# beltegeuse/rustlight

Measured on AMD Instinct MI355X. Metric: Msamples/s (paths/s) at 1080p x 128spp cbox, higher is better.
Workload: dtype f32

## Files before the change

rustlight_amd/csrc/device_types.h:

```cpp
#pragma once
#include <stdint.h>

namespace rl {

struct alignas(16) BvhNode {
    float lmin[3]; float lmax0;
    float lmax12[2]; float rmin01[2];
    float rmin2; float rmax[3];
    int32_t left, right; int32_t pad0, pad1;
};
static_assert(sizeof(BvhNode) == 64, "BvhNode must be 64 bytes");
static const int32_t RL_CHILD_NONE = (int32_t)0x80000000;

struct alignas(16) BvhNode2 {
    float lox[4], loy[4], loz[4];
    float hix[4], hiy[4], hiz[4];
    int32_t slot[4];
    int32_t child[2];
    int32_t pad[2];
};
static_assert(sizeof(BvhNode2) == 128, "BvhNode2 must be 128 bytes");

struct alignas(16) Bvh4Node {
    float org[3];
    uint32_t exps;
    uint32_t qlo[3];
    uint32_t qhi[3];
    int32_t child[4];
    uint32_t pad[2];
};
static_assert(sizeof(Bvh4Node) == 64, "Bvh4Node must be 64 bytes");

struct alignas(16) TriRecord {
    float v0[3]; float n0;
    float e1[3]; float n1;
    float e2[3]; float n2;
    float det;
    int32_t mesh;
    int32_t tri;
    int32_t gtri;
};
static_assert(sizeof(TriRecord) == 64, "TriRecord must be 64 bytes");

struct ColorTex {
    int32_t type;
    float c0[3];
    float c1[3];
    float offset[2];
    float scale[2];
    float line_width;
    int32_t bitmap;
    int32_t pad[3];
};
static_assert(sizeof(ColorTex) == 64, "ColorTex must be 64 bytes");

struct BitmapDesc { uint32_t w, h; uint64_t offset; };

struct Material {
    int32_t type;
    int32_t distribution;
    float exponent, weight_specular;
    float alpha_u, alpha_v;
    float glass_eta, glass_inv_eta;
    int32_t smooth;
    int32_t twosided;
    int32_t pad[2];
    ColorTex diffuse, specular, transmittance, eta, k;
};

struct MeshRecord {
    int32_t material;
    int32_t flags;
    float emission[3];
    float inv_area;
    float emitter_pdf;
    uint32_t vertex_base;
    uint32_t tri_base;
    uint32_t n_tris;
    uint32_t cdf_base;
    uint32_t ats_base;
    int32_t emission_type;
    float emission_scale;
    int32_t emission_bitmap;
};
enum { MESH_HAS_NORMALS = 1, MESH_HAS_UV = 2, MESH_IS_LIGHT = 4 };

enum { EMITTER_MESH = 0, EMITTER_ENV = 1, EMITTER_POINT = 2, EMITTER_DIRECTIONAL = 3 };
struct EmitterRecord {
    int32_t kind;
    int32_t mesh;
    float v[3];
    float c[3];
    float center[3];
    float radius;
    float pad[4];
};
static_assert(sizeof(EmitterRecord) == 64, "EmitterRecord must be 64 bytes");

struct LightNode {
    float bmin[3], bmax[3];
    float axis[3];
    float phi, cos_theta_o, cos_theta_e;
    int32_t left, right, parent;
    int32_t light;
};
static_assert(sizeof(LightNode) == 64, "LightNode must be 64 bytes");

struct CameraRecord {
    float sample_to_camera[16];
    float to_world[16];
    float position[3];
    uint32_t width, height;
};

struct MediumRecord {
    int32_t enabled;
    float sigma_a[3], sigma_s[3], sigma_t[3];
    int32_t phase;
    float g;
};

struct DeviceScene {
    const BvhNode* nodes;
    const TriRecord* tris;
    float root_min[3], root_max[3];
    int32_t root;
    uint32_t n_nodes, n_prims;
    uint32_t stack_depth;
    const BvhNode* nodes_t;
    int32_t root_t;
    const BvhNode2* nodes2;
    const Bvh4Node* nodes4;
    int32_t root4;
    uint32_t stack_depth4;
    const uint32_t* tri_indices;
    const float* positions;
    const float* normals;
    const float* uvs;
    const MeshRecord* meshes;
    const Material* materials;
    const BitmapDesc* bitmaps;
    const float* bitmap_texels;
    const EmitterRecord* emitters;
    const float* emitters_cdf;
    uint32_t n_emitters;
    int32_t env_emitter;
    float env_color[3];
    float env_pdf;
    uint32_t env_w, env_h;
    const float* env_texels;
    const float* env_cond_cdf;
    const float* env_cond_func;
    const float* env_marg_cdf;
    float env_marg_func_int;
    float env_sel_pdf;
    int32_t ats_root;
    const LightNode* ats_nodes;
    const int32_t* ats_light_mesh;
    const int32_t* ats_light_prim;
    const uint32_t* ats_leaf_of;
    const float* mesh_cdf;
    uint32_t n_meshes;
    CameraRecord camera;
    MediumRecord medium;
};

}
```

rustlight_amd/csrc/kernels/fused_body.inc.h:

```cpp
    const RenderConst& rc = rc_arg;
    const DeviceScene& sc = sc_arg;
    extern __shared__ __attribute__((aligned(16))) float4 smem[];
    SceneRecs recs;
    float4* after_scene = smem;
    if (LDS_SCENE) {
        stage_scene_lds(sc, smem, smem + lds_nodes_float4s(sc.n_nodes));
        recs.nodes = smem; recs.tris = smem + lds_nodes_float4s(sc.n_nodes);
        after_scene = smem + lds_scene_float4s(sc.n_nodes, sc.n_prims);
    } else {
        recs.nodes = streamed_nodes<TravStackT<false>>(sc);
        recs.tris = reinterpret_cast<const float4*>(sc.tris);
    }
    const unsigned tid = blockIdx.x * blockDim.x + threadIdx.x;
    unsigned long long* cold_q = reinterpret_cast<unsigned long long*>(after_scene);
    float* cold_f = reinterpret_cast<float*>(cold_q + 256 * FusedState::kColdQ);
    unsigned* cold_u = reinterpret_cast<unsigned*>(cold_f + 256 * FusedState::kColdF);
    const TravStackT<LDS_SCENE> stack(make_stack<LDS_SCENE>(stc, cold_u + 256 * FusedState::kColdU, tid));
    FusedState ps;
    ps.cold_q = cold_q + threadIdx.x; ps.cold_f = cold_f + threadIdx.x; ps.cold_u = cold_u + threadIdx.x;
#pragma unroll
    for (int i = 0; i < F_COUNT; i++) ps.fv[i] = 0.0f;
#pragma unroll
    for (int i = 0; i < U_COUNT; i++) ps.uv[i] = 0u;
#pragma unroll
    for (int i = 0; i < Q_COUNT; i++) ps.qv[i] = 0ull;
    storec(ps, F_AR, czero());
    PU(U_CURSOR) = 0u; PU(U_SAMPLE) = 0u;
    const unsigned item0 = (tid & ((1u << rc.item_shift) - 1u)) == 0u ? (tid >> rc.item_shift) : 0xffffffffu;
    PU(U_ITEM) = item0;
    PU(U_PRIM) = 0xffffffffu;
    PU(U_FLAGS) = item0 < rc.n_items ? (ST_REGEN | ST_FRESH) : ST_FINISHED;
    unsigned n_samples = 0, n_draws = 0, n_vertices = 0, n_shadow = 0, n_ext = 0;
#ifdef RL_STAGE_TIMERS
    unsigned long long tm[4] = {0, 0, 0, 0}, ln[5] = {0, 0, 0, 0, 0};
    unsigned long long sh_hist[5] = {0, 0, 0, 0, 0}, sh_pair[4] = {0, 0, 0, 0}, sh_cyc_exec = 0; unsigned sh_prev = 0, sh_parity = 0;
#define RL_T0 { t0 = __builtin_readcyclecounter(); }
#define RL_T1(K, COND) { unsigned long long t1 = __builtin_readcyclecounter(); tm[K] += t1 - t0; ln[K] += __popcll(__ballot(COND)); t0 = t1; }
    unsigned long long t0;
    const unsigned long long wg_t0 = wall_clock64();
#else
#define RL_T0
#define RL_T1(K, COND)
#endif
    constexpr bool qmode = QUEUE;
    constexpr unsigned kQDone = 0xffffffffu;
    if constexpr (qmode) {
        PU(U_ITEM) = 0u;
        PU(U_FLAGS) = ST_FINISHED;
    }
    for (;;) {
    if constexpr (qmode) {
        const char __attribute__((address_space(4)))* kq = (const char __attribute__((address_space(4)))*)__builtin_amdgcn_kernarg_segment_ptr();
        asm volatile("" : "+s"(kq));
        const RenderConst& rc_arg = *(const RenderConst*)kq;
        const unsigned ipb = 256u * rc_arg.split, total = rc_arg.q_n * ipb;
        unsigned fl = PU(U_FLAGS);
        for (int tries = 0; tries < 4; tries++) {
            if ((fl & ST_FINISHED) && PU(U_ITEM) != kQDone) {
                const unsigned c = atomicAdd(rc_arg.q_ctr, 1u);
                if (c >= total) PU(U_ITEM) = kQDone;
                else {
                    const unsigned j = rc_arg.q_list[c / ipb], idx = c - (c / ipb) * ipb;
                    unsigned bx_, by_, bw_, bh_;
                    block_geometry(rc_arg, rc_arg.owned_blocks[j], &bx_, &by_, &bw_, &bh_);
                    const unsigned npx = min(rc_arg.cursor_end, bw_ * bh_) - min(rc_arg.cursor_begin, bw_ * bh_);
                    if (idx < npx * rc_arg.split) {
                        PU(U_ITEM) = rc_arg.block_item_base[j] * rc_arg.split + idx;
                        PU(U_PRIM) = 0xffffffffu; PU(U_CURSOR) = 0u; PU(U_SAMPLE) = 0u;
                        storec(ps, F_AR, czero());
                        fl = ST_REGEN | ST_FRESH;
                    }
                }
            }
            if (__ballot((fl & ST_FINISHED) && PU(U_ITEM) != kQDone) == 0ull) break;
        }
        PU(U_FLAGS) = fl;
        if (__ballot(!(fl & ST_FINISHED)) == 0ull) {
            if (__ballot((fl & ST_FINISHED) && PU(U_ITEM) != kQDone) == 0ull) break;
            continue;
        }
    }
    if (!(PU(U_FLAGS) & ST_FINISHED)) do {
        const char __attribute__((address_space(4)))* ka = (const char __attribute__((address_space(4)))*)__builtin_amdgcn_kernarg_segment_ptr();
        asm volatile("" : "+s"(ka));
        constexpr size_t sc_off = (sizeof(RenderConst) + alignof(DeviceScene) - 1) / alignof(DeviceScene) * alignof(DeviceScene);
        static_assert(sc_off == offsetof(PathKernargs, sc) && offsetof(PathKernargs, rc) == 0, "kernarg layout of k_path_fused(RenderConst, DeviceScene, StackConf)");
        const DeviceScene& sc = *(const DeviceScene*)(ka + sc_off);
        const RenderConst& rc = MEDIUM ? *(const RenderConst*)ka : rc_arg;
        RL_T0
#ifdef RL_STAGE_TIMERS
        ln[4] += 64;
        const bool c0 = PU(U_FLAGS) & ST_REGEN;
#endif
#ifdef RL_FUSED_BODY_TAIL
        constexpr bool kTail = RL_FUSED_BODY_TAIL;
#else
        constexpr bool kTail = false;
#endif
        if (PU(U_FLAGS) & ST_REGEN) raygen_slot<true, decltype(ps), SMP, kTail>(rc, sc, ps, n_samples, n_draws);
        RL_T1(0, c0)
#ifdef RL_STAGE_TIMERS
        const bool c1 = PU(U_FLAGS) & ST_RAY;
#endif
        if (PU(U_FLAGS) & ST_RAY) {
            extend_slot(sc, recs, stack, ps);
            RL_T1(1, c1)
            shade_slot<MAT, MEDIUM, LIGHTS, false, SMP>(rc, sc, ps, PU(U_FLAGS), n_vertices, n_draws, n_shadow, n_ext);
        }
        RL_T1(2, c1)
#ifdef RL_STAGE_TIMERS
        const bool c3 = PU(U_FLAGS) & ST_SHADOW;
#endif
        if (PU(U_FLAGS) & ST_SHADOW) shadow_slot(sc, recs, stack, ps);
#ifdef RL_STAGE_TIMERS
        { const unsigned nsh = (unsigned)__popcll(__ballot(c3)); sh_hist[nsh == 0u ? 0 : 1 + (nsh - 1u) / 16u]++;
          if (nsh) sh_cyc_exec += __builtin_readcyclecounter() - t0;
          if (sh_parity) { const unsigned a = sh_prev, b = nsh; sh_pair[(a == 0u && b == 0u) ? 0 : ((a == 0u || b == 0u) ? 1 : (a + b <= 64u ? 2 : 3))]++; }
          sh_prev = nsh; sh_parity ^= 1u; }
#endif
        RL_T1(3, c3)
    } while (!qmode && !(PU(U_FLAGS) & ST_FINISHED));
    if (!qmode) break;
    }
#ifdef RL_STAGE_TIMERS
    if ((threadIdx.x & 63u) == 0u) { for (int k = 0; k < 4; k++) { atomicAdd(&g_stage_timers[k], tm[k]); atomicAdd(&g_stage_timers[4 + k], ln[k]); } atomicAdd(&g_stage_timers[8], ln[4]);
        for (int k = 0; k < 5; k++) atomicAdd(&g_stage_timers[16 + k], sh_hist[k]); for (int k = 0; k < 4; k++) atomicAdd(&g_stage_timers[21 + k], sh_pair[k]); atomicAdd(&g_stage_timers[25], sh_cyc_exec); }
#endif
    {
        const int which[5] = {STAT_SAMPLES, STAT_VERTICES, STAT_DRAWS, STAT_SHADOW_RAYS, STAT_EXT_RAYS};
        const unsigned vals[5] = {n_samples, n_vertices, n_draws, n_shadow, n_ext};
        block_stats<5>(rc.partials, which, vals);
    }
#ifdef RL_STAGE_TIMERS
    if (threadIdx.x == 0u && blockIdx.x < kFusedWgSlots) { g_fused_wgs[2 * blockIdx.x] = wg_t0; g_fused_wgs[2 * blockIdx.x + 1] = wall_clock64(); }
#endif
```

rustlight_amd/csrc/kernels/knobs.h:

```cpp
#pragma once
#include <cstdlib>
#include <cstring>
#include <string>

namespace rl {

enum KnobId {
    K_REF_SINGLE_PASS,
    K_STATE_BUDGET_MB,
    K_NO_OVERLAP,
    K_CHAIN_SERIAL,
    K_CHAIN_NO_PRE,
    K_CHAIN_NO_TREELETS,
    K_SPEC_FORCE,
    K_SPEC_DRAWS_PER_SAMPLE,
    K_ITEM_SHIFT,
    K_FUSED_DYNAMIC,
    K_FUSED_TAIL_BLOCKS,
    K_FUSED_TAIL_SPLIT,
    K_FUSED_TAIL_NO_BUFFER_TEST,
    K_EVAL_SPLIT,
    K_EVAL_MIN, K_EVAL_DIV,
    K_NO_EVENTS,
    K_QUEUE_DEBUG,
    K_SPEC_GROUP, K_SPEC_SUB, K_SPEC_CAP, K_SPEC_PROBE, K_SPEC_LEAD, K_SPEC_LEAD_MAX, K_SPEC_LEAD_VAR, K_SPEC_EXTRA, K_SPEC_DENSE, K_SPEC_DENSE_FRAC,
    K_SPEC_PROBE_EVERY, K_SPEC_KS, K_SPEC_KE, K_SPEC_SERIAL_RATIO, K_SPEC_NO_TRIVIAL, K_SPEC_LDS_LIMIT_TEST, K_SPEC_STATS, K_SPEC_WAVE_TIMES,
    K_SPEC_LDS_LEVELS,
    K_VPL_BATCH_PATHS,
    K_PHOTON_TREE_GROUP_PHOTONS,
    K_PLANE_GENERATE_LANES,
    K_PLANE_TREE_DEVICE,
    K_PLANE_TREE_GROUP_PLANES,
    K_PPLANE_TREE_DEVICE,
    K_FORCE_STREAMING,
    K_GENERIC_LIGHTS,
    K_COUNT
};

struct Knobs {
    struct Entry { bool set = false; std::string value; };
    Entry e[K_COUNT];

    static const char* name_of(int k) {
        static const char* const names[K_COUNT] = {
            "ref_single_pass", "state_budget_mb", "no_overlap", "chain_serial", "chain_no_pre", "chain_no_treelets", "spec_force", "spec_draws_per_sample", "item_shift",
            "fused_dynamic", "fused_tail_blocks", "fused_tail_split", "fused_tail_no_buffer_test", "eval_split", "eval_min", "eval_div", "no_events", "queue_debug",
            "spec_group", "spec_sub", "spec_cap", "spec_probe", "spec_lead", "spec_lead_max", "spec_lead_var", "spec_extra", "spec_dense", "spec_dense_frac",
            "spec_probe_every", "spec_ks", "spec_ke", "spec_serial_ratio", "spec_no_trivial", "spec_lds_limit_test", "spec_stats", "spec_wave_times", "spec_lds_levels", "vpl_batch_paths", "photon_tree_group_photons",
            "plane_generate_lanes", "plane_tree_device", "plane_tree_group_planes", "pplane_tree_device",
            "force_streaming", "generic_lights"};
        return names[k];
    }
    static int find(const char* name) {
        if (!name) return -1;
        for (int k = 0; k < K_COUNT; k++) if (std::strcmp(name, name_of(k)) == 0) return k;
        return -1;
    }
    void from_environment() {
        for (int k = 0; k < K_COUNT; k++) {
            std::string env = "RL_";
            for (const char* p = name_of(k); *p; p++) env += (char)((*p >= 'a' && *p <= 'z') ? *p - 'a' + 'A' : *p);
            const char* v = std::getenv(env.c_str());
            e[k].set = v != nullptr;
            e[k].value = v ? v : "";
        }
    }
    bool has(int k) const { return e[k].set; }
    const char* str(int k) const { return e[k].set ? e[k].value.c_str() : nullptr; }
    long long i(int k, long long dflt) const { return e[k].set ? std::atoll(e[k].value.c_str()) : dflt; }
    double f(int k, double dflt) const { return e[k].set ? std::atof(e[k].value.c_str()) : dflt; }
};

}
```

rustlight_amd/csrc/kernels/path_render.hip.h:

```cpp
#pragma once

namespace {

using namespace rl;

std::atomic<int> g_path_renders_in_flight{0};

struct Plan { unsigned split, n_items, P, item_shift; };
struct Chunk { unsigned c0, c1, n_pix; std::vector<unsigned> base; };
struct Tail { unsigned begin, pixels, shift; };

class PathRender : RenderFrame {
public:
    PathRender(rl_context* c, const rl_path_params* p, const uint64_t* seeds, size_t nb, float* out, int out_dev, void* stream_arg, rl_render_stats* s)
        : RenderFrame(c, seeds, nb, out, out_dev, stream_arg, s, p->shard_index, p->shard_count), params(p) {}

    int run() {
        struct InFlight { InFlight() { g_path_renders_in_flight++; } ~InFlight() { g_path_renders_in_flight--; } } in_flight;
        int r;
        if ((r = choose_form()) != RL_OK) return r;
        plan_chunks();
        if ((r = plan_lanes()) != RL_OK) return r;
        if ((r = upload()) != RL_OK) return r;
        if (two_pass) r = run_two_pass();
        else if (fused) r = run_fused();
        else r = run_wavefront();
        if (r != RL_OK) return r;
        return finish();
    }

private:
    const rl_path_params* const params;
    bool per_sample = false, fused = false, fast_math = false, two_pass = false, medium = false;
    bool strat = false;
    bool overlap_wanted = false;
    bool one_lane_per_pixel = false;
    bool overlapped = false;
    size_t state_budget = 0;
    std::vector<Chunk> chunks;
    unsigned max_chunk_pix = 0;
    Plan plan{1u, 0u, 0u, 0u}, plan_chain{1u, 0u, 0u, 0u};
    Tail tail{0u, 0u, 0u};
    long long tail_blocks = 0;
    unsigned tail_shift = 0;
    bool tail_forced = false;
    unsigned split = 1, n_items = 0, item_shift = 0, P = 0, n_item_pixels = 0;
    Pool pool{};
    RenderConst rc{};
    StackConf stc{};
    size_t lds_trav = 0, lds_fused = 0;
    double ms[4] = {0, 0, 0, 0}, ms_fused = 0.0, ms_chain = 0.0, ms_eval_span = 0.0;
    uint64_t iterations = 0, launches = 2, n_extend = 0;
    unsigned long long spec_stat[3] = {0, 0, 0};
    unsigned spec_group = 0;
    bool spec = false;
    SpecConf spc{};
    unsigned spec_threads = 0;
    StackConf stc_c{}, stc_s{};
    size_t lds_chain = 0, lds_spec = 0;
    int spec_levels = -1;

    static constexpr unsigned kMaxEvalLaunches = 256u;
    static constexpr size_t kEventsPerIter = 8;

    int choose_form() {
        strat = params->stream_mode == RL_STREAM_STRATIFIED;
        per_sample = params->stream_mode == RL_STREAM_PER_SAMPLE || strat;
        if (params->pipeline > 2) { rl_set_error("pipeline must be 0 (auto), 1 (wavefront) or 2 (fused)"); return RL_ERR_INVALID_ARGUMENT; }
        fused = params->pipeline == 2 || (params->pipeline == 0 && params->pool_slots == 0);
        fast_math = params->numerics == RL_NUMERICS_FAST;
        if (fast_math && !fused) { rl_set_error("numerics = fast exists for the persistent kernel only (pipeline 0 or 2, pool_slots 0)"); return RL_ERR_UNSUPPORTED; }
        if (fast_math && strat) { rl_set_error("numerics = fast is not built with the stratified sampler (stream_mode = RL_STREAM_STRATIFIED)"); return RL_ERR_UNSUPPORTED; }
        medium = ctx->ds.medium.enabled != 0;
        two_pass = !per_sample && fused && !owned.empty() && !knobs.has(K_REF_SINGLE_PASS);
        state_budget = max_state_bytes();
        if (two_pass && (size_t)owned.size() * params->spp * 32 > state_budget) two_pass = false;
        return RL_OK;
    }

    bool dynamic_items() const { return knobs.has(K_FUSED_DYNAMIC) ? knobs.i(K_FUSED_DYNAMIC, 0) != 0 : (medium || !ctx->lds_scene); }

    Plan plan_items(bool per_pixel, unsigned n_pix, unsigned n_chains, unsigned tail_lanes = 0u) const {
        Plan pl{1u, 0u, 0u, 0u};
        if (per_pixel && n_pix > 0) {
            const unsigned fused_groups = (n_pix + 255u) / 256u;
            const unsigned fused_auto = fused_groups >= 6000u ? 1u : std::max(1u, 16384u / std::max(1u, fused_groups));
            unsigned want = params->sample_split ? params->sample_split
                                : (fused ? (ctx->lds_scene ? fused_auto : std::max(fused_auto, 64u))
                                         : (ctx->lds_scene ? 1u : std::max(1u, (8u << 20) / std::max(1u, n_pix))));
            if (overlap_wanted && !params->sample_split) want = std::max(want, (unsigned)std::max<long long>(1, knobs.i(K_EVAL_SPLIT, 4)));
            if (tail_forced) want = 1u;
            pl.split = std::max(1u, std::min(want, params->spp));
            if ((size_t)n_pix * params->spp * 3 * sizeof(float) > kSampleBufBudget || one_lane_per_pixel) pl.split = 1;
            while (pl.split > 1 && (size_t)n_pix * pl.split > (size_t)0x7fffff00u) pl.split--;
        }
        pl.n_items = per_pixel ? n_pix * pl.split + tail_lanes : n_chains;
        unsigned Pp = params->pool_slots ? std::min(params->pool_slots, std::max(pl.n_items, 1u)) : std::min<unsigned>(pl.n_items, 16u << 20);
        Pp = std::max(256u, (unsigned)(((unsigned long long)Pp + 255ull) / 256ull * 256ull));
        if (fused) {
            const unsigned resident = (unsigned)cus * (unsigned)(ctx->lds_scene ? RL_FUSED_WAVES : RL_FUSED_WAVES_STREAMING) * 256u;
            Pp = std::max(256u, (std::min(pl.n_items, dynamic_items() ? resident : pl.n_items) + 255u) / 256u * 256u);
            const unsigned resident4 = (unsigned)cus * 4u * 256u / ((medium && !per_pixel) ? 2u : 1u);
            while (pl.item_shift < 6u && ((size_t)pl.n_items << (pl.item_shift + 1u)) <= resident4) pl.item_shift++;
            if (!per_pixel && knobs.has(K_ITEM_SHIFT)) pl.item_shift = std::min(6u, (unsigned)std::max<long long>(0, knobs.i(K_ITEM_SHIFT, 0)));
            if (pl.item_shift) Pp = std::max(256u, (unsigned)((((size_t)pl.n_items << pl.item_shift) + 255u) / 256u * 256u));
        }
        pl.P = Pp;
        return pl;
    }

    void plan_chunks() {
        if (two_pass && !knobs.has(K_STATE_BUDGET_MB)) {
            size_t free_b = 0, total_b = 0;
            if (hipMemGetInfo(&free_b, &total_b) == hipSuccess) state_budget = std::min(state_budget, ctx->d_sample_states.capacity() * sizeof(unsigned long long) + free_b / 10 * 6);
            else (void)hipGetLastError();
        }
        for (bool planned_states = false; two_pass && !planned_states;) {
            const size_t budget = state_budget;
            const size_t per_cursor = (size_t)owned.size() * params->spp * 32;
            if (per_cursor > budget) { two_pass = false; chunks.clear(); break; }
            chunks.clear();
            const unsigned cursors_per_chunk = (unsigned)std::max<size_t>(1, std::min<size_t>(256, budget / std::max<size_t>(1, per_cursor)));
            for (unsigned c0 = 0; c0 < 256u; c0 += cursors_per_chunk) {
                Chunk ch; ch.c0 = c0; ch.c1 = std::min(256u, c0 + cursors_per_chunk); ch.n_pix = 0;
                for (size_t j = 0; j < owned.size(); j++) {
                    const BlockRect r = block_rect(owned[j], nby, W, H);
                    const unsigned npx = r.w * r.h;
                    ch.base.push_back(ch.n_pix);
                    ch.n_pix += std::min(ch.c1, npx) - std::min(ch.c0, npx);
                }
                if (ch.n_pix) chunks.push_back(std::move(ch));
            }
            size_t need = 0;
            for (const Chunk& ch : chunks) need = std::max(need, (size_t)ch.n_pix * params->spp * 4);
            if (ctx->d_sample_states.ensure(need) == RL_OK) planned_states = true;
            else state_budget /= 2;
        }
        max_chunk_pix = 0;
        for (const Chunk& ch : chunks) max_chunk_pix = std::max(max_chunk_pix, ch.n_pix);
    }

    int plan_lanes() {
        overlap_wanted = two_pass && ctx->stream2 && !fast_math && !knobs.has(K_NO_OVERLAP) && knobs.i(K_SPEC_GROUP, 0) != 256;
        int rcode;
        tail_request();
        for (int attempt = 0; attempt < 2; attempt++) {
            plan = two_pass ? plan_items(true, max_chunk_pix, 0) : plan_items(per_sample, n_pixels, (unsigned)owned.size());
            if (two_pass) for (const Chunk& ch : chunks) { const Plan pc = plan_items(true, ch.n_pix, 0); plan.P = std::max(plan.P, pc.P); plan.split = std::max(plan.split, pc.split); }
            plan_chain = two_pass ? plan_items(false, 0, (unsigned)owned.size()) : Plan{1u, 0u, 0u, 0u};
            split = plan.split; n_items = plan.n_items; item_shift = plan.item_shift;
            P = std::max(plan.P, plan_chain.P);
            n_item_pixels = two_pass ? max_chunk_pix : n_pixels;
            if (split <= 1) break;
            if (ctx->d_sample_buf.ensure((size_t)n_item_pixels * params->spp * 3) == RL_OK) break;
            if (params->sample_split || attempt == 1) return RL_ERR_HIP;
            one_lane_per_pixel = true; overlap_wanted = false;
        }
        if ((rcode = plan_tail()) != RL_OK) return rcode;
        if ((rcode = alloc_tables()) != RL_OK) return rcode;
        if (per_sample || two_pass) {
            if (per_sample && (rcode = ctx->d_item_seed.ensure(n_item_pixels)) != RL_OK) return rcode;
            if ((rcode = ctx->d_item_pixel.ensure(n_item_pixels)) != RL_OK) return rcode;
        }
        if (two_pass) {
            if ((rcode = ctx->d_sample_states.ensure((size_t)max_chunk_pix * params->spp * 4)) != RL_OK) return rcode;
            if ((rcode = ctx->d_chain_states.ensure(owned.size() * 4)) != RL_OK) return rcode;
        }
        if (!fused && ctx->pool_q.capacity() / Q_COUNT < P) {
            ctx->pool_f.reset(); ctx->pool_u.reset(); ctx->pool_q.reset();
            if (ctx->pool_f.ensure((size_t)F_COUNT * P) != RL_OK || ctx->pool_u.ensure((size_t)U_COUNT * P) != RL_OK || ctx->pool_q.ensure((size_t)Q_COUNT * P) != RL_OK) {
                ctx->pool_f.reset(); ctx->pool_u.reset(); ctx->pool_q.reset();
                rl_set_error("out of device memory for a path-state pool of " + std::to_string(P) + " slots");
                return RL_ERR_HIP;
            }
        }
        pool = Pool{ctx->pool_f.get(), ctx->pool_u.get(), ctx->pool_q.get(), P};
        return alloc_output(std::max<size_t>((P + 255) / 256, (size_t)cus * 8u * rl_context::kEvalStreams));
    }

    static constexpr unsigned kFusedTailBlocks = 512u, kFusedTailSplit = 4u;
    void tail_request() {
        tail_blocks = 0; tail_shift = 0; tail_forced = false;
        if (!per_sample || strat || two_pass || !fused || !ctx->lds_scene || medium || dynamic_items() || params->sample_split || owned.empty()) return;
        const bool large = (n_pixels + 255u) / 256u >= 6000u && ctx->single_bsdf && ctx->bsdf_type == RL_BSDF_DIFFUSE && ctx->area_lights_only && !fast_math && g_path_renders_in_flight.load() <= 1;
        const long long T = knobs.has(K_FUSED_TAIL_BLOCKS) ? knobs.i(K_FUSED_TAIL_BLOCKS, 0) : (large ? (long long)kFusedTailBlocks : 0);
        const long long S = std::min<long long>(std::min<long long>(knobs.has(K_FUSED_TAIL_SPLIT) ? knobs.i(K_FUSED_TAIL_SPLIT, 0) : (long long)kFusedTailSplit, 64), params->spp);
        unsigned shift = 0;
        while ((2ll << shift) <= S) shift++;
        if (T <= 0 || shift == 0u) return;
        tail_blocks = T; tail_shift = shift;
        tail_forced = knobs.has(K_FUSED_TAIL_BLOCKS) || knobs.has(K_FUSED_TAIL_SPLIT);
    }
    int plan_tail() {
        tail = Tail{0u, 0u, 0u};
        if (tail_blocks <= 0 || split != 1u) return RL_OK;
        const long long T = tail_blocks;
        const unsigned shift = tail_shift;
        const bool expand = !params->has_max_depth || 1u < params->max_depth;
        const uint64_t key = ((uint64_t)params->shard_index << 33) | ((uint64_t)shard_count << 1) | (expand ? 1u : 0u);
        if (key != ctx->heavy_key || ctx->heavy_blocks.size() != owned.size()) {
            std::vector<unsigned> masks;
            trivial_pixel_masks(trivial_input(ctx), params, owned, nby, false, &masks, true);
            ctx->heavy_blocks.assign(owned.size(), 0);
            for (size_t j = 0; j < owned.size(); j++) ctx->heavy_blocks[j] = (masks[j * 8] & 1u) ? 0 : 1;
            ctx->heavy_key = key;
        }
        size_t j0 = 0, j1 = 0; long long found = 0;
        for (size_t j = owned.size(); j-- > 0 && found < T;) if (ctx->heavy_blocks[j]) { if (!found) j1 = j; j0 = j; found++; }
        if (!found) return RL_OK;
        const unsigned p0 = item_base[j0], p1 = j1 + 1 < owned.size() ? item_base[j1 + 1] : n_pixels;
        const size_t lanes = (size_t)(p1 - p0) << shift;
        if ((size_t)n_pixels + lanes > (size_t)0x7fffff00u || (size_t)(p1 - p0) * params->spp * 3 * sizeof(float) > kSampleBufBudget) return RL_OK;
        if (knobs.has(K_FUSED_TAIL_NO_BUFFER_TEST) || ctx->d_sample_buf.ensure((size_t)(p1 - p0) * params->spp * 3) != RL_OK) { rl_set_error(""); return RL_OK; }
        tail = Tail{p0, p1 - p0, shift};
        plan = plan_items(true, n_pixels, 0, (unsigned)lanes - tail.pixels);
        n_items = plan.n_items; item_shift = plan.item_shift;
        P = std::max(plan.P, plan_chain.P);
        return RL_OK;
    }

    int upload() {
        int rcode;
        if ((rcode = RenderFrame::upload(!two_pass, true)) != RL_OK) return rcode;
        Counters init{};
        init.active = std::min(plan.P, n_items);
        init.next_item = item_shift ? n_items : plan.P;
        if (!two_pass) HIP_OK(hipMemcpyAsync(ctx->d_counters.get(), &init, sizeof(init), hipMemcpyHostToDevice, st));
        if ((rcode = zero_rows()) != RL_OK) return rcode;

        rc = render_const(params->spp, params->stream_mode, params->seed_variant);
        rc.has_min = params->has_min_depth; rc.min_depth = params->min_depth;
        rc.has_max = params->has_max_depth; rc.max_depth = params->max_depth;
        rc.has_rr = params->has_rr_depth; rc.rr_depth = params->rr_depth;
        rc.strategy = params->strategy; rc.single_scattering = params->single_scattering;
        rc.n_items = n_items;
        rc.item_shift = item_shift;
        rc.split = split; rc.sample_buf = ctx->d_sample_buf.get();
        rc.tail_begin = tail.begin; rc.tail_pixels = tail.pixels; rc.tail_shift = tail.shift; rc.tail_lanes = tail.pixels << tail.shift;
        rc.sample_states = ctx->d_sample_states.get(); rc.chain_states = ctx->d_chain_states.get();

        lds_trav = traversal_lds_bytes(ctx, ctx->lds_scene, 256, true);
        if ((rcode = stack_conf(ctx, (size_t)((P + 255) / 256) * 256, &stc)) != RL_OK) return rcode;
        lds_fused = traversal_lds_bytes(ctx, ctx->lds_scene, 256, false) + kFusedColdBytes;

        const dim3 block(256);
        if (per_sample && !owned.empty()) hipLaunchKernelGGL(k_seed_pixels, dim3(((unsigned)owned.size() + 63) / 64), dim3(64), 0, st, rc);
        if (!fused) hipLaunchKernelGGL(k_init, dim3((plan.P + 255) / 256), block, 0, st, rc, pool);

        return grow_events(kEventsPerIter * (per_sample ? 8u : 32u));
    }

    void launch_fused(const RenderConst& rcl, dim3 grid, hipStream_t on, const StackConf* stcl = nullptr) const {
        const int mat = ctx->single_bsdf ? ctx->bsdf_type : -1;
        const StackConf& s = stcl ? *stcl : stc;
        if (strat)
            (ctx->lds_scene ? launch_fused_strat_lds : launch_fused_strat_stream)(medium, ctx->area_lights_only, grid, dim3(256), lds_fused, on, rcl, ctx->ds, s);
        else if (rcl.queue_mode != 0u)
            (ctx->lds_scene ? launch_fusedq_lds : launch_fusedq_stream)(mat, medium, ctx->area_lights_only, grid, dim3(256), lds_fused, on, rcl, ctx->ds, s);
        else
            (ctx->lds_scene ? (fast_math ? launch_fused_lds_fast : launch_fused_lds) : (fast_math ? launch_fused_stream_fast : launch_fused_stream))(mat, medium, ctx->area_lights_only, grid, dim3(256), lds_fused, on, rcl, ctx->ds, s);
    }

    void drain() const {
        (void)hipStreamSynchronize(st);
        for (int k = 0; k < rl_context::kEvalStreams; k++) if (ctx->eval_streams[k]) (void)hipStreamSynchronize(ctx->eval_streams[k]);
        (void)hipGetLastError();
    }
    struct DrainOnError {
        const PathRender* r; bool armed = true;
        ~DrainOnError() { if (armed) r->drain(); }
    };

    int plan_chain_pass() {
        stc_c = stc;
        if (ctx->lds_scene && !medium && ctx->ds.n_nodes <= 64u && ctx->ds.n_prims <= 64u && plan_chain.item_shift >= 5u && !knobs.has(K_CHAIN_NO_PRE)) stc_c.pre_group = 1 << plan_chain.item_shift;
        const bool treelets = !ctx->lds_scene && !fast_math && ctx->ds.nodes_t && ctx->ds.root_t >= 0 && plan_chain.item_shift >= 5u && ctx->ds.stack_depth <= 512u && !knobs.has(K_CHAIN_NO_TREELETS);
        if (treelets) stc_c.pre_group = 1 << plan_chain.item_shift;
        auto chain_lds_of = [&](bool tl) {
            return traversal_lds_bytes(ctx, ctx->lds_scene, 256, false) + (tl ? (size_t)(256 / stc_c.pre_group) * (72 + (ctx->ds.stack_depth + 1) / 2) * 16
                   : (stc_c.pre_group ? (size_t)(256 / stc_c.pre_group) * ((size_t)ctx->ds.n_nodes * 32 + (size_t)ctx->ds.n_prims * 8) : 0));
        };
        if (chain_lds_of(treelets) > ctx->lds_limit) stc_c.pre_group = 0;
        lds_chain = chain_lds_of(treelets && stc_c.pre_group != 0);

        spec = !fast_math && !knobs.has(K_CHAIN_SERIAL);
        const bool spec_force = knobs.has(K_SPEC_FORCE);
        if (spec && !spec_force) {
            const double nbar = knobs.f(K_SPEC_DRAWS_PER_SAMPLE, medium ? 150.0 : 12.0);
            if ((double)params->spp < 4.0 * nbar) spec = false;
        }
        spec_levels = ctx->lds_scene ? -1 : (int)std::max<long long>(0, std::min<long long>(knobs.i(K_SPEC_LDS_LEVELS, kSpecLdsLevelsStreaming), lds_levels_of(ctx)));
        lds_spec = traversal_lds_bytes(ctx, ctx->lds_scene, 256, false, spec_levels) + (size_t)(kSpecColdWords - (ctx->lds_scene ? 0 : kSpecHelperWords)) * 256 * 4 + kSpecGroupLdsBytes;
        const size_t spec_lds_limit = knobs.has(K_SPEC_LDS_LIMIT_TEST) ? (size_t)knobs.i(K_SPEC_LDS_LIMIT_TEST, 0) : ctx->lds_limit;
        if (lds_spec > spec_lds_limit) spec = false;
        spc = SpecConf{};
        spec_threads = 0;
        if (spec) {
            unsigned group = 16u;
            while (group < 64u && (size_t)owned.size() * group < (size_t)cus * 4u * 2u * 64u) group <<= 1;
            if (!ctx->lds_scene) group = 64u;
            if (knobs.has(K_SPEC_GROUP)) { const long long g = knobs.i(K_SPEC_GROUP, 0); if (g == 16 || g == 32 || g == 64 || g == 256) group = (unsigned)g; }
            spc.group = group;
            spc.sub = std::max(1u, group / 16u);
            spc.serial_ratio = spec_force ? 0.0f : (float)knobs.f(K_SPEC_SERIAL_RATIO, 3.0);
            if (knobs.has(K_SPEC_SUB)) { const long long v = knobs.i(K_SPEC_SUB, 0); if ((v == 1 || v == 2 || v == 4 || v == 8 || v == 16) && (unsigned)v <= group) spc.sub = (unsigned)v; }
            spc.cap = std::max(96u, std::min(3u * params->spp + 64u, 1u << 20));
            if (knobs.has(K_SPEC_CAP)) spc.cap = std::max(4u, (unsigned)knobs.i(K_SPEC_CAP, 0));
            spc.probe = knobs.has(K_SPEC_PROBE) ? (unsigned)knobs.i(K_SPEC_PROBE, 0) : std::min(32u, std::max(4u, params->spp));
            spc.lead = (unsigned)knobs.i(K_SPEC_LEAD, 24);
            spc.lead_max = (unsigned)knobs.i(K_SPEC_LEAD_MAX, 128);
            spc.lead_var = (float)knobs.f(K_SPEC_LEAD_VAR, 100.0);
            spc.extra = (unsigned)knobs.i(K_SPEC_EXTRA, 0);
            spc.dense = !ctx->lds_scene ? 0u : (knobs.has(K_SPEC_DENSE) ? std::min(64u, (unsigned)knobs.i(K_SPEC_DENSE, 0)) : 16u);
            spc.dense_frac = (float)knobs.f(K_SPEC_DENSE_FRAC, 0.6);
            spc.probe_every = (unsigned)knobs.i(K_SPEC_PROBE_EVERY, 0);
            spc.ks = (float)knobs.f(K_SPEC_KS, group >= 64u ? 2.5 : 1.65);
            spc.ke = (float)knobs.f(K_SPEC_KE, group >= 64u ? 2.5 : 1.65);
            spec_threads = (unsigned)((((size_t)owned.size() * group) + 255u) / 256u * 256u);
            const size_t need = (size_t)spec_threads * spc.cap * 36u;
            size_t free_b = 0, total_b = 0;
            const size_t have = ctx->d_trk_off.capacity() * 4u + ctx->d_trk_st.capacity() * 16u;
            if (hipMemGetInfo(&free_b, &total_b) != hipSuccess) { (void)hipGetLastError(); free_b = 0; }
            if (need > have && need - have > free_b / 2u) spec = false;
            if (spec && (ctx->d_trk_off.ensure((size_t)spec_threads * spc.cap) != RL_OK || ctx->d_trk_st.ensure((size_t)spec_threads * spc.cap * 2u) != RL_OK)) spec = false;
        }
        int rcode;
        if (spec) {
            const bool expand = !params->has_max_depth || 1u < params->max_depth;
            const bool no_trivial = knobs.has(K_SPEC_NO_TRIVIAL);
            const uint64_t key = ((uint64_t)params->shard_index << 33) | ((uint64_t)shard_count << 1) | (expand ? 1u : 0u);
            if (key != ctx->trivial_key || ctx->d_trivial.capacity() < owned.size() * 8 || no_trivial) {
                std::vector<unsigned> masks;
                trivial_pixel_masks(trivial_input(ctx), params, owned, nby, no_trivial, &masks);
                if ((rcode = ctx->d_trivial.ensure(masks.size())) != RL_OK) return rcode;
                HIP_OK(hipMemcpyAsync(ctx->d_trivial.get(), masks.data(), masks.size() * sizeof(unsigned), hipMemcpyHostToDevice, st));
                HIP_OK(hipStreamSynchronize(st));
                ctx->trivial_key = no_trivial ? ~0ull : key;
            }
            if ((rcode = ctx->d_spec_stats.ensure(32 + 8 * (size_t)(spec_threads / 64u))) != RL_OK) return rcode;
            HIP_OK(hipMemsetAsync(ctx->d_spec_stats.get(), 0, 32 * sizeof(unsigned long long), st));
            spc.trk_off = ctx->d_trk_off.get(); spc.trk_st = ctx->d_trk_st.get(); spc.trivial = ctx->d_trivial.get();
            spc.stats = (stats || knobs.has(K_SPEC_STATS)) ? ctx->d_spec_stats.get() : nullptr;
            const size_t n_thr = std::max<size_t>((size_t)((P + 255) / 256) * 256, spec_threads);
            if ((rcode = stack_conf(ctx, n_thr, &stc_s, false, spec_levels)) != RL_OK) return rcode;
            if ((rcode = stack_conf(ctx, n_thr, &stc)) != RL_OK) return rcode;
            stc_c.overflow = stc.overflow; stc_c.overflow_stride = stc.overflow_stride;
        }
        return RL_OK;
    }

    void launch_chain_pass(const RenderConst& ra) const {
        const int mat = ctx->single_bsdf ? ctx->bsdf_type : -1;
        if (spec) (ctx->lds_scene ? launch_spec_lds : launch_spec_stream)(mat, medium, dim3(spec_threads / 256u), dim3(256), lds_spec, st, ra, ctx->ds, stc_s, spc);
        else (ctx->lds_scene ? (fast_math ? launch_chain_lds_fast : launch_chain_lds) : (fast_math ? launch_chain_stream_fast : launch_chain_stream))(mat, medium, dim3((plan_chain.P + 255) / 256), dim3(256), lds_chain, st, ra, ctx->ds, stc_c);
    }

    int prepare_queue(RenderConst& ra, unsigned chain_grid) {
        const size_t n_dev = 16 + (size_t)kMaxEvalLaunches + owned.size(), n_flags = 16 + owned.size();
        int rcode;
        if ((rcode = ctx->d_queue.ensure(n_dev)) != RL_OK || (rcode = ctx->h_flags.ensure(n_flags)) != RL_OK || (rcode = ctx->h_list.ensure(owned.size())) != RL_OK) return rcode;
        HIP_OK(hipMemsetAsync(ctx->d_queue.get(), 0, (16 + (size_t)kMaxEvalLaunches) * sizeof(unsigned), st));
        ra.queue = ctx->d_queue.get(); ra.chain_grid = chain_grid;
        ra.done_flags = ctx->h_flags.device_ptr() + 16; ra.started_flag = ctx->h_flags.device_ptr();
        ra.queue_seq = ++ctx->queue_seq;
        if (ra.queue_seq == 0u) { std::memset(ctx->h_flags.get(), 0, ctx->h_flags.capacity() * sizeof(unsigned)); ra.queue_seq = ++ctx->queue_seq; }
        return RL_OK;
    }

    int overlap_loop(const RenderConst& rb, const Plan& pb, unsigned seq, dim3 grid_q, const StackConf& stc_q) {
        HIP_OK(hipEventRecord(ctx->ev_chain_done, st));
        const unsigned n_blocks_owned = (unsigned)owned.size();
        volatile unsigned* hf = ctx->h_flags.get();
        std::vector<unsigned> waiting(n_blocks_owned);
        for (unsigned j = 0; j < n_blocks_owned; j++) waiting[j] = j;
        unsigned n_listed = 0, n_launches = 0, scan_from = 0;
        const auto poll_us = std::chrono::microseconds(50 + n_blocks_owned / 100u);
        bool chain_over = false, started = false;
        const unsigned resident = grid_q.x;
        const unsigned batch_min = (unsigned)std::max<long long>(1, knobs.i(K_EVAL_MIN, 64)), batch_div = (unsigned)std::max<long long>(1, knobs.i(K_EVAL_DIV, 5));
        std::chrono::steady_clock::time_point t_first{};
        auto launch_batch = [&](unsigned first, unsigned count) -> int {
            const unsigned k = n_launches % (unsigned)rl_context::kEvalStreams;
            hipStream_t on = ctx->eval_streams[k];
            HIP_OK(hipMemcpyAsync(ctx->d_queue.get() + 16 + kMaxEvalLaunches + first, ctx->h_list.get() + first, count * sizeof(unsigned), hipMemcpyHostToDevice, on));
            RenderConst rq = rb;
            rq.q_list = ctx->d_queue.get() + 16 + kMaxEvalLaunches + first; rq.q_n = count; rq.q_ctr = ctx->d_queue.get() + 16 + n_launches;
            rq.partials = rb.partials + (size_t)k * resident * STAT_COUNT;
            StackConf stc_k = stc_q;
            if (stc_k.overflow) stc_k.overflow += (size_t)k * resident * 256u * 2u;
            const unsigned wgs = std::min<unsigned>(resident, (unsigned)(((size_t)count * 256u * pb.split + 255u) / 256u));
            if (n_launches == 0) t_first = std::chrono::steady_clock::now();
            launch_fused(rq, dim3(std::max(1u, wgs)), on, &stc_k);
            HIP_OK(hipGetLastError());
            n_launches++; launches++;
            return RL_OK;
        };
        int rcode;
        while (n_listed < n_blocks_owned) {
            if (!chain_over) {
                const hipError_t qe = hipEventQuery(ctx->ev_chain_done);
                if (qe == hipSuccess) chain_over = true;
                else if (qe != hipErrorNotReady) { rl_set_error(std::string("hipEventQuery(chain pass): ") + hipGetErrorString(qe)); (void)hipGetLastError(); return RL_ERR_HIP; }
            }
            if (!started && hf[0] == seq) started = true;
            if (started || chain_over) {
                size_t keep = 0;
                for (size_t w = 0; w < waiting.size(); w++) {
                    const unsigned j = waiting[w];
                    if (chain_over || hf[16 + j] == seq) ctx->h_list.get()[n_listed++] = j; else waiting[keep++] = j;
                }
                waiting.resize(keep);
            }
            const unsigned fresh = n_listed - scan_from, to_come = n_blocks_owned - scan_from;
            if (fresh > 0 && (chain_over || (fresh >= std::max(batch_min, to_come / batch_div) && n_launches + 2u < kMaxEvalLaunches))) {
                if ((rcode = launch_batch(scan_from, fresh)) != RL_OK) return rcode;
                scan_from = n_listed;
            }
            if (n_listed < n_blocks_owned && !chain_over) std::this_thread::sleep_for(poll_us);
        }
        if (scan_from < n_listed && (rcode = launch_batch(scan_from, n_listed - scan_from)) != RL_OK) return rcode;
        if (knobs.has(K_QUEUE_DEBUG)) std::fprintf(stderr, "[queue] %u evaluation launches beside / after the chain pass, %u blocks, started flag %s\n", n_launches, n_listed, started ? "seen" : "not seen");
        HIP_OK(hipStreamSynchronize(st));
        for (int k = 0; k < rl_context::kEvalStreams; k++) HIP_OK(hipStreamSynchronize(ctx->eval_streams[k]));
        if (n_launches) ms_eval_span += std::chrono::duration<double, std::milli>(std::chrono::steady_clock::now() - t_first).count();
        return RL_OK;
    }

    int run_chunk(const Chunk& ch) {
        DrainOnError guard{this};
        const dim3 block(256);
        HIP_OK(hipMemcpyAsync(ctx->d_item_base.get(), ch.base.data(), ch.base.size() * sizeof(unsigned), hipMemcpyHostToDevice, st));
        RenderConst ra = rc;
        ra.stream_mode = RL_STREAM_REFERENCE_ORDER;
        ra.n_items = plan_chain.n_items; ra.item_shift = plan_chain.item_shift; ra.split = 1;
        ra.n_state_pixels = ch.n_pix; ra.cursor_begin = ch.c0; ra.cursor_end = ch.c1;
        const unsigned chain_grid = spec ? spec_threads / 256u : (plan_chain.P + 255u) / 256u;
        const bool overlap = overlap_wanted;
        int rcode;
        if (overlap && (rcode = prepare_queue(ra, chain_grid)) != RL_OK) return rcode;
        hipLaunchKernelGGL(k_chunk_pixels, dim3(((unsigned)owned.size() + 63) / 64), dim3(64), 0, st, ra);
        const Plan pb = plan_items(true, ch.n_pix, 0);
        RenderConst rb = ra;
        rb.stream_mode = kStreamGivenStates;
        rb.n_items = pb.n_items; rb.item_shift = pb.item_shift; rb.split = pb.split;
        rb.queue = nullptr; rb.queue_mode = 0u; rb.done_flags = nullptr; rb.started_flag = nullptr;
        Counters cinit{};
        cinit.active = std::min(pb.P, pb.n_items);
        cinit.next_item = pb.item_shift ? pb.n_items : pb.P;
        if (overlap) cinit.next_item = pb.n_items;
        HIP_OK(hipMemcpyAsync(ctx->d_counters.get(), &cinit, sizeof(cinit), hipMemcpyHostToDevice, st));
        const dim3 grid_q((unsigned)cus * (unsigned)(ctx->lds_scene ? RL_FUSED_WAVES : RL_FUSED_WAVES_STREAMING));
        StackConf stc_q = stc;
        if (overlap && (rcode = stack_conf(ctx, (size_t)grid_q.x * 256 * rl_context::kEvalStreams, &stc_q, true)) != RL_OK) return rcode;
        if (timing) hipEventRecord(ctx->events[0], st);
        launch_chain_pass(ra);
        if (timing) hipEventRecord(ctx->events[1], st);
        HIP_OK(hipGetLastError());
        if (overlap) {
            rb.queue = ctx->d_queue.get(); rb.queue_mode = 1u; rb.chain_grid = chain_grid;
            if ((rcode = overlap_loop(rb, pb, ra.queue_seq, grid_q, stc_q)) != RL_OK) return rcode;
            overlapped = true;
            if (timing) hipEventRecord(ctx->events[3], st);
        } else {
            if (timing) hipEventRecord(ctx->events[2], st);
            launch_fused(rb, dim3((pb.P + 255) / 256), st);
            if (timing) hipEventRecord(ctx->events[3], st);
        }
        if (pb.split > 1) hipLaunchKernelGGL(k_fold_samples, dim3((ch.n_pix + 255) / 256), block, 0, st, rb);
        HIP_OK(hipGetLastError());
        HIP_OK(hipStreamSynchronize(st));
        guard.armed = false;
        if (timing) {
            float t = 0.0f;
            HIP_OK(hipEventElapsedTime(&t, ctx->events[0], ctx->events[1])); ms_chain += t;
            HIP_OK(hipEventElapsedTime(&t, ctx->events[overlap ? 1 : 2], ctx->events[3])); ms_fused += t;
            if (!overlap) ms_eval_span += t;
        }
        launches += 3 + (pb.split > 1 ? 1 : 0);
        return RL_OK;
    }

    int run_two_pass() {
        int rcode;
        if ((rcode = plan_chain_pass()) != RL_OK) return rcode;
        for (const Chunk& ch : chunks) if ((rcode = run_chunk(ch)) != RL_OK) return rcode;
        dump_stage_timers(ctx->lds_scene);
        if (ctx->lds_scene) dump_chain_timers_lds(); else dump_chain_timers_stream();
        if (spec && spc.stats && (rcode = read_spec_stats()) != RL_OK) return rcode;
        iterations = chunks.size();
        return RL_OK;
    }

    int read_spec_stats() {
        unsigned long long spec_totals[32] = {0};
        HIP_OK(hipMemcpy(spec_totals, ctx->d_spec_stats.get(), sizeof(spec_totals), hipMemcpyDeviceToHost));
        spec_group = spc.group; spec_stat[0] = spec_totals[0]; spec_stat[1] = spec_totals[1]; spec_stat[2] = spec_totals[2];
        const bool verbose = knobs.has(K_SPEC_STATS);
        if (verbose) std::fprintf(stderr, "[spec] LDS per workgroup %zu bytes (scene %zu, %d stack levels)\n", lds_spec, (size_t)(ctx->lds_scene ? ctx->scene_lds_bytes : 0), stc_s.lds_levels);
        if (verbose) std::fprintf(stderr, "[spec] group %u x sub %u cap %u: %llu speculative + %llu serial + %llu probe samples for %llu camera samples (%.2f x, %.2f serial per pixel), %llu wave iterations\n",
            spc.group, spc.sub, spc.cap, spec_totals[0], spec_totals[1], spec_totals[2], (unsigned long long)n_pixels * params->spp,
            (double)(spec_totals[0] + spec_totals[1] + spec_totals[2]) / std::max(1.0, (double)n_pixels * params->spp), (double)spec_totals[1] / std::max(1u, n_pixels), spec_totals[3]);
        if (knobs.has(K_SPEC_WAVE_TIMES) && spec_totals[8]) {
            std::vector<unsigned long long> wt(8 * (size_t)(spec_threads / 64u));
            HIP_OK(hipMemcpy(wt.data(), ctx->d_spec_stats.get() + 32, wt.size() * 8, hipMemcpyDeviceToHost));
            FILE* f = std::fopen(knobs.str(K_SPEC_WAVE_TIMES), "w");
            if (f) { unsigned long long t0 = ~0ull; for (size_t w = 0; w < wt.size() / 8; w++) if (wt[8 * w]) t0 = std::min(t0, wt[8 * w]);
                     for (size_t w = 0; w < wt.size() / 8; w++) std::fprintf(f, "%zu %.3f %.3f %llu %llu %.3f %.3f %llu %llu\n", w, (wt[8 * w] - t0) * 1e-5, (wt[8 * w + 1] - t0) * 1e-5, wt[8 * w + 2], wt[8 * w + 3], wt[8 * w + 4] * 1e-5, wt[8 * w + 5] * 1e-5, wt[8 * w + 6], wt[8 * w + 7]); std::fclose(f); }
        }
        if (verbose && spec_totals[8]) {
            const double tot = (double)(spec_totals[4] + spec_totals[5] + spec_totals[6] + spec_totals[7] + spec_totals[8]);
            std::fprintf(stderr, "[spec] cycles: bookkeeping %.1f %%, plan %.1f %%, thread %.1f %%, copy-out %.1f %%, extend+shade %.1f %%; %.1f lanes per traced iteration, %.1f %% of the traced iterations serial only, %.0f cycles per wave iteration\n",
                100.0 * spec_totals[4] / tot, 100.0 * spec_totals[5] / tot, 100.0 * spec_totals[6] / tot, 100.0 * spec_totals[7] / tot, 100.0 * spec_totals[8] / tot,
                (double)spec_totals[9] / std::max<double>(1.0, (double)spec_totals[10]), 100.0 * spec_totals[11] / std::max<double>(1.0, (double)spec_totals[10]), tot / std::max<double>(1.0, (double)spec_totals[3]));
            { const double ts = (double)(spec_totals[16] + spec_totals[17] + spec_totals[18] + spec_totals[19] + spec_totals[20]);
              std::fprintf(stderr, "[spec] iterations after a serial-only one (%.1f %% of all cycles): bookkeeping %.1f %%, plan %.1f %%, thread %.1f %%, copy-out %.1f %%, extend+shade %.1f %%\n", 100.0 * ts / tot,
                100.0 * spec_totals[16] / ts, 100.0 * spec_totals[17] / ts, 100.0 * spec_totals[18] / ts, 100.0 * spec_totals[19] / ts, 100.0 * spec_totals[20] / ts); }
            std::fprintf(stderr, "[spec] slow walks: %llu from a pixel's start, %llu across a missing link, %llu past the last track\n", spec_totals[12], spec_totals[13], spec_totals[14]);
            std::fprintf(stderr, "[spec] serial walks on helpers: %llu (one lane: %llu), %llu rounds, %llu samples taken from them\n", spec_totals[26], spec_totals[27], spec_totals[24], spec_totals[25]);
        }
        return RL_OK;
    }

    int run_fused() {
        if (timing) hipEventRecord(ctx->events[0], st);
        launch_fused(rc, dim3((plan.P + 255) / 256), st);
        if (timing) hipEventRecord(ctx->events[1], st);
        HIP_OK(hipGetLastError());
        HIP_OK(hipStreamSynchronize(st));
        if (timing) { float t = 0.0f; HIP_OK(hipEventElapsedTime(&t, ctx->events[0], ctx->events[1])); ms_fused = t; ms_eval_span = t; }
        dump_stage_timers(ctx->lds_scene);
        launches += 1;
        iterations = 1;
        return RL_OK;
    }

    int run_wavefront() {
        const dim3 block(256);
        const dim3 grid_all((plan.P + 255) / 256);
        const bool use_sort = !ctx->single_bsdf;
        const unsigned sort_chunks = split > 1 ? 4u : 1u;
        const dim3 grid_sort((P + 1023) / 1024);
        const dim3 grid_persistent(std::min<unsigned>((P + 255) / 256, (unsigned)cus * 8u));
        const unsigned poll_every = per_sample ? 8u : 32u;
        const DeviceScene& ds = ctx->ds;
        unsigned in_batch = 0;
        auto flush_events = [&](unsigned count) -> int {
            for (unsigned i = 0; i < count; i++)
                for (int k = 0; k < 4; k++) {
                    float t = 0.0f;
                    HIP_OK(hipEventElapsedTime(&t, ctx->events[kEventsPerIter * i + 2 * k], ctx->events[kEventsPerIter * i + 2 * k + 1]));
                    ms[k] += t;
                }
            return RL_OK;
        };
        for (;;) {
            hipEvent_t* ev = timing ? &ctx->events[kEventsPerIter * in_batch] : nullptr;
            if (timing) hipEventRecord(ev[0], st);
            if (strat) launch_raygen_strat(grid_persistent, block, st, rc, ds, pool);
            else hipLaunchKernelGGL(k_raygen, grid_persistent, block, 0, st, rc, ds, pool);
            if (timing) { hipEventRecord(ev[1], st); hipEventRecord(ev[2], st); }
            if (ctx->lds_scene) hipLaunchKernelGGL((k_extend<true>), grid_all, block, lds_trav, st, rc, ds, pool, stc);
            else hipLaunchKernelGGL((k_extend<false>), grid_all, block, lds_trav, st, rc, ds, pool, stc);
            if (timing) { hipEventRecord(ev[3], st); hipEventRecord(ev[4], st); }
            if (strat) launch_shade_sorted_strat(medium, sort_chunks, sort_chunks == 4u ? grid_sort : grid_all, block, st, rc, ds, pool);
            else if (use_sort) launch_shade_sorted(medium, sort_chunks, sort_chunks == 4u ? grid_sort : grid_all, block, st, rc, ds, pool);
            else launch_shade_type(ctx->bsdf_type, medium, grid_all, block, st, rc, ds, pool);
            launches += 1;
            if (timing) { hipEventRecord(ev[5], st); hipEventRecord(ev[6], st); }
            if (ctx->lds_scene) hipLaunchKernelGGL((k_shadow<true>), grid_all, block, lds_trav, st, rc, ds, pool, stc);
            else hipLaunchKernelGGL((k_shadow<false>), grid_all, block, lds_trav, st, rc, ds, pool, stc);
            if (timing) hipEventRecord(ev[7], st);
            launches += 3;
            n_extend++;
            iterations++;
            in_batch++;
            if (in_batch == poll_every) {
                HIP_OK(hipGetLastError());
                HIP_OK(hipMemcpyAsync(ctx->h_counters.get(), ctx->d_counters.get(), sizeof(Counters), hipMemcpyDeviceToHost, st));
                HIP_OK(hipStreamSynchronize(st));
                if (timing) { int r = flush_events(in_batch); if (r != RL_OK) return r; }
                in_batch = 0;
                if (ctx->h_counters.get()->active == 0) break;
            }
            if (iterations > (uint64_t)1 << 28) { rl_set_error("render did not terminate"); return RL_ERR_HIP; }
        }
#ifdef RL_TRAV_STATS
        {
            unsigned long long h[8];
            HIP_OK(hipStreamSynchronize(st));
            hipMemcpyFromSymbol(h, HIP_SYMBOL(g_trav_stats), sizeof(h));
            std::fprintf(stderr, "[trav] rays %llu (zero-step %.1f %%)  steps/ray %.1f  tris/ray %.1f  waves %llu  lanes/wave %.1f  paid steps/ray %.1f  step utilisation %.1f %%\n",
                         h[0], 100.0 * h[5] / (double)h[0], (double)h[1] / h[0], (double)h[2] / h[0], h[4], (double)h[0] / h[4], (double)h[3] / h[0], 100.0 * h[1] / (double)h[3]);
            std::memset(h, 0, sizeof(h)); hipMemcpyToSymbol(HIP_SYMBOL(g_trav_stats), h, sizeof(h));
        }
#endif
        return RL_OK;
    }

    int finish() {
        if (split > 1 && !two_pass) { hipLaunchKernelGGL(k_fold_samples, dim3((n_pixels + 255) / 256), dim3(256), 0, st, rc); launches += 1; }
        else if (tail.pixels) { hipLaunchKernelGGL(k_fold_samples, dim3((tail.pixels + 255) / 256), dim3(256), 0, st, rc); launches += 1; }
        const int rcode = download();
        if (rcode != RL_OK) return rcode;
        if (stats) {
            stats->iterations = iterations;
            stats->kernel_launches = launches;
            stats->ms_raygen = ms[0]; stats->ms_extend = ms[1]; stats->ms_shade = ms[2]; stats->ms_shadow = ms[3];
            stats->ms_other = ms_fused;
            stats->ms_prepass = ms_chain;
            stats->n_extend_launches = n_extend;
            stats->reserved[0] = spec_stat[0]; stats->reserved[1] = spec_stat[1]; stats->reserved[2] = spec_stat[2]; stats->reserved[3] = spec_group;
            stats->chunks = two_pass ? (uint32_t)chunks.size() : 0u;
            stats->overlapped = overlapped ? 1u : 0u;
            stats->ms_eval_span = ms_eval_span;
        }
        return RL_OK;
    }
};

}
```

rustlight_amd/csrc/kernels/pathstate.hip.h:

```cpp
#pragma once

namespace rl {

enum FField {
    F_OX, F_OY, F_OZ, F_DX, F_DY, F_DZ,
    F_T, F_U, F_V,
    F_BR, F_BG, F_BB,
    F_TR, F_TG, F_TB,
    F_LR, F_LG, F_LB,
    F_AR, F_AG, F_AB,
    F_WR, F_WG, F_WB,
    F_RR, F_PDF,
    F_SX, F_SY, F_SZ,
    F_CR, F_CG, F_CB,
    F_XI,
    F_COUNT
};
enum UField { U_FLAGS, U_DEPTH, U_PRIM, U_ITEM, U_CURSOR, U_SAMPLE, U_COUNT };
enum QField { Q_R0, Q_R1, Q_R2, Q_R3, Q_I0, Q_I1, Q_I2, Q_I3, Q_COUNT };

enum : unsigned {
    ST_FINISHED = 1u,
    ST_REGEN = 2u,
    ST_FRESH = 4u,
    ST_RAY = 8u,
    ST_SHADOW = 16u,
    ST_PREV_SHIFT = 5u,
    ST_PDF_SA = 128u,
    ST_ZEROED = 256u,
};
enum : unsigned { PREV_SENSOR = 0u, PREV_SURFACE = 1u, PREV_SURFACE_SMOOTH = 2u, PREV_VOLUME = 3u };

#ifndef RL_FUSED_WAVES
#define RL_FUSED_WAVES 4
#endif
#ifndef RL_FUSED_WAVES_STREAMING
#define RL_FUSED_WAVES_STREAMING 6
#endif
static constexpr unsigned kDepthCap = 2048u;

struct Pool {
    float* f;
    unsigned* u;
    unsigned long long* q;
    unsigned P;
};

struct Counters {
    unsigned int active;
    unsigned int next_item;
    unsigned int pad[2];
};

static constexpr int kLdsStackLevels = 12;
static constexpr size_t kSampleBufBudget = (size_t)16 << 30;
struct StackConf { int lds_levels; int* overflow; size_t overflow_stride; int pre_group; };

#ifndef RL_SPEC_LDS_LEVELS_STREAMING
#define RL_SPEC_LDS_LEVELS_STREAMING 4
#endif
static constexpr int kSpecLdsLevelsStreaming = RL_SPEC_LDS_LEVELS_STREAMING;
static constexpr int kSpecColdWords = 30;
static constexpr int kSpecHelperWords = 2;
static constexpr size_t kSpecGroupLdsBytes = (256 / 16) * 32 + 64 + (256 / 16) * 64 + (256 / 16) * 16;
struct SpecConf {
    unsigned group;
    unsigned sub;
    unsigned cap;
    unsigned probe;
    unsigned lead;
    unsigned lead_max; float lead_var;
    unsigned extra;
    unsigned probe_every;
    unsigned dense; float dense_frac;
    float serial_ratio;
    float ks, ke;
    unsigned* trk_off;
    ulonglong2* trk_st;
    const unsigned* trivial;
    unsigned long long* stats;
};

template <bool LDS_ONLY = false>
RL_DEV TravStackT<LDS_ONLY> make_stack(const StackConf& sc_, unsigned* lds_after_list, size_t global_thread) {
    TravStackT<LDS_ONLY> st;
    st.lds = (typename TravStackT<LDS_ONLY>::LdsPtr)(lds_after_list) + threadIdx.x;
    st.lds_levels = sc_.lds_levels;
    st.glob = sc_.overflow ? (typename TravStackT<LDS_ONLY>::GlobPtr)(sc_.overflow) + global_thread : nullptr;
    st.glob_stride = sc_.overflow_stride;
    return st;
}

struct RenderConst {
    unsigned spp;
    int has_min, has_max, has_rr;
    unsigned min_depth, max_depth, rr_depth;
    int strategy, single_scattering;
    int stream_mode, seed_variant;
    float inv_spp;
    unsigned W, H, nby;
    unsigned n_items;
    unsigned item_shift;
    unsigned split;
    float* sample_buf;
    const unsigned* owned_blocks;
    const unsigned* block_item_base;
    unsigned n_owned;
    const unsigned long long* block_seeds;
    unsigned long long* item_seed;
    unsigned* item_pixel;
    float* out;
    Counters* counters;
    unsigned long long* partials;
    unsigned long long* sample_states;
    unsigned n_state_pixels;
    unsigned cursor_begin, cursor_end;
    unsigned long long* chain_states;
    unsigned* queue;
    unsigned* done_flags;
    unsigned* started_flag;
    unsigned queue_seq, chain_grid;
    unsigned queue_mode;
    const unsigned* q_list;
    unsigned q_n;
    unsigned* q_ctr;
    unsigned tail_begin, tail_lanes, tail_shift, tail_pixels;
};
RL_DEV void queue_workgroup_started(const RenderConst& rc) {
    if (atomicAdd(rc.queue, 1u) + 1u == rc.chain_grid) __hip_atomic_store(rc.started_flag, rc.queue_seq, __ATOMIC_RELEASE, __HIP_MEMORY_SCOPE_SYSTEM);
}
RL_DEV void queue_push(const RenderConst& rc, unsigned item) {
    __builtin_amdgcn_fence(__ATOMIC_RELEASE, "agent");
    __hip_atomic_store(&rc.done_flags[item], rc.queue_seq, __ATOMIC_RELEASE, __HIP_MEMORY_SCOPE_SYSTEM);
}
enum : int { kStreamGivenStates = 1000 };

struct PathKernargs { RenderConst rc; DeviceScene sc; StackConf stc; };
struct SpecKernargs { RenderConst rc; DeviceScene sc; StackConf stc; SpecConf spec; };

struct PoolState {
    Pool pool; unsigned slot;
    RL_DEV float& f(int field) const { return pool.f[(size_t)field * pool.P + slot]; }
    RL_DEV unsigned& u(int field) const { return pool.u[(size_t)field * pool.P + slot]; }
    RL_DEV unsigned long long& q(int field) const { return pool.q[(size_t)field * pool.P + slot]; }
};
struct RegState {
    float fv[F_COUNT]; unsigned uv[U_COUNT]; unsigned long long qv[Q_COUNT];
    RL_DEV float& f(int field) { return fv[field]; }
    RL_DEV unsigned& u(int field) { return uv[field]; }
    RL_DEV unsigned long long& q(int field) { return qv[field]; }
};
struct FusedState {
    float fv[F_COUNT]; unsigned uv[U_COUNT]; unsigned long long qv[Q_COUNT];
    float* cold_f; unsigned* cold_u; unsigned long long* cold_q;
    static constexpr int kColdF = 3, kColdU = 3, kColdQ = 4;
    RL_DEV float& f(int field) { return (field >= F_AR && field <= F_AB) ? cold_f[(field - F_AR) * 256] : fv[field]; }
    RL_DEV unsigned& u(int field) { return (field >= U_ITEM && field <= U_SAMPLE) ? cold_u[(field - U_ITEM) * 256] : uv[field]; }
    RL_DEV unsigned long long& q(int field) { return (field >= Q_I0) ? cold_q[(field - Q_I0) * 256] : qv[field]; }
};
static constexpr size_t kFusedColdBytes = 256 * (FusedState::kColdQ * 8 + FusedState::kColdF * 4 + FusedState::kColdU * 4);
#define PF(field) ps.f(field)
#define PU(field) ps.u(field)
#define PQ(field) ps.q(field)

template <class PS> RL_DEV V3 load3(PS& ps, int f0) { return mk3(PF(f0), PF(f0 + 1), PF(f0 + 2)); }
template <class PS> RL_DEV Col loadc(PS& ps, int f0) { return mkc(PF(f0), PF(f0 + 1), PF(f0 + 2)); }
template <class PS> RL_DEV void store3(PS& ps, int f0, V3 v) { PF(f0) = v.x; PF(f0 + 1) = v.y; PF(f0 + 2) = v.z; }
template <class PS> RL_DEV void storec(PS& ps, int f0, Col c) { PF(f0) = c.r; PF(f0 + 1) = c.g; PF(f0 + 2) = c.b; }
template <class PS> RL_DEV Rng load_rng(PS& ps, int q0) { Rng r; r.s0 = PQ(q0); r.s1 = PQ(q0 + 1); r.s2 = PQ(q0 + 2); r.s3 = PQ(q0 + 3); return r; }
template <class PS> RL_DEV void store_rng(PS& ps, int q0, const Rng& r) { PQ(q0) = r.s0; PQ(q0 + 1) = r.s1; PQ(q0 + 2) = r.s2; PQ(q0 + 3) = r.s3; }

enum { STAT_SAMPLES, STAT_VERTICES, STAT_EXT_RAYS, STAT_SHADOW_RAYS, STAT_DRAWS, STAT_COUNT = 8 };
RL_DEV unsigned wave_sum(unsigned v) {
    for (int off = 32; off > 0; off >>= 1) v += __shfl_down(v, off, 64);
    return v;
}
template <int N>
RL_DEV void block_stats(unsigned long long* partials, const int (&which)[N], const unsigned (&vals)[N]) {
    __shared__ unsigned s_acc[N];
    if (threadIdx.x < N) s_acc[threadIdx.x] = 0u;
    __syncthreads();
#pragma unroll
    for (int k = 0; k < N; k++) {
        unsigned v = wave_sum(vals[k]);
        if ((threadIdx.x & 63u) == 0u && v) atomicAdd(&s_acc[k], v);
    }
    __syncthreads();
    if (threadIdx.x < N && s_acc[threadIdx.x]) partials[(size_t)blockIdx.x * STAT_COUNT + which[threadIdx.x]] += s_acc[threadIdx.x];
}

RL_DEV unsigned block_compact(bool pred, unsigned slot, unsigned* list) {
    const unsigned lane = threadIdx.x & 63u, wave = threadIdx.x >> 6;
    const unsigned long long mask = __ballot(pred);
    const unsigned rank = __popcll(mask & ((1ull << lane) - 1ull));
    unsigned* wave_cnt = list + 256;
    if (lane == 0u) wave_cnt[wave] = (unsigned)__popcll(mask);
    __syncthreads();
    unsigned base = 0, total = 0;
#pragma unroll
    for (unsigned w = 0; w < 4u; w++) { unsigned c = wave_cnt[w]; if (w < wave) base += c; total += c; }
    if (pred) list[base + rank] = slot;
    __syncthreads();
    return total;
}

RL_DEV void block_geometry(const RenderConst& rc, unsigned b, unsigned* bx, unsigned* by, unsigned* bw, unsigned* bh) {
    *bx = (b / rc.nby) * 16u;
    *by = (b % rc.nby) * 16u;
    *bw = min(16u, rc.W - *bx);
    *bh = min(16u, rc.H - *by);
}

}
```

rustlight_amd/csrc/kernels/shade.hip:

```cpp
#include "common.hip.h"
#include "shade_sorted.hip.h"

namespace rl {

template <int MAT, bool MEDIUM>
__global__ void __launch_bounds__(256) k_shade(RenderConst rc, DeviceScene sc, Pool pool) {
    unsigned slot = blockIdx.x * blockDim.x + threadIdx.x;
    unsigned n_vertices = 0, n_draws = 0, n_shadow = 0, n_ext = 0;
    PoolState ps{pool, slot};
    unsigned flags = slot < pool.P ? PU(U_FLAGS) : 0u;
    if (flags & ST_RAY) shade_slot<MAT, MEDIUM>(rc, sc, ps, flags, n_vertices, n_draws, n_shadow, n_ext);
    {
        const int which[4] = {STAT_VERTICES, STAT_DRAWS, STAT_SHADOW_RAYS, STAT_EXT_RAYS};
        const unsigned vals[4] = {n_vertices, n_draws, n_shadow, n_ext};
        block_stats<4>(rc.partials, which, vals);
    }
}

template <bool MEDIUM, unsigned CHUNKS>
__global__ void __launch_bounds__(256, RL_SORT_WAVES) k_shade_sorted(RenderConst rc, DeviceScene sc, Pool pool) {
    using SMP = Rng;
#include "shade_sorted_body.inc.h"
}

void launch_shade_type(int type, bool medium, dim3 grid, dim3 block, hipStream_t st, const RenderConst& rc, const DeviceScene& ds, const Pool& pool) {
    with_bsdf(type, [&](auto M) {
        if constexpr (decltype(M)::value < 0) launch_shade_sorted(medium, 1u, grid, block, st, rc, ds, pool);
        else with_flag(medium, [&](auto MED) { hipLaunchKernelGGL((k_shade<decltype(M)::value, decltype(MED)::value>), grid, block, 0, st, rc, ds, pool); });
    });
}

void launch_shade_sorted(bool medium, unsigned chunks, dim3 grid, dim3 block, hipStream_t st, const RenderConst& rc, const DeviceScene& ds, const Pool& pool) {
    with_flag(chunks == 4u, [&](auto FOUR) { with_flag(medium, [&](auto MED) {
        hipLaunchKernelGGL((k_shade_sorted<decltype(MED)::value, decltype(FOUR)::value ? 4u : 1u>), grid, block, 0, st, rc, ds, pool);
    }); });
}

}
```

rustlight_amd/csrc/kernels/shade_sorted_body.inc.h:

```cpp
    __shared__ unsigned s_list[256 * CHUNKS];
    __shared__ unsigned s_cnt[kNumBins][CHUNKS][4];
    unsigned n_vertices = 0, n_draws = 0, n_shadow = 0, n_ext = 0;
    const unsigned lane = threadIdx.x & 63u, wave = threadIdx.x >> 6;
    unsigned slot[CHUNKS], rank[CHUNKS];
    int bin[CHUNKS];
#pragma unroll
    for (unsigned c = 0; c < CHUNKS; c++) {
        slot[c] = (blockIdx.x * CHUNKS + c) * blockDim.x + threadIdx.x;
        const unsigned flags = slot[c] < pool.P ? pool.u[(size_t)U_FLAGS * pool.P + slot[c]] : 0u;
        bin[c] = -1;
        if (flags & ST_RAY) {
            const int prim = (int)pool.u[(size_t)U_PRIM * pool.P + slot[c]];
            bin[c] = 0;
            if (prim >= 0) bin[c] = sc.materials[sc.meshes[sc.tris[prim].mesh].material].type;
        }
        rank[c] = 0;
#pragma unroll
        for (int b = 0; b < kNumBins; b++) {
            const unsigned long long mask = __ballot(bin[c] == b);
            if (bin[c] == b) rank[c] = __popcll(mask & ((1ull << lane) - 1ull));
            if (lane == 0u) s_cnt[b][c][wave] = (unsigned)__popcll(mask);
        }
    }
    __syncthreads();
    unsigned bin_begin[kNumBins + 1];
    unsigned my_off[CHUNKS];
    unsigned run = 0;
#pragma unroll
    for (int b = 0; b < kNumBins; b++) {
        bin_begin[b] = run;
#pragma unroll
        for (unsigned c = 0; c < CHUNKS; c++)
#pragma unroll
            for (unsigned w = 0; w < 4u; w++) { if (b == bin[c] && w == wave) my_off[c] = run; run += s_cnt[b][c][w]; }
    }
    bin_begin[kNumBins] = run;
#pragma unroll
    for (unsigned c = 0; c < CHUNKS; c++) if (bin[c] >= 0) s_list[my_off[c] + rank[c]] = slot[c];
    __syncthreads();
#define RL_SHADE_BIN(B)                                                                                       \
    { const unsigned n = bin_begin[(B) + 1] - bin_begin[B];                                                   \
      for (unsigned i = threadIdx.x; i < n; i += blockDim.x) { PoolState pb{pool, s_list[bin_begin[B] + i]};    \
          shade_slot<B, MEDIUM, LIGHTS_ANY, false, SMP>(rc, sc, pb, pb.u(U_FLAGS), n_vertices, n_draws, n_shadow, n_ext); } }
    RL_SHADE_BIN(0) RL_SHADE_BIN(1) RL_SHADE_BIN(2) RL_SHADE_BIN(3) RL_SHADE_BIN(4)
#undef RL_SHADE_BIN
    {
        const int which[4] = {STAT_VERTICES, STAT_DRAWS, STAT_SHADOW_RAYS, STAT_EXT_RAYS};
        const unsigned vals[4] = {n_vertices, n_draws, n_shadow, n_ext};
        block_stats<4>(rc.partials, which, vals);
    }
```

rustlight_amd/csrc/kernels/shading.hip.h:

```cpp
#pragma once
#include "../device_types.h"
#include "devmath.hip.h"

namespace rl {

enum { BSDF_DIFFUSE = 0, BSDF_PHONG = 1, BSDF_METAL = 2, BSDF_GLASS = 3, BSDF_SUBSTRATE = 4 };
enum { TEXTURE_CONSTANT = 0, TEXTURE_CHECKER = 1, TEXTURE_GRID = 2, TEXTURE_BITMAP = 3 };
enum { MICRO_NONE = 0, MICRO_BECKMANN = 1, MICRO_GGX = 2 };
enum { PDF_SOLID_ANGLE = 0, PDF_AREA = 1, PDF_DISCRETE = 2 };

struct SurfacePoint {
    V3 p, n_g, n_s, wi;
    Frame frame;
    V2 uv;
    bool has_uv;
    int mesh;
};

RL_DEV unsigned long long f32_as_usize(float f) { if (!(f > 0.0f)) return 0ull; if (f >= 1.8446744e19f) return ~0ull; return (unsigned long long)f; }
RL_DEV int f32_as_i32(float f) { if (f != f) return 0; if (f >= 2147483648.0f) return 2147483647; if (f <= -2147483648.0f) return (-2147483647 - 1); return (int)f; }
RL_DEV float modulo1(float a) { return fmodf(fmodf(a, 1.0f) + 1.0f, 1.0f); }

RL_DEV Col tex_color(const DeviceScene& sc, const ColorTex& t, bool has_uv, V2 uv) {
    if (t.type == TEXTURE_CONSTANT) return mkc(t.c0[0], t.c0[1], t.c0[2]);
// ... 151 lines not shown
    if (d.type == MICRO_BECKMANN) {
        float tan2 = alpha_sqr * -m_logf(1.0f - s.x);
        cos_m = div_rn(1.0f, sqrt_rn(1.0f + tan2));
        pdf = div_rn(1.0f - s.x, kPi * d.au * d.av * powi_f(cos_m, 3));
    } else {
        float tan2 = div_rn(alpha_sqr * s.x, 1.0f - s.x);
        cos_m = div_rn(1.0f, sqrt_rn(1.0f + tan2));
        float tmp = 1.0f + div_rn(tan2, alpha_sqr);
        pdf = div_rn(kInvPi, d.au * d.av * powi_f(cos_m, 3) * powi_f(tmp, 2));
    }
    if (pdf < 1e-20f) pdf = 0.0f;
    float sin_m = sqrt_rn(rmax(1.0f - powi_f(cos_m, 2), 0.0f));
    *m = mk3(sin_m * cos_phi, sin_m * sin_phi, cos_m);
    *pdf_out = pdf;
}
RL_DEV float smith_g1(const Micro& d, V3 v, V3 m) {
    if (dot(v, m) * v.z <= 0.0f) return 0.0f;
    float tt = fabsf(tan_theta(v));
    if (tt == 0.0f) return 1.0f;
    float alpha = d.au;
    if (d.type == MICRO_BECKMANN) {
        float a = div_rn(1.0f, alpha * tt);
        if (a >= 1.6f) return 1.0f;
        float a2 = powi_f(a, 2);
        return div_rn(3.535f * a + 2.181f * a2, 1.0f + 2.276f * a + 2.577f * a2);
    }
    float root = alpha * tt;
    return div_rn(2.0f, 1.0f + hypot2(1.0f, root));
}
RL_DEV float micro_g(const Micro& d, V3 wi, V3 wo, V3 m) { return smith_g1(d, wi, m) * smith_g1(d, wo, m); }

struct BsdfSample { Col weight; V3 d; float pdf; int pdf_kind; };

RL_DEV Col schlick_fresnel(const DeviceScene& sc, const Material& mat, bool huv, V2 uv, float cos_t) {
    Col rs = tex_color(sc, mat.specular, huv, uv);
    return rs + (cone() - rs) * powi_f(1.0f - cos_t, 5);
}

template <int MAT>
RL_DEV float bsdf_pdf(const DeviceScene& sc, const Material& mat, bool huv, V2 uv, V3 wi, V3 wo, bool discrete) {
    const int type = MAT >= 0 ? MAT : mat.type;
    if (type == BSDF_DIFFUSE) {
        if (wi.z <= 0.0f) return 0.0f;
        if (wo.z <= 0.0f) return 0.0f;
        return wo.z * kInvPi;
    }
    if (type == BSDF_PHONG) {
        if (wi.z <= 0.0f || wo.z <= 0.0f) return 0.0f;
        float alpha = dot(reflect_z(wi), wo);
        float ps = 0.0f;
        if (alpha > 0.0f) ps = div_rn(mat.weight_specular * m_powf(alpha, mat.exponent) * (mat.exponent + 1.0f), 2.0f * kPi);
        float pd = (1.0f - mat.weight_specular) * wo.z * kInvPi;
        return ps + pd;
    }
    if (type == BSDF_METAL) {
        if (mat.distribution == MICRO_NONE) return 1.0f;
        V3 h = normalize(wi + wo);
        Micro d = {mat.distribution, mat.alpha_u, mat.alpha_v};
        return div_rn(micro_pdf(d, h), 4.0f * fabsf(dot(wo, h)));
    }
    if (type == BSDF_SUBSTRATE) {
        if (wi.z <= 0.0f || wo.z <= 0.0f) return 0.0f;
        V3 m = wi + wo;
        if (m.x == 0.0f && m.y == 0.0f && m.z == 0.0f) return 0.0f;
        m = normalize(m);
        if (discrete) return 0.5f;
        float pd = wo.z * kInvPi;
        float ps = 0.0f;
        if (mat.distribution != MICRO_NONE) {
            Micro d = {mat.distribution, mat.alpha_u, mat.alpha_v};
            ps = div_rn(micro_pdf(d, m), 4.0f * fabsf(dot(wo, m)));
        }
        return 0.5f * (pd + ps);
    }
    return 0.0f;
}

template <int MAT>
RL_DEV Col bsdf_eval(const DeviceScene& sc, const Material& mat, bool huv, V2 uv, V3 wi, V3 wo, bool discrete) {
    const int type = MAT >= 0 ? MAT : mat.type;
    if (type == BSDF_DIFFUSE) {
        if (wi.z <= 0.0f) return czero();
        if (wo.z > 0.0f) return tex_color(sc, mat.diffuse, huv, uv) * wo.z * kInvPi;
        return czero();
    }
    if (type == BSDF_PHONG) {
        if (wi.z <= 0.0f || wo.z <= 0.0f) return czero();
        float alpha = dot(reflect_z(wi), wo);
        Col spec = czero();
        if (alpha > 0.0f) spec = tex_color(sc, mat.specular, huv, uv) * div_rn(m_powf(alpha, mat.exponent) * (mat.exponent + 2.0f), 2.0f * kPi);
        Col diff = tex_color(sc, mat.diffuse, huv, uv) * wo.z * kInvPi;
        return spec + diff;
    }
    if (type == BSDF_METAL) {
        if (mat.distribution == MICRO_NONE)
            return tex_color(sc, mat.specular, huv, uv) * fresnel_conductor(fabsf(wi.z), tex_color(sc, mat.eta, huv, uv), tex_color(sc, mat.k, huv, uv));
        V3 h = normalize(wi + wo);
        Micro d = {mat.distribution, mat.alpha_u, mat.alpha_v};
        float dv = micro_eval(d, h);
        if (dv == 0.0f) return czero();
        Col f = tex_color(sc, mat.specular, huv, uv) * fresnel_conductor(dot(wi, h), tex_color(sc, mat.eta, huv, uv), tex_color(sc, mat.k, huv, uv));
        float g = micro_g(d, wi, wo, h);
        float model = div_rn(dv * g, 4.0f * wi.z);
        return f * model;
    }
    if (type == BSDF_SUBSTRATE) {
        if (wi.z <= 0.0f || wo.z <= 0.0f) return czero();
        V3 m = wi + wo;
        if (m.x == 0.0f && m.y == 0.0f && m.z == 0.0f) return czero();
        m = normalize(m);
        if (discrete) return schlick_fresnel(sc, mat, huv, uv, dot(wi, m));
        Col diff = tex_color(sc, mat.diffuse, huv, uv) * (cone() - tex_color(sc, mat.specular, huv, uv)) *
                   div_rn(28.0f, 23.0f * kPi) * (1.0f - powi_f(1.0f - 0.5f * fabsf(wi.z), 5)) * (1.0f - powi_f(1.0f - 0.5f * fabsf(wo.z), 5));
        Col spec = czero();
        if (mat.distribution != MICRO_NONE) {
            Micro d = {mat.distribution, mat.alpha_u, mat.alpha_v};
            float model = div_rn(micro_eval(d, m), 4.0f * fabsf(dot(wi, m)) * rmax(fabsf(wi.z), fabsf(wo.z)));
            spec = model * schlick_fresnel(sc, mat, huv, uv, dot(wi, m));
        }
        return (diff + spec) * wo.z;
    }
    return czero();
}

template <int MAT, bool RADIANCE = false>
RL_DEV bool bsdf_sample(const DeviceScene& sc, const Material& mat, bool huv, V2 uv, V3 wi, V2 s, BsdfSample* out) {
    const int type = MAT >= 0 ? MAT : mat.type;
    if (type == BSDF_DIFFUSE) {
        if (wi.z <= 0.0f) return false;
        V3 d = cosine_sample_hemisphere(s);
        out->weight = tex_color(sc, mat.diffuse, huv, uv);
        out->d = d; out->pdf = d.z * kInvPi; out->pdf_kind = PDF_SOLID_ANGLE;
        return true;
    }
    if (type == BSDF_PHONG) {
        if (wi.z <= 0.0f) return false;
        V3 d;
        if (s.x < mat.weight_specular) {
            s.x = div_rn(s.x, mat.weight_specular);
            float sin_a = sqrt_rn(1.0f - m_powf(s.y, div_rn(2.0f, mat.exponent + 1.0f)));
            float cos_a = m_powf(s.y, div_rn(1.0f, mat.exponent + 1.0f));
            float phi = 2.0f * kPi * s.x;
            V3 local = mk3(sin_a * m_cosf(phi), sin_a * m_sinf(phi), cos_a);
            Frame fr = make_frame(reflect_z(wi));
            d = to_world(fr, local);
            if (d.z <= 0.0f) return false;
        } else {
            s.x = div_rn(s.x - mat.weight_specular, 1.0f - mat.weight_specular);
            d = cosine_sample_hemisphere(s);
        }
        float p = bsdf_pdf<MAT>(sc, mat, huv, uv, wi, d, false);
        if (p == 0.0f) return false;
        out->weight = bsdf_eval<MAT>(sc, mat, huv, uv, wi, d, false) / p;
        out->d = d; out->pdf = p; out->pdf_kind = PDF_SOLID_ANGLE;
        return true;
    }
    if (type == BSDF_METAL) {
        if (wi.z <= 0.0f) return false;
        if (mat.distribution == MICRO_NONE) {
            out->weight = tex_color(sc, mat.specular, huv, uv) * fresnel_conductor(wi.z, tex_color(sc, mat.eta, huv, uv), tex_color(sc, mat.k, huv, uv));
            out->d = reflect_z(wi); out->pdf = 1.0f; out->pdf_kind = PDF_DISCRETE;
            return true;
        }
        Micro di = {mat.distribution, mat.alpha_u, mat.alpha_v};
        V3 m; float p;
        micro_sample(di, s, &m, &p);
        if (p == 0.0f) return false;
        V3 wo = reflect_vector(wi, m);
        if (wo.z <= 0.0f) return false;
        Col f = fresnel_conductor(dot(wi, m), tex_color(sc, mat.eta, huv, uv), tex_color(sc, mat.k, huv, uv)) * tex_color(sc, mat.specular, huv, uv);
        float w = div_rn(micro_eval(di, m) * micro_g(di, wi, wo, m) * dot(wi, m), p * wi.z);
        out->weight = w * f;
        out->d = wo; out->pdf = p; out->pdf_kind = PDF_SOLID_ANGLE;
        return true;
    }
    if (type == BSDF_GLASS) {
        float fres, cos_t;
        fresnel_dielectric(wi.z, mat.glass_eta, &fres, &cos_t);
        if (s.x <= fres) {
            out->weight = tex_color(sc, mat.specular, huv, uv);
            out->d = reflect_z(wi);
        } else {
            float factor = RADIANCE ? (cos_t < 0.0f ? mat.glass_inv_eta : mat.glass_eta) : 1.0f;
            float scale = cos_t < 0.0f ? -mat.glass_inv_eta : -mat.glass_eta;
            out->weight = tex_color(sc, mat.transmittance, huv, uv) * factor * factor;
            out->d = mk3(scale * wi.x, scale * wi.y, cos_t);
        }
        out->pdf = fres; out->pdf_kind = PDF_DISCRETE;
        return true;
    }
    if (type == BSDF_SUBSTRATE) {
        if (wi.z <= 0.0f) return false;
        V3 d; bool discrete = false;
        if (s.x < 0.5f) {
            s.x *= 2.0f;
            d = cosine_sample_hemisphere(s);
        } else {
            s.x = (s.x - 0.5f) * 2.0f;
            V3 m;
            if (mat.distribution == MICRO_NONE) { m = mk3(0.0f, 0.0f, 1.0f); discrete = true; }
            else {
                Micro di = {mat.distribution, mat.alpha_u, mat.alpha_v};
                float p;
                micro_sample(di, s, &m, &p);
                if (p == 0.0f) return false;
            }
            d = reflect_vector(wi, m);
            if (d.z <= 0.0f) return false;
        }
        float p = bsdf_pdf<MAT>(sc, mat, huv, uv, wi, d, discrete);
        if (p == 0.0f) return false;
        Col f = bsdf_eval<MAT>(sc, mat, huv, uv, wi, d, discrete);
        out->weight = f / p;
        out->d = d; out->pdf = p; out->pdf_kind = discrete ? PDF_DISCRETE : PDF_SOLID_ANGLE;
        return true;
    }
    return false;
}

RL_DEV unsigned int cdf_sample(const float* cdf, unsigned int n_entries, float v) {
    unsigned int lo = 0, hi = n_entries;
    while (lo < hi) { unsigned int mid = lo + (hi - lo) / 2; if (cdf[mid] <= v) lo = mid + 1; else hi = mid; }
    return lo ? lo - 1 : 0u;
}

struct LightSample { float pdf; int pdf_kind; V3 p, n, d; Col weight; int kind; };

RL_DEV float clamp_f(float v, float lo, float hi) { return v < lo ? lo : (v > hi ? hi : v); }
RL_DEV float cdf_sample_continuous(const float* cdf, unsigned int n, float v) {
    unsigned int i = cdf_sample(cdf, n + 1, v);
    float dv = v - cdf[i];
    float p = cdf[i + 1] - cdf[i];
    if (p > 0.0f) dv = div_rn(dv, p);
    return (float)i + dv;
}
RL_DEV float env_bin_pdf(const DeviceScene& sc, unsigned long long x, unsigned long long y) {
    return div_rn(sc.env_cond_func[y * sc.env_w + x], sc.env_marg_func_int);
}
RL_DEV V2 env_to_spherical(V3 d) {
    float p = dm::atan2f_det(d.y, d.x);
    if (p < 0.0f) p = p + 2.0f * kPi;
    V2 uv; uv.x = p * kInvPi * 0.5f; uv.y = dm::acosf_det(clamp_f(d.z, -1.0f, 1.0f)) * kInvPi;
    uv.x = clamp_f(uv.x, 0.0f, 0.9999999403953552f);
    uv.y = clamp_f(uv.y, 0.0f, 0.9999999403953552f);
    return uv;
}
RL_DEV Col env_eval(const DeviceScene& sc, V3 d) {
    if (sc.env_w == 0u) return mkc(sc.env_color[0], sc.env_color[1], sc.env_color[2]);
    V2 uv = env_to_spherical(d);
    float ux = modulo1(uv.x), uy = modulo1(uv.y);
    unsigned long long x = f32_as_usize(ux * (float)sc.env_w), y = f32_as_usize(uy * (float)sc.env_h);
    unsigned long long i = (unsigned long long)sc.env_w * y + x;
    if (i >= (unsigned long long)sc.env_w * sc.env_h) return czero();
    return mkc(sc.env_texels[3 * i], sc.env_texels[3 * i + 1], sc.env_texels[3 * i + 2]);
}
RL_DEV float env_direct_pdf(const DeviceScene& sc, V3 d) {
    if (sc.env_w == 0u) return sc.env_pdf;
    V2 uv = env_to_spherical(d);
    float p = env_bin_pdf(sc, f32_as_usize(uv.x * (float)sc.env_w), f32_as_usize(uv.y * (float)sc.env_h));
    float st = m_sinf(kPi * uv.y);
    float v = st == 0.0f ? 0.0f : div_rn(p, (2.0f * powi_f(kPi, 2)) * st);
    return v * sc.env_sel_pdf;
}
RL_DEV void env_sample_direction(const DeviceScene& sc, V2 u, V3* d, Col* value, float* pdf) {
    float y = cdf_sample_continuous(sc.env_marg_cdf, sc.env_h, u.y);
    unsigned long long row = f32_as_usize(y);
    float x = cdf_sample_continuous(sc.env_cond_cdf + row * (sc.env_w + 1u), sc.env_w, u.x);
    x = clamp_f(x, 0.0f, (float)sc.env_w - 1.0f);
    y = clamp_f(y, 0.0f, (float)sc.env_h - 1.0f);
    unsigned long long px = f32_as_usize(x), py = f32_as_usize(y);
    const float* t = sc.env_texels + 3ull * (py * sc.env_w + px);
    float p = env_bin_pdf(sc, px, py);
    float sp, cp, st, ct;
    m_sincosf(div_rn(2.0f * kPi, (float)sc.env_w) * x, &sp, &cp);
    m_sincosf(div_rn(kPi, (float)sc.env_h) * y, &st, &ct);
    *d = mk3(st * cp, st * sp, ct);
    if (st == 0.0f) { *value = czero(); *pdf = 0.0f; }
    else { *value = mkc(t[0], t[1], t[2]); *pdf = div_rn(p, (2.0f * powi_f(kPi, 2)) * st); }
}

RL_DEV bool bsphere_intersect(V3 center, float radius, V3 o, V3 d, float tnear, float tfar, float* t_out) {
    V3 d_p = center - o;
    float a = length2(d);
    float b = 2.0f * dot(d_p, d);
    float c = length2(d_p) - radius * radius;
    float x0, x1;
    if (a == 0.0f) {
        if (b == 0.0f) return false;
        float v = div_rn(-c, b);
        x0 = v; x1 = v;
    } else {
        float disc = b * b - 4.0f * a * c;
        if (disc < 0.0f) return false;
        float d_sqrt = sqrt_rn(disc);
        float tmp = b < 0.0f ? -0.5f * (b - d_sqrt) : -0.5f * (b + d_sqrt);
        float r0 = div_rn(tmp, a), r1 = div_rn(c, tmp);
        if (r0 > r1) { x0 = r1; x1 = r0; } else { x0 = r0; x1 = r1; }
    }
    if (x0 < tnear) { if (x1 < tfar) { *t_out = x1; return true; } return false; }
    if (x0 < tfar) { *t_out = x0; return true; }
    return false;
}

template <int LIGHTS = LIGHTS_ANY>
RL_DEV void mesh_sample_triangle(const DeviceScene& sc, const MeshRecord& mr, unsigned int prim, float pdf_area, V3 p, V2 uv, LightSample* ls) {
    unsigned int gtri = mr.tri_base + prim;
    unsigned int i0 = sc.tri_indices[3 * gtri], i1 = sc.tri_indices[3 * gtri + 1], i2 = sc.tri_indices[3 * gtri + 2];
    V3 v0 = mk3(sc.positions[3 * i0], sc.positions[3 * i0 + 1], sc.positions[3 * i0 + 2]);
    V3 v1 = mk3(sc.positions[3 * i1], sc.positions[3 * i1 + 1], sc.positions[3 * i1 + 2]);
    V3 v2 = mk3(sc.positions[3 * i2], sc.positions[3 * i2 + 1], sc.positions[3 * i2 + 2]);
    V2 b = uniform_sample_triangle(uv);
    float w2 = 1.0f - b.x - b.y;
    V3 pos = v0 * b.x + v1 * b.y + v2 * w2;
    V3 n_g = normalize(cross(v2 - v0, v1 - v0));
    if (mr.flags & MESH_HAS_NORMALS) {
        V3 n0 = mk3(sc.normals[3 * i0], sc.normals[3 * i0 + 1], sc.normals[3 * i0 + 2]);
        V3 n1 = mk3(sc.normals[3 * i1], sc.normals[3 * i1 + 1], sc.normals[3 * i1 + 2]);
        V3 n2 = mk3(sc.normals[3 * i2], sc.normals[3 * i2 + 1], sc.normals[3 * i2 + 2]);
        V3 n = n0 * b.x + n1 * b.y + n2 * w2;
        float nl = length2(n);
        if (nl == 0.0f) n = n_g;
        else if (nl != 1.0f) n = n / sqrt_rn(nl);
        if (dot(n_g, n) < 0.0f) n_g = -n_g;
    }
    if (pdf_area < 0.0f) pdf_area = div_rn(1.0f, length(cross(v1 - v0, v2 - v0)) * 0.5f);
    V3 d = pos - p;
    float dist = length(d);
    if (dist != 0.0f) d = d / dist;
    float geom = dist != 0.0f ? div_rn(rmax(dot(n_g, -d), 0.0f), dist * dist) : 0.0f;
    float pdf = geom == 0.0f ? 0.0f : div_rn(pdf_area, geom);
    Col emit;
    if (LIGHTS == LIGHTS_AREA_ONLY || __builtin_expect(mr.emission_type == 0, 1)) emit = mkc(mr.emission[0], mr.emission[1], mr.emission[2]);
    else emit = mesh_emit_sampled(sc.bitmaps, sc.bitmap_texels, sc.uvs, mr.emission_type, mr.emission_scale, mr.emission_bitmap, (mr.flags & MESH_HAS_UV) != 0, i0, i1, i2, b.x, b.y, w2);
    ls->weight = pdf == 0.0f ? czero() : emit * geom / pdf_area;
    ls->pdf = pdf; ls->pdf_kind = PDF_SOLID_ANGLE;
    ls->p = pos; ls->n = n_g; ls->d = d;
}

RL_DEV float ats_cos_subtended(V3 bmin, V3 bmax, V3 p) {
    V3 c = (bmax - bmin) * 0.5f + bmin;
    float radius = length(c - bmax);
    if (length2(p - c) < radius * radius) return -1.0f;
    float sin2 = div_rn(radius * radius, length2(c - p));
    return sqrt_rn(rmax(1.0f - sin2, 0.0f));
}
RL_DEV float ats_cos_sub(float sa, float ca, float sb, float cb) { return ca > cb ? 1.0f : ca * cb + sa * sb; }
RL_DEV float ats_sin_sub(float sa, float ca, float sb, float cb) { return ca > cb ? 1.0f : sa * cb - ca * sb; }
RL_DEV float ats_importance(const LightNode& nd, V3 p, bool has_n, V3 n) {
    V3 bmin = mk3(nd.bmin[0], nd.bmin[1], nd.bmin[2]), bmax = mk3(nd.bmax[0], nd.bmax[1], nd.bmax[2]);
    V3 pc = (bmax - bmin) * 0.5f + bmin;
    float d2 = rmax(length2(p - pc), 0.0001f);
    V3 wi = normalize(p - pc);
    float cos_theta = dot(mk3(nd.axis[0], nd.axis[1], nd.axis[2]), wi);
    float sin_theta = sqrt_rn(rmax(1.0f - cos_theta * cos_theta, 0.0f));
    float cos_u = ats_cos_subtended(bmin, bmax, p);
    float sin_u = sqrt_rn(rmax(1.0f - cos_u * cos_u, 0.0f));
    float sin_o = sqrt_rn(rmax(1.0f - nd.cos_theta_o * nd.cos_theta_o, 0.0f));
    float cos_x = ats_cos_sub(sin_theta, cos_theta, sin_o, nd.cos_theta_o);
    float sin_x = ats_sin_sub(sin_theta, cos_theta, sin_o, nd.cos_theta_o);
    float cos_p = ats_cos_sub(sin_x, cos_x, sin_u, cos_u);
    if (cos_p <= nd.cos_theta_e) return 0.0f;
    float imp = div_rn(nd.phi * cos_p, d2);
    if (has_n) {
        float cos_i = fabsf(dot(wi, n));
        float sin_i = sqrt_rn(rmax(1.0f - cos_i * cos_i, 0.0f));
        imp = imp * ats_cos_sub(sin_i, cos_i, sin_u, cos_u);
    }
    return rmax(imp, 0.0f);
}
RL_DEV float ats_prob_left(const DeviceScene& sc, const LightNode& nd, V3 p, bool has_n, V3 n) {
    float il = ats_importance(sc.ats_nodes[nd.left], p, has_n, n), ir = ats_importance(sc.ats_nodes[nd.right], p, has_n, n);
    return (il == 0.0f && ir == 0.0f) ? 0.5f : div_rn(il, il + ir);
}
RL_DEV int ats_sample(const DeviceScene& sc, float r, V3 p, bool has_n, V3 n, float* pdf_sel) {
    float pdf = 1.0f;
    int ni = sc.ats_root;
    for (;;) {
        const LightNode nd = sc.ats_nodes[ni];
        if (nd.left < 0 && nd.right < 0) { *pdf_sel = pdf; return nd.light; }
        float pl = ats_prob_left(sc, nd, p, has_n, n);
        if (r < pl) { r = div_rn(r, pl); ni = nd.left; pdf = pdf * pl; }
        else { r = div_rn(r - pl, 1.0f - pl); ni = nd.right; pdf = pdf * (1.0f - pl); }
    }
}
RL_DEV float ats_pdf(const DeviceScene& sc, unsigned int leaf, V3 p, bool has_n, V3 n) {
    int id = (int)leaf;
    float pdf = 1.0f;
    for (;;) {
        int ip = sc.ats_nodes[id].parent;
        if (ip < 0) break;
        const LightNode nd = sc.ats_nodes[ip];
        float pl = ats_prob_left(sc, nd, p, has_n, n);
        pdf = nd.left == id ? pdf * pl : pdf * (1.0f - pl);
        id = ip;
    }
    return pdf;
}

template <int LIGHTS = LIGHTS_ANY>
RL_DEV LightSample sample_light(const DeviceScene& sc, V3 p, bool has_n, V3 n, float r_sel, float r, V2 uv) {
    if (LIGHTS != LIGHTS_AREA_ONLY && sc.ats_root >= 0) {
        float pdf_sel;
        int li = ats_sample(sc, r_sel, p, has_n, n, &pdf_sel);
        LightSample ls;
        ls.kind = EMITTER_MESH;
        mesh_sample_triangle<LIGHTS>(sc, sc.meshes[sc.ats_light_mesh[li]], (unsigned int)sc.ats_light_prim[li], -1.0f, p, uv, &ls);
        ls.weight = div_unguarded(ls.weight, pdf_sel);
        ls.pdf = ls.pdf * pdf_sel;
        return ls;
    }
    unsigned int id = cdf_sample(sc.emitters_cdf, sc.n_emitters + 1, r_sel);
    float pdf_sel = sc.emitters_cdf[id + 1] - sc.emitters_cdf[id];
    const EmitterRecord em = sc.emitters[id];
    LightSample ls;
    ls.kind = LIGHTS == LIGHTS_AREA_ONLY ? (int)EMITTER_MESH : em.kind;
    if (LIGHTS == LIGHTS_AREA_ONLY || em.kind == EMITTER_MESH) {
        MeshRecord mr = sc.meshes[em.mesh];
        unsigned int prim = cdf_sample(sc.mesh_cdf + mr.cdf_base, mr.n_tris + 1, r);
        mesh_sample_triangle<LIGHTS>(sc, mr, prim, mr.inv_area, p, uv, &ls);
    } else if (em.kind == EMITTER_POINT) {
        V3 lp = mk3(em.v[0], em.v[1], em.v[2]);
        V3 d = lp - p;
        float dist = length(d);
        d = d / dist;
        ls.pdf = 1.0f; ls.pdf_kind = PDF_DISCRETE;
        ls.p = lp; ls.n = mk3(0.0f, 0.0f, 0.0f); ls.d = d;
        ls.weight = mkc(em.c[0], em.c[1], em.c[2]) / powi_f(dist, 2);
    } else if (em.kind == EMITTER_DIRECTIONAL) {
        V3 dir = mk3(em.v[0], em.v[1], em.v[2]);
        ls.pdf = 1.0f; ls.pdf_kind = PDF_DISCRETE;
        ls.p = p - em.radius * dir; ls.n = dir; ls.d = -dir;
        ls.weight = mkc(em.c[0], em.c[1], em.c[2]);
    } else {
        V3 d; float pdf; Col lum = mkc(em.c[0], em.c[1], em.c[2]);
        if (sc.env_w) env_sample_direction(sc, uv, &d, &lum, &pdf);
        else { d = sample_uniform_sphere(uv); pdf = div_rn(1.0f, kPi * 4.0f); }
        float t;
        ls.pdf = pdf; ls.pdf_kind = PDF_SOLID_ANGLE; ls.d = d;
        if (!bsphere_intersect(mk3(em.center[0], em.center[1], em.center[2]), em.radius, p, d, kEps, kF32Max, &t)) {
            ls.p = mk3(0.0f, 0.0f, 0.0f); ls.n = mk3(0.0f, 0.0f, 0.0f); ls.weight = czero();
        } else {
            ls.p = p + d * t;
            ls.n = normalize(mk3(em.center[0], em.center[1], em.center[2]) - ls.p);
            ls.weight = lum / pdf;
        }
    }
    ls.weight = div_unguarded(ls.weight, pdf_sel);
    ls.pdf = ls.pdf * pdf_sel;
    return ls;
}

template <int LIGHTS = LIGHTS_ANY>
RL_DEV float light_direct_pdf(const DeviceScene& sc, const MeshRecord& mr, int prim_in_mesh, V3 o, V3 p, V3 n, V3 dir, bool has_ns, V3 ns) {
    float cos_light = rmax(dot(n, -dir), 0.0f);
    if (LIGHTS != LIGHTS_AREA_ONLY && sc.ats_root >= 0) {
        float tri = 0.0f;
        if (cos_light != 0.0f) {
            float geom = div_rn(cos_light, length2(p - o));
            unsigned int gtri = mr.tri_base + (unsigned int)prim_in_mesh;
            unsigned int i0 = sc.tri_indices[3 * gtri], i1 = sc.tri_indices[3 * gtri + 1], i2 = sc.tri_indices[3 * gtri + 2];
            V3 v0 = mk3(sc.positions[3 * i0], sc.positions[3 * i0 + 1], sc.positions[3 * i0 + 2]);
            V3 v1 = mk3(sc.positions[3 * i1], sc.positions[3 * i1 + 1], sc.positions[3 * i1 + 2]);
            V3 v2 = mk3(sc.positions[3 * i2], sc.positions[3 * i2 + 1], sc.positions[3 * i2 + 2]);
            float area_tri = length(cross(v1 - v0, v2 - v0)) * 0.5f;
            tri = div_rn(div_rn(1.0f, area_tri), geom);
        }
        return tri * ats_pdf(sc, sc.ats_leaf_of[mr.ats_base + (unsigned int)prim_in_mesh], o, has_ns, ns);
    }
    if (cos_light == 0.0f) return 0.0f * mr.emitter_pdf;
    float geom = div_rn(cos_light, length2(p - o));
    return div_rn(mr.inv_area, geom) * mr.emitter_pdf;
}

struct MediumSample { float t; Col w; bool exited; };
RL_DEV Col cexp(Col c) {
    if ((c.r == c.g) & (c.g == c.b)) { const float e = m_expf(c.r); return mkc(e, e, e); }
    return mkc(m_expf(c.r), m_expf(c.g), m_expf(c.b));
}
RL_DEV MediumSample medium_sample(const MediumRecord& m, float max_t, float u) {
    Col sigma_t = mkc(m.sigma_t[0], m.sigma_t[1], m.sigma_t[2]);
    Col sigma_s = mkc(m.sigma_s[0], m.sigma_s[1], m.sigma_s[2]);
    float u3 = u * 3.0f;
    int component = u3 != u3 ? 0 : (u3 <= 0.0f ? 0 : (u3 >= 255.0f ? 255 : (int)u3));
    u = u * 3.0f - (float)component;
    float sigma_t_c = cget(sigma_t, component);
    float t = div_rn(-m_logf(1.0f - u), sigma_t_c);
    float t_min = rmin(t, max_t);
    bool exited = t >= max_t;
    Col tau = t_min * sigma_t;
    Col w = cexp(-tau);
    float pdf;
    if (exited) pdf = cavg(cexp(-tau));
    else { w = w * sigma_s; pdf = cavg(sigma_t * cexp(-tau)); }
    w = div_unguarded(w, pdf);
    MediumSample r; r.t = t_min; r.w = w; r.exited = exited;
    return r;
}
RL_DEV Col medium_transmittance(const MediumRecord& m, float tfar) {
    Col sigma_t = mkc(m.sigma_t[0], m.sigma_t[1], m.sigma_t[2]);
    Col tau = sigma_t * tfar;
    return cexp(-tau);
}
RL_DEV Col phase_eval(const MediumRecord& m, V3 w_i, V3 w_o) {
    if (m.phase == 0) return cval(div_rn(1.0f, kPi * 4.0f));
    float g = m.g;
    float tmp = 1.0f + g * g + 2.0f * g * dot(w_i, w_o);
    return cval(div_rn(kInvPi * 0.25f * (1.0f - g * g), tmp * sqrt_rn(tmp)));
}
RL_DEV float phase_pdf(const MediumRecord& m, V3 w_i, V3 w_o) { return cavg(phase_eval(m, w_i, w_o)); }
RL_DEV void phase_sample(const MediumRecord& m, V3 d_in, V2 u, V3* d, Col* weight, float* pdf) {
    if (m.phase == 0) { *d = sample_uniform_sphere(u); *weight = cone(); *pdf = div_rn(1.0f, kPi * 4.0f); return; }
    float g = m.g;
    float cos_t;
    if (fabsf(g) < 0.000001f) cos_t = 1.0f - 2.0f * u.x;
    else { float sq = div_rn(1.0f - g * g, 1.0f - g + 2.0f * g * u.x); cos_t = div_rn(1.0f + g * g - sq * sq, 2.0f * g); }
    float sin_t = sqrt_rn(rmax(1.0f - cos_t * cos_t, 0.0f));
    float sp, cp;
    m_sincosf(2.0f * kPi * u.y, &sp, &cp);
    V3 rev = d_in * -1.0f;
    *d = to_world(make_frame(rev), mk3(sin_t * cp, sin_t * sp, cos_t));
    *weight = cone();
    *pdf = phase_pdf(m, d_in, *d);
}

}
```

rustlight_amd/csrc/kernels/stages.hip.h:

```cpp
#pragma once

namespace rl {

RL_DEV V3 camera_direction(const DeviceScene& sc, float u, float v) {
    const float* m = sc.camera.sample_to_camera;
    float sx = div_rn(u, (float)sc.camera.width), sy = div_rn(v, (float)sc.camera.height), sz = 0.0f;
    float hx = ((m[0] * sx + m[4] * sy) + m[8] * sz) + m[12] * 1.0f;
    float hy = ((m[1] * sx + m[5] * sy) + m[9] * sz) + m[13] * 1.0f;
    float hz = ((m[2] * sx + m[6] * sy) + m[10] * sz) + m[14] * 1.0f;
    float hw = ((m[3] * sx + m[7] * sy) + m[11] * sz) + m[15] * 1.0f;
    float inv_w = div_rn(1.0f, hw);
    V3 near_p = mk3(hx * inv_w, hy * inv_w, hz * inv_w);
    V3 dl = normalize(near_p);
    const float* tw = sc.camera.to_world;
    return mk3(((tw[0] * dl.x + tw[4] * dl.y) + tw[8] * dl.z) + tw[12] * 0.0f,
               ((tw[1] * dl.x + tw[5] * dl.y) + tw[9] * dl.z) + tw[13] * 0.0f,
               ((tw[2] * dl.x + tw[6] * dl.y) + tw[10] * dl.z) + tw[14] * 0.0f);
}

RL_DEV Rng load_sample_state(const RenderConst& rc, unsigned s, unsigned p) {
    const ulonglong2* q = reinterpret_cast<const ulonglong2*>(rc.sample_states + 4 * ((size_t)s * rc.n_state_pixels + p));
    const ulonglong2 a = q[0], b = q[1];
    Rng r; r.s0 = a.x; r.s1 = a.y; r.s2 = b.x; r.s3 = b.y;
    return r;
}
RL_DEV void store_sample_state(const RenderConst& rc, unsigned s, unsigned p, const Rng& r) {
    ulonglong2* q = reinterpret_cast<ulonglong2*>(rc.sample_states + 4 * ((size_t)s * rc.n_state_pixels + p));
    q[0] = make_ulonglong2(r.s0, r.s1); q[1] = make_ulonglong2(r.s2, r.s3);
}

template <class PS>
RL_DEV void raygen_chain_slot(const RenderConst& rc, const DeviceScene& sc, PS& ps) {
    const unsigned flags = PU(U_FLAGS);
    const unsigned item = PU(U_ITEM);
    unsigned s = PU(U_SAMPLE), cursor = PU(U_CURSOR);
    unsigned bx, by, bw, bh;
    const unsigned b = rc.owned_blocks[item];
    block_geometry(rc, b, &bx, &by, &bw, &bh);
    const unsigned c_end = min(rc.cursor_end, bw * bh);
    Rng rng;
    if (flags & ST_FRESH) {
        cursor = rc.cursor_begin; s = 0;
        if (cursor >= c_end) { if (rc.queue) queue_push(rc, item); PU(U_FLAGS) = ST_FINISHED; return; }
        if (rc.cursor_begin == 0u) rng = rng_seed(rc.block_seeds[b], rc.seed_variant);
        else { const unsigned long long* q = rc.chain_states + 4 * (size_t)item; rng.s0 = q[0]; rng.s1 = q[1]; rng.s2 = q[2]; rng.s3 = q[3]; }
    } else {
        rng = load_rng(ps, Q_R0);
        s++;
        if (s == rc.spp) { s = 0; cursor++; }
        if (cursor == c_end) {
            unsigned long long* q = rc.chain_states + 4 * (size_t)item;
            q[0] = rng.s0; q[1] = rng.s1; q[2] = rng.s2; q[3] = rng.s3;
            if (rc.queue) queue_push(rc, item);
            PU(U_FLAGS) = ST_FINISHED;
            return;
        }
    }
    store_sample_state(rc, s, rc.block_item_base[item] + (cursor - rc.cursor_begin), rng);
    const unsigned px = bx + cursor % bw, py = by + cursor / bw;
    const float u = (float)px + rng_next_f32(rng);
    const float v = (float)py + rng_next_f32(rng);
    PU(U_SAMPLE) = s;
    PU(U_CURSOR) = cursor;
    const bool expand = (!rc.has_max || 1u < rc.max_depth);
    if (!expand) { store_rng(ps, Q_R0, rng); PU(U_FLAGS) = ST_REGEN; return; }
    store3(ps, F_DX, camera_direction(sc, u, v));
    if (sc.medium.enabled) PF(F_XI) = rng_next_f32(rng);
    store_rng(ps, Q_R0, rng);
    PU(U_DEPTH) = 1u;
    PU(U_FLAGS) = ST_RAY | (PREV_SENSOR << ST_PREV_SHIFT) | ST_PDF_SA;
}

template <bool DYNAMIC, class PS, class SMP = Rng, bool TAIL = false>
RL_DEV void raygen_slot(const RenderConst& rc, const DeviceScene& sc, PS& ps, unsigned& n_samples, unsigned& n_draws) {
    unsigned flags = PU(U_FLAGS);
    if (!(flags & ST_REGEN)) return;
    const bool fresh = (flags & ST_FRESH) != 0u;
    unsigned item = PU(U_ITEM), s = PU(U_SAMPLE), cursor = PU(U_CURSOR);
    Col acc = loadc(ps, F_AR);
    bool need_item = fresh;
    unsigned bx = 0, by = 0, bw = 1, bh = 1;
    if (rc.stream_mode == RL_STREAM_REFERENCE_ORDER && item < rc.n_items) block_geometry(rc, rc.owned_blocks[item], &bx, &by, &bw, &bh);
    constexpr bool STRAT = !std::is_same<SMP, Rng>::value;
    const bool per_pixel = STRAT || rc.stream_mode != RL_STREAM_REFERENCE_ORDER;
    const bool given = !STRAT && rc.stream_mode == kStreamGivenStates;
    unsigned split = per_pixel ? rc.split : 1u;
    unsigned pitem = split > 1u ? item / split : item;
    unsigned tail_begin = 0u, tail_lanes = 0u, tail_shift = 0u;
    constexpr bool tail = TAIL;
    if constexpr (TAIL) {
        const char __attribute__((address_space(4)))* kt = (const char __attribute__((address_space(4)))*)__builtin_amdgcn_kernarg_segment_ptr();
        asm volatile("" : "+s"(kt));
        const RenderConst& rt = *(const RenderConst*)kt;
        tail_begin = rt.tail_begin; tail_lanes = rt.tail_lanes; tail_shift = rt.tail_shift;
        const unsigned rel = item - tail_begin;
        const bool in_tail = rel < tail_lanes;
        split = in_tail ? 1u << tail_shift : 1u;
        pitem = in_tail ? tail_begin + (rel >> tail_shift) : (item < tail_begin ? item : item - (tail_lanes - (tail_lanes >> tail_shift)));
    }
    if (!fresh && split > 1u) {
        const Col L = loadc(ps, F_LR);
        float* dst = tail ? rc.sample_buf + 3 * ((size_t)s * (tail_lanes >> tail_shift) + (pitem - tail_begin)) : rc.sample_buf + 3 * ((size_t)s * (rc.n_items / split) + pitem);
        dst[0] = L.r; dst[1] = L.g; dst[2] = L.b;
        s += split;
        if (s >= rc.spp) need_item = true;
    } else if (!fresh) {
        acc = acc + loadc(ps, F_LR);
        s++;
        if (s == rc.spp) {
            unsigned pix = per_pixel ? rc.item_pixel[TAIL ? pitem : item] : (by + cursor / bw) * rc.W + (bx + cursor % bw);
            Col px = scale_unguarded(acc, rc.inv_spp);
            rc.out[3 * (size_t)pix] = px.r; rc.out[3 * (size_t)pix + 1] = px.g; rc.out[3 * (size_t)pix + 2] = px.b;
            acc = czero();
            s = 0;
            if (per_pixel) need_item = true;
            else { cursor++; if (cursor == bw * bh) need_item = true; }
        }
    }
    Rng rng;
    if (need_item) {
        if (!fresh) item = DYNAMIC ? atomicAdd(&rc.counters->next_item, 1u) : rc.n_items;
        if (item >= rc.n_items) {
            PU(U_FLAGS) = ST_FINISHED;
            if (DYNAMIC) atomicSub(&rc.counters->active, 1u);
            return;
        }
        cursor = 0;
        if (given) {
            const unsigned pi = split > 1u ? item / split : item;
            if (split > 1u) s = item % split;
            rng = load_sample_state(rc, s, pi);
        } else if (per_pixel) {
            const unsigned pi = TAIL ? pitem : (split > 1u ? item / split : item);
            Rng item_rng = rng_seed(rc.item_seed[pi], rc.seed_variant);
            if (split > 1u) { s = tail ? (item - tail_begin) & (split - 1u) : item % split; for (unsigned k = 0; k < s; k++) rng_next_u64(item_rng); }
            rng = rng_seed(rng_next_u64(item_rng), rc.seed_variant);
            store_rng(ps, Q_I0, item_rng);
        } else {
            unsigned b = rc.owned_blocks[item];
            block_geometry(rc, b, &bx, &by, &bw, &bh);
            rng = rng_seed(rc.block_seeds[b], rc.seed_variant);
        }
        PU(U_ITEM) = item;
    } else if (given) {
        rng = load_sample_state(rc, s, pitem);
    } else if (per_pixel) {
        Rng item_rng = load_rng(ps, Q_I0);
        for (unsigned k = 1; k < split; k++) rng_next_u64(item_rng);
        rng = rng_seed(rng_next_u64(item_rng), rc.seed_variant);
        store_rng(ps, Q_I0, item_rng);
    } else {
        rng = load_rng(ps, Q_R0);
    }
    unsigned px, py;
    if (per_pixel) { unsigned pix = rc.item_pixel[TAIL ? pitem : (split > 1u ? item / split : item)]; px = pix % rc.W; py = pix / rc.W; }
    else { px = bx + cursor % bw; py = by + cursor / bw; }
    SMP smp = SmpState<SMP>::begin(rc, rng, TAIL ? pitem : (split > 1u ? item / split : item), s);
    float u = (float)px + smp_next(smp);
    float v = (float)py + smp_next(smp);
    n_draws += 2;
    n_samples++;
    storec(ps, F_AR, acc);
    PU(U_SAMPLE) = s;
    PU(U_CURSOR) = cursor;
    const bool expand = (!rc.has_max || 1u < rc.max_depth);
    if (!expand) {
        storec(ps, F_LR, czero());
        smp_store(ps, smp);
        PU(U_FLAGS) = ST_REGEN;
        return;
    }
    const V3 d = camera_direction(sc, u, v);
    store3(ps, F_DX, d);
    if (sc.medium.enabled) { PF(F_XI) = smp_next(smp); n_draws++; }
    smp_store(ps, smp);
    PU(U_DEPTH) = 1u;
    PU(U_FLAGS) = ST_RAY | (PREV_SENSOR << ST_PREV_SHIFT) | ST_PDF_SA | smp_flag_bits(smp);
}

template <bool LDS_SCENE>
RL_DEV TravStackT<LDS_SCENE> open_scene(const DeviceScene& sc, const StackConf& stc, float4* smem, unsigned tid, SceneRecs* recs) {
    float4* after_scene = smem;
    if (LDS_SCENE) {
        stage_scene_lds(sc, smem, smem + lds_nodes_float4s(sc.n_nodes));
        recs->nodes = smem; recs->tris = smem + lds_nodes_float4s(sc.n_nodes);
        after_scene = smem + lds_scene_float4s(sc.n_nodes, sc.n_prims);
    } else {
        recs->nodes = streamed_nodes<TravStackT<false>>(sc);
        recs->tris = reinterpret_cast<const float4*>(sc.tris);
    }
    return make_stack<LDS_SCENE>(stc, reinterpret_cast<unsigned*>(after_scene), tid);
}

template <class PS, class Stack>
RL_DEV void extend_slot(const DeviceScene& sc, const SceneRecs& recs, const Stack& stack, PS& ps, int* dbg = nullptr) {
    const unsigned flags = PU(U_FLAGS);
    const bool primary = ((flags >> ST_PREV_SHIFT) & 3u) == PREV_SENSOR;
    V3 o = primary ? mk3(sc.camera.position[0], sc.camera.position[1], sc.camera.position[2]) : load3(ps, F_OX);
    V3 d = load3(ps, F_DX);
    Hit hit; hit.t = kF32Max; hit.u = 0.0f; hit.v = 0.0f; hit.prim = -1;
    traverse<false>(recs, Stack::kBvh4 ? sc.root4 : sc.root, mk3(sc.root_min[0], sc.root_min[1], sc.root_min[2]), mk3(sc.root_max[0], sc.root_max[1], sc.root_max[2]),
                    o, d, kEps, kF32Max, hit, stack);
    PF(F_T) = hit.t; PF(F_U) = hit.u; PF(F_V) = hit.v;
    PU(U_PRIM) = (unsigned)hit.prim;
    if (dbg) { dbg[0] = hit.steps; dbg[1] = hit.tris; }
}
template <class Stack>
RL_DEV bool shadow_visible(const DeviceScene& sc, const SceneRecs& recs, const Stack& stack, V3 p0, V3 p1) {
    V3 d = p1 - p0;
    float len = length(d);
    d = d / len;
    float tfar = len * (1.0f - 0.00001f);
    Hit hit; hit.t = tfar; hit.u = 0.0f; hit.v = 0.0f; hit.prim = -1;
    V3 inv_d = mk3(div_rn(1.0f, d.x), div_rn(1.0f, d.y), div_rn(1.0f, d.z));
    float te;
    if (!slab(mk3(sc.root_min[0], sc.root_min[1], sc.root_min[2]), mk3(sc.root_max[0], sc.root_max[1], sc.root_max[2]), p0, inv_d, kEps, tfar, &te))
        return false;
    return !traverse<true>(recs, Stack::kBvh4 ? sc.root4 : sc.root, mk3(sc.root_min[0], sc.root_min[1], sc.root_min[2]), mk3(sc.root_max[0], sc.root_max[1], sc.root_max[2]),
                           p0, d, kEps, tfar, hit, stack);
}
template <class Stack>
RL_DEV bool trace_closest(const DeviceScene& sc, const SceneRecs& recs, const Stack& stack, V3 o, V3 d, Hit& hit) {
    hit.t = kF32Max; hit.u = 0.0f; hit.v = 0.0f; hit.prim = -1;
    traverse<false>(recs, sc.root, mk3(sc.root_min[0], sc.root_min[1], sc.root_min[2]), mk3(sc.root_max[0], sc.root_max[1], sc.root_max[2]),
                    o, d, kEps, kF32Max, hit, stack);
    return hit.prim >= 0;
}
template <class Stack>
RL_DEV bool trace_none(const DeviceScene& sc, const SceneRecs& recs, const Stack& stack, V3 o, V3 d) {
    Hit hit; hit.t = kF32Max; hit.u = 0.0f; hit.v = 0.0f; hit.prim = -1;
    return !traverse<true>(recs, sc.root, mk3(sc.root_min[0], sc.root_min[1], sc.root_min[2]), mk3(sc.root_max[0], sc.root_max[1], sc.root_max[2]),
                           o, d, kEps, kF32Max, hit, stack);
}
template <class PS, class Stack>
RL_DEV void shadow_slot(const DeviceScene& sc, const SceneRecs& recs, const Stack& stack, PS& ps) {
    if (shadow_visible(sc, recs, stack, load3(ps, F_OX), load3(ps, F_SX))) storec(ps, F_LR, loadc(ps, F_LR) + loadc(ps, F_CR));
}

template <int MAT, bool MEDIUM, int LIGHTS = LIGHTS_ANY, bool DRAWS_ONLY = false, class SMP = Rng, class PS>
RL_DEV void shade_slot(const RenderConst& rc, const DeviceScene& sc, PS& ps, unsigned flags,
                       unsigned& n_vertices, unsigned& n_draws, unsigned& n_shadow, unsigned& n_ext) {
    n_ext += 1;
    const unsigned prev = (flags >> ST_PREV_SHIFT) & 3u;
    const unsigned depth = PU(U_DEPTH);
    const int prim = (int)PU(U_PRIM);
    const bool primary = prev == PREV_SENSOR;
    const V3 ro = primary ? mk3(sc.camera.position[0], sc.camera.position[1], sc.camera.position[2]) : load3(ps, F_OX);
    const V3 rd = load3(ps, F_DX);
    const float t_hit = PF(F_T);
    Col w_edge = (primary || DRAWS_ONLY) ? cone() : loadc(ps, F_WR);
    const float rr = (primary || DRAWS_ONLY) ? 1.0f : PF(F_RR);
    const float pdf_edge = (primary || DRAWS_ONLY) ? 1.0f : PF(F_PDF);
    Col beta = (primary || DRAWS_ONLY) ? cone() : loadc(ps, F_BR);
    Col L = (primary || DRAWS_ONLY) ? czero() : loadc(ps, F_LR);
    bool zeroed = (flags & ST_ZEROED) != 0u;
    const bool hit = prim >= 0;
    bool is_volume = false;
    V3 vpos = mk3(0.0f, 0.0f, 0.0f);
    if (MEDIUM) {
        MediumSample ms = medium_sample(sc.medium, hit ? t_hit : kF32Max, PF(F_XI));
        w_edge = w_edge * ms.w;
        is_volume = !hit || !ms.exited;
        if (is_volume) vpos = ro + rd * ms.t;
    }
    bool ended = false;
    unsigned new_flags = ST_REGEN;
    unsigned smp_bits = 0u;
    if (!MEDIUM && !hit) {
        ended = true;
        if constexpr (!DRAWS_ONLY) {
        Col contrib = (w_edge * rr) * (LIGHTS != LIGHTS_AREA_ONLY && sc.env_emitter >= 0 ? env_eval(sc, rd) : czero());
        const bool add_contrib = rc.has_min ? (depth - 1u) >= rc.min_depth : true;
        if (prev == PREV_SENSOR) {
            if (!is_zero(contrib) && add_contrib) L = L + contrib;
        } else if (!zeroed) {
            if (rc.strategy == RL_STRATEGY_EMITTER) contrib = czero();
            Col term = czero();
            if (!is_zero(contrib) && add_contrib) {
                float wmis = 1.0f;
                if (rc.strategy == RL_STRATEGY_ALL && (flags & ST_PDF_SA)) {
                    float p2 = (LIGHTS != LIGHTS_AREA_ONLY && (prev == PREV_SURFACE || prev == PREV_VOLUME)) ? env_direct_pdf(sc, rd) : 0.0f;
                    float total = (0.0f + pdf_edge) + p2;
                    wmis = div_rn(pdf_edge, total);
                }
                term = contrib * wmis;
            }
            L = L + beta * term;
        }
        storec(ps, F_LR, L);
        }
    }
    if (!ended) {
        const Col W = w_edge * rr;
        SurfacePoint sp;
        const Material* mat = nullptr;
        MeshRecord mr;
        if (!is_volume) {
            sp = fill_intersection(sc, prim, PF(F_U), PF(F_V), ro, rd, t_hit);
            mr = sc.meshes[sp.mesh];
            mat = &sc.materials[mr.material];
        }
        if constexpr (!DRAWS_ONLY) {
        Col emit = czero();
        if (!is_volume && (mr.flags & MESH_IS_LIGHT) && dot(sp.n_s, -rd) >= 0.0f) emit = mesh_emit<LIGHTS>(sc, mr, sp.has_uv, sp.uv);
        Col contrib = W * emit;
        const unsigned cur = depth - 1u;
        const bool add_contrib = rc.has_min ? cur >= rc.min_depth : true;
        if (prev == PREV_SENSOR) {
            if (!is_zero(contrib) && add_contrib) L = L + contrib;
        } else if (!zeroed) {
            if (rc.strategy == RL_STRATEGY_EMITTER) contrib = czero();
            Col term = czero();
            if (!is_zero(contrib) && add_contrib) {
                float wmis = 1.0f;
                if (rc.strategy == RL_STRATEGY_ALL && (flags & ST_PDF_SA)) {
                    float p2 = 0.0f;
                    if (!is_volume && (mr.flags & MESH_IS_LIGHT) && (prev == PREV_SURFACE || prev == PREV_VOLUME))
                        p2 = light_direct_pdf<LIGHTS>(sc, mr, sc.tris[prim].tri, ro, sp.p, sp.n_g, rd, false, mk3(0.0f, 0.0f, 0.0f));
                    float total = (0.0f + pdf_edge) + p2;
                    wmis = div_rn(pdf_edge, total);
                }
                term = contrib * wmis;
            }
            L = L + beta * term;
        }
        beta = beta * W;
        if (rc.single_scattering && !is_volume) zeroed = true;
        }

        const unsigned gen = depth + 1u;
        const bool expand = (rc.has_max ? gen < rc.max_depth : true) && gen < kDepthCap;
        if (expand) {
            n_vertices += 1;
            SMP rng = SmpState<SMP>::load(rc, ps, flags);
            Col thr = primary ? cone() : loadc(ps, F_TR);
            const V3 vp = is_volume ? vpos : sp.p;
            const V3 d_in = -rd;
            V2 s2 = smp_next2d(rng);
            n_draws += 2;
            bool has_edge = false;
            bool sampled = false;
            Col sw = czero(); V3 sd_world = mk3(0.0f, 0.0f, 0.0f); float spdf = 0.0f; int spdf_kind = PDF_SOLID_ANGLE;
            if (is_volume) {
                phase_sample(sc.medium, d_in, s2, &sd_world, &sw, &spdf);
                sampled = true;
            } else {
                BsdfSample bs;
                if (bsdf_sample<MAT>(sc, *mat, sp.has_uv, sp.uv, sp.wi, s2, &bs)) {
                    sampled = true;
                    sw = bs.weight; spdf = bs.pdf; spdf_kind = bs.pdf_kind;
                    sd_world = to_world(sp.frame, bs.d);
                }
            }
            float rr_new = 1.0f;
            if (sampled) {
                thr = thr * sw;
                if (!is_zero(thr)) {
                    const bool do_rr = rc.has_rr ? rc.rr_depth <= gen : true;
                    bool alive = true;
                    if (do_rr) {
                        float q = rmin(channel_max(thr), 0.95f);
                        float x = smp_next(rng);
                        n_draws++;
                        if (q < x) alive = false; else rr_new = div_rn(1.0f, q);
                    }
                    if (alive) {
                        thr = scale_unguarded(thr, rr_new);
                        has_edge = true;
                        if (MEDIUM) { PF(F_XI) = smp_next(rng); n_draws++; }
                    }
                }
            }
            const bool use_light = rc.strategy != RL_STRATEGY_BSDF;
            const bool smooth = !is_volume && mat->smooth;
            bool shadow = false;
            if (DRAWS_ONLY) {
                if constexpr (std::is_same<SMP, Rng>::value) if (use_light && !smooth) { rng_next_u64(rng); rng_next_u64(rng); rng_next_u64(rng); rng_next_u64(rng); n_draws += 4; }
            } else
            if (use_light && !smooth) {
                float a = smp_next(rng);
                float b = smp_next(rng);
                V2 c = smp_next2d(rng);
                n_draws += 4;
                n_shadow += 1;
                LightSample ls = sample_light<LIGHTS>(sc, vp, !is_volume, is_volume ? mk3(0.0f, 0.0f, 0.0f) : sp.n_s, a, b, c);
                if (ls.pdf != 0.0f) {
                    Col wl;
                    float p_dir;
                    if (is_volume) { wl = phase_eval(sc.medium, d_in, ls.d); p_dir = phase_pdf(sc.medium, d_in, ls.d); }
                    else {
                        V3 wo = to_local(sp.frame, ls.d);
                        wl = bsdf_eval<MAT>(sc, *mat, sp.has_uv, sp.uv, sp.wi, wo, false);
                        V3 wo_edge = wo;
                        if (LIGHTS != LIGHTS_AREA_ONLY && ls.kind == EMITTER_ENV) { V3 ed = ls.p - vp; ed = ed / length(ed); wo_edge = to_local(sp.frame, ed); }
                        p_dir = bsdf_pdf<MAT>(sc, *mat, sp.has_uv, sp.uv, sp.wi, wo_edge, false);
                    }
                    if (MEDIUM) {
                        V3 dd = ls.p - vp;
                        wl = wl * medium_transmittance(sc.medium, dot(dd, ls.d));
                    }
                    Col c_l = ls.weight * wl * 1.0f;
                    const bool add_l = rc.has_min ? (gen - 1u) >= rc.min_depth : true;
                    if (!zeroed) {
                        Col term = czero();
                        if (!is_zero(c_l) && add_l) {
                            float wmis = 1.0f;
                            if (rc.strategy == RL_STRATEGY_ALL && (LIGHTS == LIGHTS_AREA_ONLY || ls.pdf_kind == PDF_SOLID_ANGLE)) {
                                float total = (0.0f + p_dir) + ls.pdf;
                                wmis = div_rn(ls.pdf, total);
                            }
                            term = c_l * wmis;
                        }
                        Col pending = beta * term;
                        if (!is_zero(pending)) {
                            shadow = true;
                            store3(ps, F_SX, ls.p);
                            storec(ps, F_CR, pending);
                        }
                    }
                }
            }
            smp_store(ps, rng);
            smp_bits = smp_flag_bits(rng);
            store3(ps, F_OX, vp);
            new_flags = shadow ? ST_SHADOW : 0u;
            if (has_edge) {
                store3(ps, F_DX, sd_world);
                storec(ps, F_TR, thr);
                if constexpr (!DRAWS_ONLY) {
                    storec(ps, F_WR, sw);
                    PF(F_RR) = rr_new;
                    PF(F_PDF) = spdf;
                }
                PU(U_DEPTH) = gen;
                const unsigned kind = is_volume ? PREV_VOLUME : (smooth ? PREV_SURFACE_SMOOTH : PREV_SURFACE);
                new_flags |= ST_RAY | (kind << ST_PREV_SHIFT) | (spdf_kind == PDF_SOLID_ANGLE ? ST_PDF_SA : 0u) | (zeroed ? ST_ZEROED : 0u);
            } else new_flags |= ST_REGEN;
        }
        if constexpr (!DRAWS_ONLY) {
            storec(ps, F_BR, beta);
            storec(ps, F_LR, L);
        }
    }
    PU(U_FLAGS) = new_flags | smp_bits;
}

}
```

rustlight_amd/csrc/kernels/wavefront.hip:

```cpp
#include <hip/hip_runtime.h>

#include <algorithm>
#include <atomic>
#include <chrono>
#include <cmath>
#include <cstdio>
#include <cstring>
#include <memory>
#include <string>
#include <thread>
#include <vector>

#include "common.hip.h"
#include "rngjump.h"
#include "../host/hip_buffer.h"
#include "../host/photontree.h"
#include "../host/beamtree.h"
#include "phototree.h"
#include "../host/scene.h"
#include "wavefront.h"
#include "knobs.h"
#include "light.hip.h"

namespace rl {

__global__ void k_seed_pixels(RenderConst rc) {
    unsigned j = blockIdx.x * blockDim.x + threadIdx.x;
    if (j >= rc.n_owned) return;
    unsigned b = rc.owned_blocks[j];
    unsigned bx, by, bw, bh;
    block_geometry(rc, b, &bx, &by, &bw, &bh);
    Rng rng = rng_seed(rc.block_seeds[b], rc.seed_variant);
    unsigned base = rc.block_item_base[j];
    for (unsigned iy = 0; iy < bh; iy++)
        for (unsigned ix = 0; ix < bw; ix++) {
            unsigned k = base + iy * bw + ix;
            rc.item_seed[k] = rng_next_u64(rng);
            rc.item_pixel[k] = (by + iy) * rc.W + (bx + ix);
        }
}

__global__ void k_chunk_pixels(RenderConst rc) {
    unsigned j = blockIdx.x * blockDim.x + threadIdx.x;
    if (j >= rc.n_owned) return;
    unsigned bx, by, bw, bh;
    block_geometry(rc, rc.owned_blocks[j], &bx, &by, &bw, &bh);
    const unsigned c_end = min(rc.cursor_end, bw * bh), base = rc.block_item_base[j];
    for (unsigned c = rc.cursor_begin; c < c_end; c++) rc.item_pixel[base + (c - rc.cursor_begin)] = (by + c / bw) * rc.W + (bx + c % bw);
}

__global__ void k_init(RenderConst rc, Pool pool) {
    unsigned slot = blockIdx.x * blockDim.x + threadIdx.x;
    if (slot >= pool.P) return;
    PoolState ps{pool, slot};
    PU(U_ITEM) = slot;
    PU(U_CURSOR) = 0u;
    PU(U_SAMPLE) = 0u;
    PU(U_DEPTH) = 0u;
    PU(U_PRIM) = 0xffffffffu;
    PU(U_FLAGS) = slot < rc.n_items ? (ST_REGEN | ST_FRESH) : ST_FINISHED;
    storec(ps, F_AR, czero());
    storec(ps, F_LR, czero());
}

__global__ void __launch_bounds__(256) k_raygen(RenderConst rc, DeviceScene sc, Pool pool) {
    unsigned n_samples = 0, n_draws = 0;
    for (unsigned slot = blockIdx.x * blockDim.x + threadIdx.x; slot < pool.P; slot += gridDim.x * blockDim.x) {
        PoolState ps{pool, slot};
        raygen_slot<true>(rc, sc, ps, n_samples, n_draws);
    }
    { const int which[2] = {STAT_SAMPLES, STAT_DRAWS}; const unsigned vals[2] = {n_samples, n_draws}; block_stats<2>(rc.partials, which, vals); }
}

__global__ void __launch_bounds__(256) k_fold_samples(RenderConst rc) {
    const bool tail = rc.tail_lanes != 0u;
    const unsigned n_pix = tail ? rc.tail_pixels : rc.n_items / rc.split;
    const unsigned p = blockIdx.x * blockDim.x + threadIdx.x;
    if (p >= n_pix) return;
    Col acc = czero();
    for (unsigned s = 0; s < rc.spp; s++) {
        const float* src = rc.sample_buf + 3 * ((size_t)s * n_pix + p);
        acc = acc + mkc(src[0], src[1], src[2]);
    }
    const Col px = scale_unguarded(acc, rc.inv_spp);
    const size_t pix = rc.item_pixel[tail ? rc.tail_begin + p : p];
    rc.out[3 * pix] = px.r; rc.out[3 * pix + 1] = px.g; rc.out[3 * pix + 2] = px.b;
}

#ifdef RL_TRAV_STATS
__device__ unsigned long long g_trav_stats[8];
#endif
template <bool LDS_SCENE, bool SHADOW>
RL_DEV void trace_kernel_body(const DeviceScene& sc, const Pool& pool, const StackConf& stc) {
    extern __shared__ __attribute__((aligned(16))) float4 smem[];
    float4* after_scene = LDS_SCENE ? smem + lds_scene_float4s(sc.n_nodes, sc.n_prims) : smem;
    unsigned* list = reinterpret_cast<unsigned*>(after_scene);
    unsigned slot = blockIdx.x * blockDim.x + threadIdx.x;
    const TravStackT<LDS_SCENE> stack = make_stack<LDS_SCENE>(stc, list + 272, slot);
    const unsigned flags = slot < pool.P ? pool.u[(size_t)U_FLAGS * pool.P + slot] : 0u;
    const unsigned n_live = block_compact((flags & (SHADOW ? ST_SHADOW : ST_RAY)) != 0u, slot, list);
    if (n_live == 0u) return;
    SceneRecs recs;
    if (LDS_SCENE) {
        stage_scene_lds(sc, smem, smem + lds_nodes_float4s(sc.n_nodes));
        recs.nodes = smem; recs.tris = smem + lds_nodes_float4s(sc.n_nodes);
    } else {
        recs.nodes = streamed_nodes<TravStackT<false>>(sc);
        recs.tris = reinterpret_cast<const float4*>(sc.tris);
    }
#ifdef RL_TRAV_STATS
    int dbg[2] = {-1, 0};
    if (threadIdx.x < n_live) {
        PoolState ps{pool, list[threadIdx.x]};
        if (SHADOW) shadow_slot(sc, recs, stack, ps);
        else extend_slot(sc, recs, stack, ps, dbg);
    }
    if (!SHADOW) {
        int mx = dbg[0];
        for (int off = 32; off > 0; off >>= 1) mx = max(mx, __shfl_xor(mx, off, 64));
        if (dbg[0] >= 0) { atomicAdd(&g_trav_stats[0], 1ull); atomicAdd(&g_trav_stats[1], (unsigned long long)dbg[0]); atomicAdd(&g_trav_stats[2], (unsigned long long)dbg[1]); if (dbg[0] == 0) atomicAdd(&g_trav_stats[5], 1ull); }
        if ((threadIdx.x & 63u) == 0u && mx >= 0) { atomicAdd(&g_trav_stats[3], 64ull * (unsigned long long)mx); atomicAdd(&g_trav_stats[4], 1ull); }
    }
#else
    if (threadIdx.x < n_live) {
        PoolState ps{pool, list[threadIdx.x]};
        if (SHADOW) shadow_slot(sc, recs, stack, ps);
        else extend_slot(sc, recs, stack, ps);
    }
#endif
}

template <bool LDS_SCENE>
__global__ void __launch_bounds__(256) k_extend(RenderConst rc, DeviceScene sc, Pool pool, StackConf stc) { trace_kernel_body<LDS_SCENE, false>(sc, pool, stc); }
template <bool LDS_SCENE>
__global__ void __launch_bounds__(256) k_shadow(RenderConst rc, DeviceScene sc, Pool pool, StackConf stc) { trace_kernel_body<LDS_SCENE, true>(sc, pool, stc); }

__global__ void __launch_bounds__(256) k_trace_batch(DeviceScene sc, StackConf stc, unsigned n, const float* o, const float* d, float* t_out, float* u_out,
                                                     float* v_out, int* mesh_out, int* tri_out) {
    extern __shared__ __attribute__((aligned(16))) float4 smem[];
    SceneRecs recs;
    recs.nodes = streamed_nodes<TravStackT<false>>(sc);
    recs.tris = reinterpret_cast<const float4*>(sc.tris);
    unsigned i = blockIdx.x * blockDim.x + threadIdx.x;
    const TravStack stack = make_stack(stc, reinterpret_cast<unsigned*>(smem), i);
    if (i >= n) return;
    V3 ro = mk3(o[3 * i], o[3 * i + 1], o[3 * i + 2]), rd = mk3(d[3 * i], d[3 * i + 1], d[3 * i + 2]);
    Hit hit;
    trace_closest(sc, recs, stack, ro, rd, hit);
    t_out[i] = hit.t; u_out[i] = hit.u; v_out[i] = hit.v;
    if (hit.prim >= 0) { mesh_out[i] = sc.tris[hit.prim].mesh; tri_out[i] = sc.tris[hit.prim].tri; }
    else { mesh_out[i] = -1; tri_out[i] = -1; }
}

__global__ void __launch_bounds__(256) k_trace_batch_two_level(DeviceScene sc, StackConf stc, unsigned n, const float* o, const float* d, float* t_out, float* u_out,
                                                               float* v_out, int* mesh_out, int* tri_out, int* steps_out, int any_hit) {
    extern __shared__ __attribute__((aligned(16))) float4 smem[];
    SceneRecs recs;
    recs.nodes = reinterpret_cast<const float4*>(sc.nodes2);
    recs.tris = reinterpret_cast<const float4*>(sc.tris);
    unsigned i = blockIdx.x * blockDim.x + threadIdx.x;
    const TravStack2 stack(make_stack(stc, reinterpret_cast<unsigned*>(smem), i));
    if (i >= n) return;
    V3 ro = mk3(o[3 * i], o[3 * i + 1], o[3 * i + 2]), rd = mk3(d[3 * i], d[3 * i + 1], d[3 * i + 2]);
    Hit hit; hit.t = kF32Max; hit.u = 0.0f; hit.v = 0.0f; hit.prim = -1;
    if (any_hit) {
        hit.t = t_out[i];
        const bool f = traverse<true>(recs, sc.root, mk3(sc.root_min[0], sc.root_min[1], sc.root_min[2]), mk3(sc.root_max[0], sc.root_max[1], sc.root_max[2]), ro, rd, kEps, hit.t, hit, stack);
        t_out[i] = f ? 1.0f : 0.0f; steps_out[i] = hit.steps;
        return;
    }
    trace_closest(sc, recs, stack, ro, rd, hit);
    t_out[i] = hit.t; u_out[i] = hit.u; v_out[i] = hit.v; steps_out[i] = hit.steps;
    if (hit.prim >= 0) { mesh_out[i] = sc.tris[hit.prim].mesh; tri_out[i] = sc.tris[hit.prim].tri; }
    else { mesh_out[i] = -1; tri_out[i] = -1; }
}

__global__ void __launch_bounds__(256) k_visible_batch(DeviceScene sc, StackConf stc, unsigned n, const float* p0a, const float* p1a, unsigned char* out) {
    extern __shared__ __attribute__((aligned(16))) float4 smem[];
    SceneRecs recs;
    recs.nodes = streamed_nodes<TravStackT<false>>(sc);
    recs.tris = reinterpret_cast<const float4*>(sc.tris);
    unsigned i = blockIdx.x * blockDim.x + threadIdx.x;
    const TravStack stack = make_stack(stc, reinterpret_cast<unsigned*>(smem), i);
    if (i >= n) return;
    V3 p0 = mk3(p0a[3 * i], p0a[3 * i + 1], p0a[3 * i + 2]), p1 = mk3(p1a[3 * i], p1a[3 * i + 1], p1a[3 * i + 2]);
    out[i] = shadow_visible(sc, recs, stack, p0, p1) ? 1 : 0;
}

__global__ void k_numerics_probe(unsigned n, const float* a, const float* b, float* out_div, float* out_sqrt, float* out_mad, float* out_sin,
                                 float* out_cos, float* out_exp, float* out_log, float* out_pow, float* out_acos, float* out_atan2) {
    unsigned i = blockIdx.x * blockDim.x + threadIdx.x;
    if (i >= n) return;
    out_div[i] = div_rn(a[i], b[i]);
    out_sqrt[i] = sqrt_rn(fabsf(a[i]));
    out_mad[i] = a[i] * b[i] + a[i];
    out_sin[i] = dm::sinf_det(a[i]);
    out_cos[i] = dm::cosf_det(a[i]);
    out_exp[i] = dm::expf_det(a[i]);
    out_log[i] = dm::logf_det(fabsf(a[i]));
    out_pow[i] = dm::powf_det(fabsf(a[i]), b[i]);
    out_acos[i] = dm::acosf_det(a[i] * 0.15f);
    out_atan2[i] = dm::atan2f_det(a[i], b[i]);
}

__global__ void k_math_sweep(int fn, int swap, unsigned first_bits, unsigned stride, unsigned period, unsigned n, const float* b, float b_const, float* out) {
    unsigned i = blockIdx.x * blockDim.x + threadIdx.x;
    if (i >= n) return;
    const float g = __uint_as_float(first_bits + (period ? i % period : i) * stride);
    const float c = b ? b[i] : b_const;
    const float x = swap ? c : g, y = swap ? g : c;
    float r;
    switch (fn) {
        case RL_MATH_SINF: r = dm::sinf_det(x); break;
        case RL_MATH_COSF: r = dm::cosf_det(x); break;
        case RL_MATH_EXPF: r = dm::expf_det(x); break;
        case RL_MATH_LOGF: r = dm::logf_det(x); break;
        case RL_MATH_POWF: r = dm::powf_det(x, y); break;
        case RL_MATH_ACOSF: r = dm::acosf_det(x); break;
        case RL_MATH_ATAN2F: r = dm::atan2f_det(x, y); break;
        case RL_MATH_ASINF: r = dm::asinf_det(x); break;
        case RL_MATH_SQRT_RN: r = sqrt_rn(x); break;
        case RL_MATH_DIV_RN: r = div_rn(x, y); break;
        default: r = x * y + x; break;
    }
    out[i] = r;
}

}

using namespace rl;

static thread_local std::string g_last_error;
void rl_set_error(const std::string& s) { g_last_error = s; }
extern "C" const char* rl_last_error(void) { return g_last_error.c_str(); }

struct rl_context {
    int device = 0;
    hipStream_t stream = nullptr;
    DeviceScene ds{};
    std::vector<HipBuffer<unsigned char>> allocs;
    uint32_t width = 0, height = 0;
    bool single_bsdf = true;
    int bsdf_type = 0;
    bool lds_scene = false;
    bool area_lights_only = false;
    bool has_directional = false;
    size_t scene_lds_bytes = 0;
    size_t lds_limit = 64 * 1024;
    HipBuffer<float> pool_f; HipBuffer<unsigned> pool_u; HipBuffer<unsigned long long> pool_q;
    HipBuffer<unsigned> d_owned, d_item_base;
    HipBuffer<unsigned long long> d_block_seeds, d_item_seed;
    HipBuffer<unsigned> d_item_pixel;
    HipBuffer<float> d_out;
    HipBuffer<Counters> d_counters;
    HipBuffer<Counters, Mem::Pinned> h_counters;
    HipBuffer<unsigned long long> d_partials;
    HipBuffer<int> d_overflow;
    HipBuffer<int> d_overflow2;
    HipBuffer<float> d_sample_buf;
    HipBuffer<unsigned long long> d_sample_states;
    HipBuffer<unsigned long long> d_chain_states;
    HipBuffer<unsigned> d_trk_off;
    HipBuffer<ulonglong2> d_trk_st;
    HipBuffer<unsigned> d_trivial;
    uint64_t trivial_key = ~0ull;
    std::vector<unsigned char> heavy_blocks;
    uint64_t heavy_key = ~0ull;
    HipBuffer<unsigned long long> d_spec_stats;
    std::vector<hipEvent_t> events;
    static constexpr int kEvalStreams = 4;
    hipStream_t stream2 = nullptr; hipStream_t eval_streams[kEvalStreams] = {};
    HipBuffer<unsigned> d_queue;
    hipEvent_t ev_chain_done = nullptr;
    HipBuffer<unsigned, Mem::Mapped> h_flags;
    HipBuffer<unsigned, Mem::Pinned> h_list;
    unsigned queue_seq = 0;
    BvhBuild bvh_dump;
    Knobs knobs;
    LightConst light_cam{};
    std::vector<RectLight> rect_lights;
    int rect_lights_rc = RL_OK;
    std::string rect_lights_err;
};

template <typename T>
static int upload(rl_context* ctx, const std::vector<T>& v, const T** out) {
    *out = nullptr;
    ctx->allocs.emplace_back();
    HipBuffer<unsigned char>& b = ctx->allocs.back();
    int rcode;
    if ((rcode = b.ensure(std::max<size_t>(v.size(), 1) * sizeof(T))) != RL_OK) return rcode;
    if (!v.empty()) HIP_OK(hipMemcpy(b.get(), v.data(), v.size() * sizeof(T), hipMemcpyHostToDevice));
    *out = reinterpret_cast<const T*>(b.get());
    return RL_OK;
}

static int ensure_two_level(rl_context* ctx) {
    if (ctx->ds.nodes2) return RL_OK;
    std::vector<BvhNode2> n2;
    two_level_nodes(ctx->bvh_dump, &n2);
    return upload(ctx, n2, &ctx->ds.nodes2);
}

extern "C" int rl_device_count(int* count) {
    if (!count) return RL_ERR_INVALID_ARGUMENT;
    int n = 0;
    if (hipGetDeviceCount(&n) != hipSuccess || n <= 0) { *count = 0; return RL_ERR_NO_DEVICE; }
    *count = n;
    return RL_OK;
}

extern "C" int rl_context_create(const rl_scene* scene, int device, rl_context** out) {
    if (!scene || !out) return RL_ERR_INVALID_ARGUMENT;
    if (!scene->has_camera) return RL_ERR_INVALID_ARGUMENT;
    if (!scene->emitters_built) return RL_ERR_NOT_BUILT;
    int n_dev = 0;
    hipError_t e = hipGetDeviceCount(&n_dev);
    if (e != hipSuccess || n_dev <= 0) {
        rl_set_error("no HIP device available (hipGetDeviceCount); the MI355X path has no CPU fallback");
        return RL_ERR_NO_DEVICE;
    }
    if (device < 0 || device >= n_dev) { rl_set_error("device ordinal out of range"); return RL_ERR_NO_DEVICE; }
    HIP_OK(hipSetDevice(device));
    rl_context* ctx = new rl_context();
    ctx->device = device;
    ctx->width = scene->width; ctx->height = scene->height;
    ctx->knobs.from_environment();
    int rc = RL_OK;
    do {
        {
            int prio_least = 0, prio_greatest = 0;
            if (hipDeviceGetStreamPriorityRange(&prio_least, &prio_greatest) != hipSuccess) { (void)hipGetLastError(); prio_least = prio_greatest = 0; }
            if (hipStreamCreateWithPriority(&ctx->stream, hipStreamNonBlocking, prio_greatest) != hipSuccess) { rl_set_error("hipStreamCreate failed"); rc = RL_ERR_HIP; break; }
            if (hipStreamCreateWithPriority(&ctx->stream2, hipStreamNonBlocking, prio_least) != hipSuccess) { (void)hipGetLastError(); ctx->stream2 = nullptr; }
            if (ctx->stream2 && hipEventCreateWithFlags(&ctx->ev_chain_done, hipEventDisableTiming) != hipSuccess) { (void)hipGetLastError(); hipStreamDestroy(ctx->stream2); ctx->stream2 = nullptr; }
            if (ctx->stream2) {
                ctx->eval_streams[0] = ctx->stream2;
                for (int k = 1; k < rl_context::kEvalStreams; k++)
                    if (hipStreamCreateWithPriority(&ctx->eval_streams[k], hipStreamNonBlocking, prio_least) != hipSuccess) { (void)hipGetLastError(); ctx->eval_streams[k] = ctx->stream2; }
            }
        }
        BvhBuild& bvh = ctx->bvh_dump;
        build_bvh(*scene, &bvh);
        FlatScene flat;
        flatten_scene(*scene, &flat);
        DeviceScene& ds = ctx->ds;
        if ((rc = upload(ctx, bvh.nodes, &ds.nodes)) != RL_OK) break;
        if ((rc = upload(ctx, bvh.tris, &ds.tris)) != RL_OK) break;
        for (int i = 0; i < 3; i++) { ds.root_min[i] = bvh.root_min[i]; ds.root_max[i] = bvh.root_max[i]; }
        ds.root = bvh.root;
        ds.n_nodes = (uint32_t)bvh.nodes.size();
        ds.n_prims = (uint32_t)bvh.tris.size();
        ds.stack_depth = bvh.stack_depth;
        ds.nodes4 = nullptr; ds.root4 = RL_CHILD_NONE; ds.stack_depth4 = 0;
        ds.nodes_t = nullptr; ds.root_t = RL_CHILD_NONE;
        ds.nodes2 = nullptr;
        if ((rc = upload(ctx, flat.tri_indices, &ds.tri_indices)) != RL_OK) break;
        if ((rc = upload(ctx, flat.positions, &ds.positions)) != RL_OK) break;
        if ((rc = upload(ctx, flat.normals, &ds.normals)) != RL_OK) break;
        if ((rc = upload(ctx, flat.uvs, &ds.uvs)) != RL_OK) break;
        for (MeshRecord& mr : flat.meshes) mr.ats_base = 0xffffffffu;
        std::vector<int32_t> ats_light_mesh;
        if (scene->ats_root >= 0) {
            for (size_t e = 0; e < scene->emitters.size(); e++) flat.meshes[scene->emitters[e].mesh].ats_base = scene->ats_emitter_base[e];
            for (int32_t e : scene->ats_light_emitter) ats_light_mesh.push_back(scene->emitters[e].mesh);
        }
        if ((rc = upload(ctx, flat.meshes, &ds.meshes)) != RL_OK) break;
        ds.ats_root = scene->ats_root;
        if ((rc = upload(ctx, scene->ats_nodes, &ds.ats_nodes)) != RL_OK) break;
        if ((rc = upload(ctx, ats_light_mesh, &ds.ats_light_mesh)) != RL_OK) break;
        if ((rc = upload(ctx, scene->ats_light_prim, &ds.ats_light_prim)) != RL_OK) break;
        if ((rc = upload(ctx, scene->ats_leaf_of, &ds.ats_leaf_of)) != RL_OK) break;
        if ((rc = upload(ctx, flat.materials, &ds.materials)) != RL_OK) break;
        if ((rc = upload(ctx, flat.bitmaps, &ds.bitmaps)) != RL_OK) break;
        if ((rc = upload(ctx, flat.bitmap_texels, &ds.bitmap_texels)) != RL_OK) break;
        if ((rc = upload(ctx, scene->emitters, &ds.emitters)) != RL_OK) break;
        if ((rc = upload(ctx, scene->emitters_cdf, &ds.emitters_cdf)) != RL_OK) break;
        ds.n_emitters = (uint32_t)scene->emitters.size();
        ds.env_emitter = -1;
        for (size_t e = 0; e < scene->emitters.size(); e++)
            if (scene->emitters[e].kind == EMITTER_ENV) {
                ds.env_emitter = (int32_t)e;
                for (int k = 0; k < 3; k++) ds.env_color[k] = scene->emitters[e].c[k];
                ds.env_pdf = (1.0f / (3.14159265358979323846f * 4.0f)) * (scene->emitters_cdf[e + 1] - scene->emitters_cdf[e]);
                ds.env_sel_pdf = scene->emitters_cdf[e + 1] - scene->emitters_cdf[e];
            }
        ds.env_w = ds.env_h = 0;
        if (ds.env_emitter >= 0 && scene->env_map.w) {
            ds.env_w = scene->env_map.w; ds.env_h = scene->env_map.h;
            ds.env_marg_func_int = scene->env_marg_func_int;
            if ((rc = upload(ctx, scene->env_map.rgb, &ds.env_texels)) != RL_OK) break;
            if ((rc = upload(ctx, scene->env_cond_cdf, &ds.env_cond_cdf)) != RL_OK) break;
            if ((rc = upload(ctx, scene->env_cond_func, &ds.env_cond_func)) != RL_OK) break;
            if ((rc = upload(ctx, scene->env_marg_cdf, &ds.env_marg_cdf)) != RL_OK) break;
        }
        if (ds.env_emitter >= 0 && scene->medium.enabled) { rl_set_error("an environment emitter cannot be combined with a medium (paths/edge.rs:94)"); rc = RL_ERR_UNSUPPORTED; break; }
        if ((rc = upload(ctx, flat.mesh_cdf, &ds.mesh_cdf)) != RL_OK) break;
        ds.n_meshes = (uint32_t)flat.meshes.size();
        scene->sample_to_camera.to_cols(ds.camera.sample_to_camera);
        scene->to_world.to_cols(ds.camera.to_world);
        ds.camera.position[0] = scene->cam_pos.x; ds.camera.position[1] = scene->cam_pos.y; ds.camera.position[2] = scene->cam_pos.z;
        ds.camera.width = scene->width; ds.camera.height = scene->height;
        {
            scene->camera_to_sample.to_cols(ctx->light_cam.camera_to_sample);
            scene->to_local.to_cols(ctx->light_cam.to_local);
            const Vec3 p0 = scene->sample_to_camera.xform_point({0.0f, 0.0f, 0.0f}), p1 = scene->sample_to_camera.xform_point({1.0f, 1.0f, 0.0f});
            const float zmin = std::fmin(p0.z, p1.z), zmax = std::fmax(p0.z, p1.z);
            ctx->light_cam.rect_min[0] = std::fmin(p0.x, p1.x) / zmin; ctx->light_cam.rect_min[1] = std::fmin(p0.y, p1.y) / zmin;
            ctx->light_cam.rect_max[0] = std::fmax(p0.x, p1.x) / zmax; ctx->light_cam.rect_max[1] = std::fmax(p0.y, p1.y) / zmax;
        }
        ds.medium = scene->medium;
        {
            const char* why = "";
            if ((ctx->rect_lights_rc = build_rect_lights(*scene, &ctx->rect_lights, &why)) != RL_OK) ctx->rect_lights_err = why;
        }
        ctx->area_lights_only = scene->ats_root < 0 && !ctx->knobs.has(K_GENERIC_LIGHTS);
        for (const EmitterRecord& e : scene->emitters) if (e.kind != EMITTER_MESH) ctx->area_lights_only = false;
        for (const EmitterRecord& e : scene->emitters) if (e.kind == EMITTER_DIRECTIONAL) ctx->has_directional = true;
        for (const HostMesh& hm : scene->meshes) if (hm.is_light && hm.emission_type != RL_EMISSION_COLOR) ctx->area_lights_only = false;
        ctx->single_bsdf = true;
        ctx->bsdf_type = flat.materials.empty() ? 0 : flat.materials[0].type;
        for (const Material& m : flat.materials) if (m.type != ctx->bsdf_type) ctx->single_bsdf = false;
        ctx->scene_lds_bytes = (size_t)16 * lds_scene_float4s(ds.n_nodes, ds.n_prims);
        ctx->lds_scene = ctx->scene_lds_bytes <= 48 * 1024 && ds.stack_depth <= (uint32_t)kLdsStackLevels;
        {
            int lds_limit = 64 * 1024;
            if (hipDeviceGetAttribute(&lds_limit, hipDeviceAttributeMaxSharedMemoryPerBlock, device) != hipSuccess) { (void)hipGetLastError(); lds_limit = 64 * 1024; }
            ctx->lds_limit = (size_t)std::max(lds_limit, 16 * 1024);
            const size_t worst = ctx->scene_lds_bytes + std::max<size_t>(272 * sizeof(unsigned), kFusedColdBytes) + (size_t)2 * kLdsStackLevels * 256 * sizeof(int);
            if (worst > (size_t)lds_limit) ctx->lds_scene = false;
        }
        if (ctx->knobs.has(K_FORCE_STREAMING)) ctx->lds_scene = false;
        if (!ctx->lds_scene) {
            Bvh4Build b4;
            build_bvh4(bvh, &b4);
            if ((rc = upload(ctx, b4.nodes, &ds.nodes4)) != RL_OK) break;
            ds.root4 = b4.root; ds.stack_depth4 = b4.stack_depth;
            std::vector<BvhNode> blocks;
            int32_t root_t = RL_CHILD_NONE;
            treelet_blocks(bvh, &blocks, &root_t);
            if ((rc = upload(ctx, blocks, &ds.nodes_t)) != RL_OK) break;
            ds.root_t = root_t;
        }
        if (ctx->d_counters.ensure(1) != RL_OK) { rl_set_error("hipMalloc counters"); rc = RL_ERR_HIP; break; }
        if (ctx->h_counters.ensure(1) != RL_OK) { rl_set_error("hipHostMalloc counters"); rc = RL_ERR_HIP; break; }
    } while (0);
    if (rc != RL_OK) { rl_context_destroy(ctx); return rc; }
    *out = ctx;
    return RL_OK;
}

extern "C" void rl_context_destroy(rl_context* ctx) {
    if (!ctx) return;
    hipSetDevice(ctx->device);
    for (hipEvent_t ev : ctx->events) hipEventDestroy(ev);
    if (ctx->ev_chain_done) hipEventDestroy(ctx->ev_chain_done);
    for (int k = 1; k < rl_context::kEvalStreams; k++) if (ctx->eval_streams[k] && ctx->eval_streams[k] != ctx->stream2) hipStreamDestroy(ctx->eval_streams[k]);
    if (ctx->stream2) hipStreamDestroy(ctx->stream2);
    if (ctx->stream) hipStreamDestroy(ctx->stream);
    delete ctx;
}

#ifndef RL_LDS_LEVELS_STREAMING
#define RL_LDS_LEVELS_STREAMING 6
#endif
static constexpr int kLdsStackLevelsStreaming = RL_LDS_LEVELS_STREAMING;
static int lds_levels_of(const rl_context* ctx) { return std::min<int>((int)ctx->ds.stack_depth, ctx->lds_scene ? kLdsStackLevels : kLdsStackLevelsStreaming); }
static size_t traversal_lds_bytes(const rl_context* ctx, bool lds_scene, unsigned block, bool with_list, int lds_levels = -1) {
    size_t stack = (size_t)2 * (lds_levels >= 0 ? lds_levels : lds_levels_of(ctx)) * block * sizeof(int);
    return (lds_scene ? ctx->scene_lds_bytes : 0) + (with_list ? 272 * sizeof(unsigned) : 0) + stack;
}
static int stack_conf(rl_context* ctx, size_t n_threads, StackConf* out, bool second = false, int lds_levels = -1) {
    HipBuffer<int>& d_overflow = second ? ctx->d_overflow2 : ctx->d_overflow;
    out->lds_levels = lds_levels >= 0 ? std::min(lds_levels, lds_levels_of(ctx)) : lds_levels_of(ctx);
    out->pre_group = 0;
    out->overflow = nullptr;
    out->overflow_stride = n_threads;
    int extra = (int)std::max(ctx->ds.stack_depth, ctx->ds.stack_depth4) - out->lds_levels;
    if (extra > 0) {
        const int rcode = d_overflow.ensure((size_t)2 * extra * n_threads);
        if (rcode != RL_OK) return rcode;
        out->overflow = d_overflow.get();
    }
    return RL_OK;
}

struct BlockRect { unsigned x, y, w, h; };
static BlockRect block_rect(size_t b, size_t nby, uint32_t W, uint32_t H) {
    const unsigned x = (unsigned)(b / nby) * 16u, y = (unsigned)(b % nby) * 16u;
    return {x, y, std::min(16u, W - x), std::min(16u, H - y)};
}

struct TrivialInput { uint32_t W, H; bool medium, empty; float root_min[3], root_max[3]; CameraRecord camera; };
static TrivialInput trivial_input(const rl_context* ctx) {
    TrivialInput in{};
    in.W = ctx->width; in.H = ctx->height; in.medium = ctx->ds.medium.enabled != 0; in.empty = ctx->ds.root == RL_CHILD_NONE || ctx->ds.n_prims == 0;
    for (int k = 0; k < 3; k++) { in.root_min[k] = ctx->ds.root_min[k]; in.root_max[k] = ctx->ds.root_max[k]; }
    in.camera = ctx->ds.camera;
    return in;
}
static void trivial_pixel_masks(const TrivialInput& ti, const rl_path_params* params, const std::vector<unsigned>& owned, size_t nby, bool no_shortcut, std::vector<unsigned>* out, bool blocks_only = false) {
    const uint32_t W = ti.W, H = ti.H;
    out->assign(owned.size() * 8, 0u);
    const bool expand = !params->has_max_depth || 1u < params->max_depth;
    auto all_of_block = [&](size_t j, unsigned npx) { for (unsigned c = 0; c < npx; c++) (*out)[j * 8 + (c >> 5)] |= 1u << (c & 31u); };
    if (!expand) {
        for (size_t j = 0; j < owned.size(); j++) { const BlockRect r = block_rect(owned[j], nby, W, H); all_of_block(j, r.w * r.h); }
        return;
    }
    if (ti.medium || no_shortcut) return;
    const bool empty = ti.empty;
    double lo[3], hi[3];
    for (int k = 0; k < 3; k++) {
        lo[k] = ti.root_min[k]; hi[k] = ti.root_max[k];
        if (!empty && !(std::isfinite(lo[k]) && std::isfinite(hi[k]) && lo[k] <= hi[k])) return;
        const double grow = 1e-3 * (hi[k] - lo[k]) + 1e-4 * std::max(1.0, std::max(std::fabs(lo[k]), std::fabs(hi[k])));
        lo[k] -= grow; hi[k] += grow;
    }
    const float* m = ti.camera.sample_to_camera; const float* tw = ti.camera.to_world;
    const double cam[3] = {ti.camera.position[0], ti.camera.position[1], ti.camera.position[2]};
    auto ray_dir = [&](double u, double v, double* d) -> bool {
        const double sx = u / (double)W, sy = v / (double)H;
        const double hx = m[0] * sx + m[4] * sy + m[12], hy = m[1] * sx + m[5] * sy + m[13], hz = m[2] * sx + m[6] * sy + m[14], hw = m[3] * sx + m[7] * sy + m[15];
        if (!(std::fabs(hw) > 1e-12) || !std::isfinite(hx + hy + hz + hw)) return false;
        const double nx = hx / hw, ny = hy / hw, nz = hz / hw;
        d[0] = tw[0] * nx + tw[4] * ny + tw[8] * nz; d[1] = tw[1] * nx + tw[5] * ny + tw[9] * nz; d[2] = tw[2] * nx + tw[6] * ny + tw[10] * nz;
        d[3] = hw;
        const double len = std::sqrt(d[0] * d[0] + d[1] * d[1] + d[2] * d[2]);
        if (!(len > 1e-30) || !std::isfinite(len)) return false;
        d[0] /= len; d[1] /= len; d[2] /= len;
        return true;
    };
    auto misses = [&](double u0, double v0, double u1, double v1) -> bool {
        if (empty) return true;
        double d[4][4];
        const double us[4] = {u0, u1, u1, u0}, vs[4] = {v0, v0, v1, v1};
        for (int k = 0; k < 4; k++) if (!ray_dir(us[k], vs[k], d[k])) return false;
        for (int k = 1; k < 4; k++) if ((d[k][3] > 0) != (d[0][3] > 0)) return false;
        for (int k = 0; k < 4; k++) {
            const double* a = d[k]; const double* b = d[(k + 1) & 3]; const double* o = d[(k + 2) & 3];
            double n[3] = {a[1] * b[2] - a[2] * b[1], a[2] * b[0] - a[0] * b[2], a[0] * b[1] - a[1] * b[0]};
            const double nl = std::sqrt(n[0] * n[0] + n[1] * n[1] + n[2] * n[2]);
            if (!(nl > 1e-14)) return false;
            double inside = (n[0] * o[0] + n[1] * o[1] + n[2] * o[2]) / nl;
            if (!(std::fabs(inside) > 1e-9)) return false;
            const double sgn = inside > 0 ? 1.0 : -1.0;
            bool all_out = true;
            for (int cbit = 0; cbit < 8 && all_out; cbit++) {
                const double p[3] = {((cbit & 1) ? hi[0] : lo[0]) - cam[0], ((cbit & 2) ? hi[1] : lo[1]) - cam[1], ((cbit & 4) ? hi[2] : lo[2]) - cam[2]};
                const double pl = std::sqrt(p[0] * p[0] + p[1] * p[1] + p[2] * p[2]);
                const double s = sgn * (n[0] * p[0] + n[1] * p[1] + n[2] * p[2]) / nl;
                if (!(s < -1e-7 * pl - 1e-12)) all_out = false;
            }
            if (all_out) return true;
        }
        return false;
    };
    for (size_t j = 0; j < owned.size(); j++) {
        const BlockRect r = block_rect(owned[j], nby, W, H);
        const unsigned bx = r.x, by = r.y, bw = r.w, bh = r.h;
        if (misses(bx - 0.25, by - 0.25, bx + bw + 0.25, by + bh + 0.25)) { all_of_block(j, bw * bh); continue; }
        if (blocks_only) continue;
        for (unsigned c = 0; c < bw * bh; c++) {
            const double x = bx + c % bw, y = by + c / bw;
            if (misses(x - 0.25, y - 0.25, x + 1.25, y + 1.25)) (*out)[j * 8 + (c >> 5)] |= 1u << (c & 31u);
        }
    }
}

extern "C" int rl_debug_trivial_pixels(const rl_scene* scene, int has_max_depth, uint32_t max_depth, uint8_t* out) {
    if (!scene || !out || !scene->has_camera) return RL_ERR_INVALID_ARGUMENT;
    BvhBuild bvh;
    build_bvh(*scene, &bvh);
    TrivialInput ti{};
    ti.W = scene->width; ti.H = scene->height; ti.medium = scene->medium.enabled != 0; ti.empty = bvh.root == RL_CHILD_NONE || bvh.tris.empty();
    for (int k = 0; k < 3; k++) { ti.root_min[k] = bvh.root_min[k]; ti.root_max[k] = bvh.root_max[k]; }
    scene->sample_to_camera.to_cols(ti.camera.sample_to_camera);
    scene->to_world.to_cols(ti.camera.to_world);
    ti.camera.position[0] = scene->cam_pos.x; ti.camera.position[1] = scene->cam_pos.y; ti.camera.position[2] = scene->cam_pos.z;
    ti.camera.width = scene->width; ti.camera.height = scene->height;
    rl_path_params pp{};
    pp.has_max_depth = has_max_depth; pp.max_depth = max_depth;
    const size_t nbx = (ti.W + 15) / 16, nby = (ti.H + 15) / 16;
    std::vector<unsigned> owned(nbx * nby), masks;
    for (size_t b = 0; b < owned.size(); b++) owned[b] = (unsigned)b;
    trivial_pixel_masks(ti, &pp, owned, nby, false, &masks);
    std::memset(out, 0, (size_t)ti.W * ti.H);
    for (size_t b = 0; b < owned.size(); b++) {
        const BlockRect r = block_rect(b, nby, ti.W, ti.H);
        for (unsigned c = 0; c < r.w * r.h; c++) if ((masks[b * 8 + (c >> 5)] >> (c & 31u)) & 1u) out[(size_t)(r.y + c / r.w) * ti.W + r.x + c % r.w] = 1;
    }
    return RL_OK;
}

static int check_frame(const rl_context* ctx, uint32_t spp, const uint64_t* block_seeds, size_t n_blocks, const float* out_rgb) {
    if (!ctx || !block_seeds || !out_rgb) return RL_ERR_INVALID_ARGUMENT;
    if (n_blocks != (size_t)((ctx->width + 15) / 16) * ((ctx->height + 15) / 16)) { rl_set_error("n_blocks does not match the image size"); return RL_ERR_INVALID_ARGUMENT; }
    if (spp == 0) { rl_set_error("spp must be > 0 (assert_ne!(scene.nb_samples, 0), mod.rs:410)"); return RL_ERR_INVALID_ARGUMENT; }
    return RL_OK;
}
template <typename Params>
static int check_frame(const rl_context* ctx, const Params* params, const uint64_t* block_seeds, size_t n_blocks, const float* out_rgb) {
    return params ? check_frame(ctx, params->spp, block_seeds, n_blocks, out_rgb) : RL_ERR_INVALID_ARGUMENT;
}
static int check_streams(int32_t stream_mode, uint32_t spp, uint32_t numerics, uint32_t shard_index, uint32_t shard_count) {
    if (stream_mode < RL_STREAM_REFERENCE_ORDER || stream_mode > RL_STREAM_STRATIFIED) { rl_set_error("stream_mode must be 0 (reference order), 1 (per sample) or 2 (stratified)"); return RL_ERR_INVALID_ARGUMENT; }
    if (stream_mode == RL_STREAM_STRATIFIED && spp > (1u << 30)) { rl_set_error("the stratified sampler takes at most 2^30 spp"); return RL_ERR_INVALID_ARGUMENT; }
    if (numerics > RL_NUMERICS_FAST) { rl_set_error("numerics must be 0 (exact) or 1 (fast)"); return RL_ERR_INVALID_ARGUMENT; }
    if (shard_index >= (shard_count ? shard_count : 1)) return RL_ERR_INVALID_ARGUMENT;
    return RL_OK;
}

namespace {

struct RenderFrame {
    rl_context* const ctx;
    const uint64_t* const block_seeds;
    const size_t n_blocks;
    float* const out_rgb;
    const int out_is_device;
    const hipStream_t st;
    rl_render_stats* const stats;
    const Knobs knobs;
    const uint32_t W, H;
    const size_t nby;
    const uint32_t shard_count;
    const std::chrono::steady_clock::time_point t_start;
    const bool timing;
    int cus = 256;
    std::vector<unsigned> owned, item_base;
    unsigned n_pixels = 0;
    float* d_out = nullptr;
    size_t n_rows = 0;
    unsigned long long totals[STAT_COUNT] = {};

    RenderFrame(rl_context* c, const uint64_t* seeds, size_t nb, float* out, int out_dev, void* stream_arg, rl_render_stats* s, uint32_t shard_index, uint32_t n_shards)
        : ctx(c), block_seeds(seeds), n_blocks(nb), out_rgb(out), out_is_device(out_dev), st(stream_arg ? (hipStream_t)stream_arg : c->stream), stats(s),
          knobs(c->knobs), W(c->width), H(c->height), nby((c->height + 15) / 16), shard_count(n_shards ? n_shards : 1), t_start(std::chrono::steady_clock::now()),
          timing(s != nullptr && !knobs.has(K_NO_EVENTS)) {
        for (size_t b = 0; b < n_blocks; b++) {
            if (b % shard_count != shard_index) continue;
            const BlockRect r = block_rect(b, nby, W, H);
            owned.push_back((unsigned)b);
            item_base.push_back(n_pixels);
            n_pixels += r.w * r.h;
        }
        hipDeviceGetAttribute(&cus, hipDeviceAttributeMultiprocessorCount, ctx->device);
    }

    size_t max_state_bytes() const { return knobs.has(K_STATE_BUDGET_MB) ? std::max<size_t>(1, (size_t)knobs.i(K_STATE_BUDGET_MB, 0)) << 20 : (size_t)24 << 30; }

    int alloc_tables() {
        int rcode;
        if ((rcode = ctx->d_owned.ensure(owned.size())) != RL_OK || (rcode = ctx->d_item_base.ensure(owned.size())) != RL_OK ||
            (rcode = ctx->d_block_seeds.ensure(n_blocks)) != RL_OK) return rcode;
        return RL_OK;
    }
    int alloc_output(size_t rows) {
        d_out = out_rgb;
        if (!out_is_device) {
            const int rcode = ctx->d_out.ensure((size_t)3 * W * H);
            if (rcode != RL_OK) return rcode;
            d_out = ctx->d_out.get();
        }
        n_rows = rows;
        return ctx->d_partials.ensure(n_rows * STAT_COUNT);
    }
    int upload(bool with_item_base, bool zero_image) {
        HIP_OK(hipMemcpyAsync(ctx->d_owned.get(), owned.data(), owned.size() * sizeof(unsigned), hipMemcpyHostToDevice, st));
        if (with_item_base) HIP_OK(hipMemcpyAsync(ctx->d_item_base.get(), item_base.data(), item_base.size() * sizeof(unsigned), hipMemcpyHostToDevice, st));
        HIP_OK(hipMemcpyAsync(ctx->d_block_seeds.get(), block_seeds, n_blocks * sizeof(uint64_t), hipMemcpyHostToDevice, st));
        if (zero_image) HIP_OK(hipMemsetAsync(d_out, 0, (size_t)3 * W * H * sizeof(float), st));
        return RL_OK;
    }
    int zero_rows() {
        HIP_OK(hipMemsetAsync(ctx->d_partials.get(), 0, n_rows * STAT_COUNT * sizeof(unsigned long long), st));
        return RL_OK;
    }
    RenderConst render_const(uint32_t spp, int32_t stream_mode, int32_t seed_variant) const {
        RenderConst rc{};
        rc.spp = spp;
        rc.stream_mode = stream_mode; rc.seed_variant = seed_variant;
        rc.inv_spp = 1.0f / (float)spp;
        rc.W = W; rc.H = H; rc.nby = (unsigned)nby;
        rc.owned_blocks = ctx->d_owned.get(); rc.block_item_base = ctx->d_item_base.get(); rc.n_owned = (unsigned)owned.size();
        rc.block_seeds = ctx->d_block_seeds.get();
        rc.item_seed = ctx->d_item_seed.get(); rc.item_pixel = ctx->d_item_pixel.get();
        rc.out = d_out;
        rc.counters = ctx->d_counters.get();
        rc.partials = ctx->d_partials.get();
        return rc;
    }
    int grow_events(size_t n) {
        if (timing) while (ctx->events.size() < n) { hipEvent_t ev; HIP_OK(hipEventCreate(&ev)); ctx->events.push_back(ev); }
        return RL_OK;
    }
    int download() {
        if (!out_is_device) HIP_OK(hipMemcpyAsync(out_rgb, d_out, (size_t)3 * W * H * sizeof(float), hipMemcpyDeviceToHost, st));
        std::vector<unsigned long long> partials(n_rows * STAT_COUNT);
        HIP_OK(hipMemcpyAsync(partials.data(), ctx->d_partials.get(), partials.size() * sizeof(unsigned long long), hipMemcpyDeviceToHost, st));
        HIP_OK(hipStreamSynchronize(st));
        HIP_OK(hipGetLastError());
        for (size_t r = 0; r < n_rows; r++) for (int k = 0; k < STAT_COUNT; k++) totals[k] += partials[r * STAT_COUNT + k];
        if (stats) {
            std::memset(stats, 0, sizeof(*stats));
            stats->camera_samples = totals[STAT_SAMPLES]; stats->vertices = totals[STAT_VERTICES]; stats->extension_rays = totals[STAT_EXT_RAYS];
            stats->shadow_rays = totals[STAT_SHADOW_RAYS]; stats->rng_draws = totals[STAT_DRAWS];
            stats->render_ms = std::chrono::duration<double, std::milli>(std::chrono::steady_clock::now() - t_start).count();
        }
        return RL_OK;
    }
};

struct LaneRun {
    std::vector<unsigned long long> words;
    EventPair ev;
    std::chrono::steady_clock::time_point t0;
};
template <class Launch>
int run_one_lane(hipStream_t st, bool timing, const rl_sampler* sampler, size_t n_counters, LaneRun* run, Launch&& launch) {
    int rcode;
    HipBuffer<unsigned long long> d_gen;
    if ((rcode = d_gen.ensure(4 + n_counters)) != RL_OK || (rcode = run->ev.open(timing)) != RL_OK) return rcode;
    run->words.assign(4 + n_counters, 0ull);
    for (int i = 0; i < 4; i++) run->words[i] = sampler->s[i];
    HIP_OK(hipMemcpyAsync(d_gen.get(), run->words.data(), run->words.size() * sizeof(unsigned long long), hipMemcpyHostToDevice, st));
    run->ev.begin(st);
    run->t0 = std::chrono::steady_clock::now();
    launch(d_gen.get());
    run->ev.end(st);
    HIP_OK(hipMemcpyAsync(run->words.data(), d_gen.get(), run->words.size() * sizeof(unsigned long long), hipMemcpyDeviceToHost, st));
    HIP_OK(hipStreamSynchronize(st));
    HIP_OK(hipGetLastError());
    run->ev.add();
    return RL_OK;
}
}

#include "path_render.hip.h"

extern "C" int rl_render_path(rl_context* ctx, const rl_path_params* params, const uint64_t* block_seeds, size_t n_blocks, float* out_rgb,
                              int out_is_device, void* stream_arg, rl_render_stats* stats) {
    int rcode;
    if ((rcode = check_frame(ctx, params, block_seeds, n_blocks, out_rgb)) != RL_OK) return rcode;
    if (params->strategy < 0 || params->strategy > 2) return RL_ERR_INVALID_ARGUMENT;
// ... 629 lines not shown
```

Measured before the change: 5497.

## Precompute light-triangle records and per-item pixel coordinates for shading

At context creation, each emissive mesh triangle gets a packed 64-byte record holding its corners, geometric normal and inverse area. Light sampling can then read four float4s instead of chasing index and position buffers and recomputing the normal and area. The change also stores per-item (x, y) pixel coordinates so raygen avoids a div/mod, and skips the pdf_sel scaling when it equals one. The cost is extra device memory, a setup kernel, and more template variants; the knob can turn the records off.

```diff
diff --git a/rustlight_amd/csrc/device_types.h b/rustlight_amd/csrc/device_types.h
--- a/rustlight_amd/csrc/device_types.h
+++ b/rustlight_amd/csrc/device_types.h
@@ -85,6 +85,15 @@
 };
 enum { MESH_HAS_NORMALS = 1, MESH_HAS_UV = 2, MESH_IS_LIGHT = 4 };
 
+struct alignas(16) LightTriRecord {
+    float v0[3]; float n0;
+    float v1[3]; float n1;
+    float v2[3]; float n2;
+    float inv_area;
+    float pad[3];
+};
+static_assert(sizeof(LightTriRecord) == 64, "LightTriRecord must be 64 bytes");
+
 enum { EMITTER_MESH = 0, EMITTER_ENV = 1, EMITTER_POINT = 2, EMITTER_DIRECTIONAL = 3 };
 struct EmitterRecord {
     int32_t kind;
@@ -93,7 +102,8 @@
     float c[3];
     float center[3];
     float radius;
-    float pad[4];
+    uint32_t light_tri_base;
+    float pad[3];
 };
 static_assert(sizeof(EmitterRecord) == 64, "EmitterRecord must be 64 bytes");
 
@@ -163,6 +173,8 @@
     uint32_t n_meshes;
     CameraRecord camera;
     MediumRecord medium;
+    const LightTriRecord* light_tris;
+    const uint32_t* light_tri_base;
 };
 
 }
diff --git a/rustlight_amd/csrc/kernels/fused_body.inc.h b/rustlight_amd/csrc/kernels/fused_body.inc.h
--- a/rustlight_amd/csrc/kernels/fused_body.inc.h
+++ b/rustlight_amd/csrc/kernels/fused_body.inc.h
@@ -97,7 +97,8 @@
 #else
         constexpr bool kTail = false;
 #endif
-        if (PU(U_FLAGS) & ST_REGEN) raygen_slot<true, decltype(ps), SMP, kTail>(rc, sc, ps, n_samples, n_draws);
+        constexpr bool kSceneRecs = RL_NUMERICS_ID == 0;
+        if (PU(U_FLAGS) & ST_REGEN) raygen_slot<true, decltype(ps), SMP, kTail, !qmode>(rc, sc, ps, n_samples, n_draws);
         RL_T1(0, c0)
 #ifdef RL_STAGE_TIMERS
         const bool c1 = PU(U_FLAGS) & ST_RAY;
@@ -105,7 +106,7 @@
         if (PU(U_FLAGS) & ST_RAY) {
             extend_slot(sc, recs, stack, ps);
             RL_T1(1, c1)
-            shade_slot<MAT, MEDIUM, LIGHTS, false, SMP>(rc, sc, ps, PU(U_FLAGS), n_vertices, n_draws, n_shadow, n_ext);
+            shade_slot<MAT, MEDIUM, LIGHTS, false, SMP, kSceneRecs>(rc, sc, ps, PU(U_FLAGS), n_vertices, n_draws, n_shadow, n_ext);
         }
         RL_T1(2, c1)
 #ifdef RL_STAGE_TIMERS
diff --git a/rustlight_amd/csrc/kernels/knobs.h b/rustlight_amd/csrc/kernels/knobs.h
--- a/rustlight_amd/csrc/kernels/knobs.h
+++ b/rustlight_amd/csrc/kernels/knobs.h
@@ -32,6 +32,7 @@
     K_PLANE_TREE_DEVICE,
     K_PLANE_TREE_GROUP_PLANES,
     K_PPLANE_TREE_DEVICE,
+    K_NO_SCENE_RECORDS,
     K_FORCE_STREAMING,
     K_GENERIC_LIGHTS,
     K_COUNT
@@ -47,7 +48,7 @@
             "fused_dynamic", "fused_tail_blocks", "fused_tail_split", "fused_tail_no_buffer_test", "eval_split", "eval_min", "eval_div", "no_events", "queue_debug",
             "spec_group", "spec_sub", "spec_cap", "spec_probe", "spec_lead", "spec_lead_max", "spec_lead_var", "spec_extra", "spec_dense", "spec_dense_frac",
             "spec_probe_every", "spec_ks", "spec_ke", "spec_serial_ratio", "spec_no_trivial", "spec_lds_limit_test", "spec_stats", "spec_wave_times", "spec_lds_levels", "vpl_batch_paths", "photon_tree_group_photons",
-            "plane_generate_lanes", "plane_tree_device", "plane_tree_group_planes", "pplane_tree_device",
+            "plane_generate_lanes", "plane_tree_device", "plane_tree_group_planes", "pplane_tree_device", "no_scene_records",
             "force_streaming", "generic_lights"};
         return names[k];
     }
diff --git a/rustlight_amd/csrc/kernels/path_render.hip.h b/rustlight_amd/csrc/kernels/path_render.hip.h
--- a/rustlight_amd/csrc/kernels/path_render.hip.h
+++ b/rustlight_amd/csrc/kernels/path_render.hip.h
@@ -161,6 +161,7 @@
         if (per_sample || two_pass) {
             if (per_sample && (rcode = ctx->d_item_seed.ensure(n_item_pixels)) != RL_OK) return rcode;
             if ((rcode = ctx->d_item_pixel.ensure(n_item_pixels)) != RL_OK) return rcode;
+            if ((rcode = ctx->d_item_xy.ensure(n_item_pixels)) != RL_OK) return rcode;
         }
         if (two_pass) {
             if ((rcode = ctx->d_sample_states.ensure((size_t)max_chunk_pix * params->spp * 4)) != RL_OK) return rcode;
@@ -238,6 +239,7 @@
         rc.split = split; rc.sample_buf = ctx->d_sample_buf.get();
         rc.tail_begin = tail.begin; rc.tail_pixels = tail.pixels; rc.tail_shift = tail.shift; rc.tail_lanes = tail.pixels << tail.shift;
         rc.sample_states = ctx->d_sample_states.get(); rc.chain_states = ctx->d_chain_states.get();
+        rc.item_xy = (per_sample || two_pass) ? ctx->d_item_xy.get() : nullptr;
 
         lds_trav = traversal_lds_bytes(ctx, ctx->lds_scene, 256, true);
         if ((rcode = stack_conf(ctx, (size_t)((P + 255) / 256) * 256, &stc)) != RL_OK) return rcode;
@@ -250,15 +252,22 @@
         return grow_events(kEventsPerIter * (per_sample ? 8u : 32u));
     }
 
+    DeviceScene shading_scene() const {
+        DeviceScene ds = ctx->ds;
+        if (knobs.has(K_NO_SCENE_RECORDS) && knobs.i(K_NO_SCENE_RECORDS, 0) != 0) { ds.light_tris = nullptr; ds.light_tri_base = nullptr; }
+        return ds;
+    }
+
     void launch_fused(const RenderConst& rcl, dim3 grid, hipStream_t on, const StackConf* stcl = nullptr) const {
         const int mat = ctx->single_bsdf ? ctx->bsdf_type : -1;
         const StackConf& s = stcl ? *stcl : stc;
+        const DeviceScene ds = shading_scene();
         if (strat)
-            (ctx->lds_scene ? launch_fused_strat_lds : launch_fused_strat_stream)(medium, ctx->area_lights_only, grid, dim3(256), lds_fused, on, rcl, ctx->ds, s);
+            (ctx->lds_scene ? launch_fused_strat_lds : launch_fused_strat_stream)(medium, ctx->area_lights_only, grid, dim3(256), lds_fused, on, rcl, ds, s);
         else if (rcl.queue_mode != 0u)
-            (ctx->lds_scene ? launch_fusedq_lds : launch_fusedq_stream)(mat, medium, ctx->area_lights_only, grid, dim3(256), lds_fused, on, rcl, ctx->ds, s);
+            (ctx->lds_scene ? launch_fusedq_lds : launch_fusedq_stream)(mat, medium, ctx->area_lights_only, grid, dim3(256), lds_fused, on, rcl, ds, s);
         else
-            (ctx->lds_scene ? (fast_math ? launch_fused_lds_fast : launch_fused_lds) : (fast_math ? launch_fused_stream_fast : launch_fused_stream))(mat, medium, ctx->area_lights_only, grid, dim3(256), lds_fused, on, rcl, ctx->ds, s);
+            (ctx->lds_scene ? (fast_math ? launch_fused_lds_fast : launch_fused_lds) : (fast_math ? launch_fused_stream_fast : launch_fused_stream))(mat, medium, ctx->area_lights_only, grid, dim3(256), lds_fused, on, rcl, ds, s);
     }
 
     void drain() const {
@@ -542,7 +551,7 @@
         const dim3 grid_sort((P + 1023) / 1024);
         const dim3 grid_persistent(std::min<unsigned>((P + 255) / 256, (unsigned)cus * 8u));
         const unsigned poll_every = per_sample ? 8u : 32u;
-        const DeviceScene& ds = ctx->ds;
+        const DeviceScene ds = shading_scene();
         unsigned in_batch = 0;
         auto flush_events = [&](unsigned count) -> int {
             for (unsigned i = 0; i < count; i++)
diff --git a/rustlight_amd/csrc/kernels/pathstate.hip.h b/rustlight_amd/csrc/kernels/pathstate.hip.h
--- a/rustlight_amd/csrc/kernels/pathstate.hip.h
+++ b/rustlight_amd/csrc/kernels/pathstate.hip.h
@@ -125,6 +125,7 @@
     unsigned q_n;
     unsigned* q_ctr;
     unsigned tail_begin, tail_lanes, tail_shift, tail_pixels;
+    uint2* item_xy;
 };
 RL_DEV void queue_workgroup_started(const RenderConst& rc) {
     if (atomicAdd(rc.queue, 1u) + 1u == rc.chain_grid) __hip_atomic_store(rc.started_flag, rc.queue_seq, __ATOMIC_RELEASE, __HIP_MEMORY_SCOPE_SYSTEM);
diff --git a/rustlight_amd/csrc/kernels/shade.hip b/rustlight_amd/csrc/kernels/shade.hip
--- a/rustlight_amd/csrc/kernels/shade.hip
+++ b/rustlight_amd/csrc/kernels/shade.hip
@@ -9,7 +9,7 @@
     unsigned n_vertices = 0, n_draws = 0, n_shadow = 0, n_ext = 0;
     PoolState ps{pool, slot};
     unsigned flags = slot < pool.P ? PU(U_FLAGS) : 0u;
-    if (flags & ST_RAY) shade_slot<MAT, MEDIUM>(rc, sc, ps, flags, n_vertices, n_draws, n_shadow, n_ext);
+    if (flags & ST_RAY) shade_slot<MAT, MEDIUM, LIGHTS_ANY, false, Rng, true>(rc, sc, ps, flags, n_vertices, n_draws, n_shadow, n_ext);
     {
         const int which[4] = {STAT_VERTICES, STAT_DRAWS, STAT_SHADOW_RAYS, STAT_EXT_RAYS};
         const unsigned vals[4] = {n_vertices, n_draws, n_shadow, n_ext};
diff --git a/rustlight_amd/csrc/kernels/shade_sorted_body.inc.h b/rustlight_amd/csrc/kernels/shade_sorted_body.inc.h
--- a/rustlight_amd/csrc/kernels/shade_sorted_body.inc.h
+++ b/rustlight_amd/csrc/kernels/shade_sorted_body.inc.h
@@ -41,7 +41,7 @@
 #define RL_SHADE_BIN(B)                                                                                       \
     { const unsigned n = bin_begin[(B) + 1] - bin_begin[B];                                                   \
       for (unsigned i = threadIdx.x; i < n; i += blockDim.x) { PoolState pb{pool, s_list[bin_begin[B] + i]};    \
-          shade_slot<B, MEDIUM, LIGHTS_ANY, false, SMP>(rc, sc, pb, pb.u(U_FLAGS), n_vertices, n_draws, n_shadow, n_ext); } }
+          shade_slot<B, MEDIUM, LIGHTS_ANY, false, SMP, true>(rc, sc, pb, pb.u(U_FLAGS), n_vertices, n_draws, n_shadow, n_ext); } }
     RL_SHADE_BIN(0) RL_SHADE_BIN(1) RL_SHADE_BIN(2) RL_SHADE_BIN(3) RL_SHADE_BIN(4)
 #undef RL_SHADE_BIN
     {
diff --git a/rustlight_amd/csrc/kernels/shading.hip.h b/rustlight_amd/csrc/kernels/shading.hip.h
--- a/rustlight_amd/csrc/kernels/shading.hip.h
+++ b/rustlight_amd/csrc/kernels/shading.hip.h
@@ -477,17 +477,36 @@
     return false;
 }
 
-template <int LIGHTS = LIGHTS_ANY>
-RL_DEV void mesh_sample_triangle(const DeviceScene& sc, const MeshRecord& mr, unsigned int prim, float pdf_area, V3 p, V2 uv, LightSample* ls) {
+RL_DEV void light_tri_corners(const DeviceScene& sc, unsigned int i0, unsigned int i1, unsigned int i2, V3* v0, V3* v1, V3* v2) {
+    *v0 = mk3(sc.positions[3 * i0], sc.positions[3 * i0 + 1], sc.positions[3 * i0 + 2]);
+    *v1 = mk3(sc.positions[3 * i1], sc.positions[3 * i1 + 1], sc.positions[3 * i1 + 2]);
+    *v2 = mk3(sc.positions[3 * i2], sc.positions[3 * i2 + 1], sc.positions[3 * i2 + 2]);
+}
+RL_DEV V3 light_tri_normal(V3 v0, V3 v1, V3 v2) { return normalize(cross(v2 - v0, v1 - v0)); }
+RL_DEV float light_tri_inv_area(V3 v0, V3 v1, V3 v2) { return div_rn(1.0f, length(cross(v1 - v0, v2 - v0)) * 0.5f); }
+template <int LIGHTS = LIGHTS_ANY, bool RECS = false>
+RL_DEV void mesh_sample_triangle(const DeviceScene& sc, const MeshRecord& mr, unsigned int rec_base, unsigned int prim, float pdf_area, V3 p, V2 uv, LightSample* ls) {
     unsigned int gtri = mr.tri_base + prim;
-    unsigned int i0 = sc.tri_indices[3 * gtri], i1 = sc.tri_indices[3 * gtri + 1], i2 = sc.tri_indices[3 * gtri + 2];
-    V3 v0 = mk3(sc.positions[3 * i0], sc.positions[3 * i0 + 1], sc.positions[3 * i0 + 2]);
-    V3 v1 = mk3(sc.positions[3 * i1], sc.positions[3 * i1 + 1], sc.positions[3 * i1 + 2]);
-    V3 v2 = mk3(sc.positions[3 * i2], sc.positions[3 * i2 + 1], sc.positions[3 * i2 + 2]);
+    unsigned int i0 = 0u, i1 = 0u, i2 = 0u;
+    V3 v0, v1, v2, n_g;
+    bool from_record = false;
+    if constexpr (RECS) from_record = sc.light_tris != nullptr;
+    const bool uv_emission = LIGHTS != LIGHTS_AREA_ONLY && !__builtin_expect(mr.emission_type == 0, 1);
+    if (from_record) {
+        const float4* q = reinterpret_cast<const float4*>(sc.light_tris + (rec_base + prim));
+        const float4 q0 = q[0], q1 = q[1], q2 = q[2];
+        v0 = mk3(q0.x, q0.y, q0.z); v1 = mk3(q1.x, q1.y, q1.z); v2 = mk3(q2.x, q2.y, q2.z);
+        n_g = mk3(q0.w, q1.w, q2.w);
+        if (pdf_area < 0.0f) pdf_area = q[3].x;
+        if ((mr.flags & MESH_HAS_NORMALS) || uv_emission) { i0 = sc.tri_indices[3 * gtri]; i1 = sc.tri_indices[3 * gtri + 1]; i2 = sc.tri_indices[3 * gtri + 2]; }
+    } else {
+        i0 = sc.tri_indices[3 * gtri]; i1 = sc.tri_indices[3 * gtri + 1]; i2 = sc.tri_indices[3 * gtri + 2];
+        light_tri_corners(sc, i0, i1, i2, &v0, &v1, &v2);
+        n_g = light_tri_normal(v0, v1, v2);
+    }
     V2 b = uniform_sample_triangle(uv);
     float w2 = 1.0f - b.x - b.y;
     V3 pos = v0 * b.x + v1 * b.y + v2 * w2;
-    V3 n_g = normalize(cross(v2 - v0, v1 - v0));
     if (mr.flags & MESH_HAS_NORMALS) {
         V3 n0 = mk3(sc.normals[3 * i0], sc.normals[3 * i0 + 1], sc.normals[3 * i0 + 2]);
         V3 n1 = mk3(sc.normals[3 * i1], sc.normals[3 * i1 + 1], sc.normals[3 * i1 + 2]);
@@ -498,14 +517,14 @@
         else if (nl != 1.0f) n = n / sqrt_rn(nl);
         if (dot(n_g, n) < 0.0f) n_g = -n_g;
     }
-    if (pdf_area < 0.0f) pdf_area = div_rn(1.0f, length(cross(v1 - v0, v2 - v0)) * 0.5f);
+    if (pdf_area < 0.0f) pdf_area = light_tri_inv_area(v0, v1, v2);
     V3 d = pos - p;
     float dist = length(d);
     if (dist != 0.0f) d = d / dist;
     float geom = dist != 0.0f ? div_rn(rmax(dot(n_g, -d), 0.0f), dist * dist) : 0.0f;
     float pdf = geom == 0.0f ? 0.0f : div_rn(pdf_area, geom);
     Col emit;
-    if (LIGHTS == LIGHTS_AREA_ONLY || __builtin_expect(mr.emission_type == 0, 1)) emit = mkc(mr.emission[0], mr.emission[1], mr.emission[2]);
+    if (!uv_emission) emit = mkc(mr.emission[0], mr.emission[1], mr.emission[2]);
     else emit = mesh_emit_sampled(sc.bitmaps, sc.bitmap_texels, sc.uvs, mr.emission_type, mr.emission_scale, mr.emission_bitmap, (mr.flags & MESH_HAS_UV) != 0, i0, i1, i2, b.x, b.y, w2);
     ls->weight = pdf == 0.0f ? czero() : emit * geom / pdf_area;
     ls->pdf = pdf; ls->pdf_kind = PDF_SOLID_ANGLE;
@@ -572,16 +591,19 @@
     return pdf;
 }
 
-template <int LIGHTS = LIGHTS_ANY>
+template <int LIGHTS = LIGHTS_ANY, bool RECS = false>
 RL_DEV LightSample sample_light(const DeviceScene& sc, V3 p, bool has_n, V3 n, float r_sel, float r, V2 uv) {
     if (LIGHTS != LIGHTS_AREA_ONLY && sc.ats_root >= 0) {
         float pdf_sel;
         int li = ats_sample(sc, r_sel, p, has_n, n, &pdf_sel);
         LightSample ls;
         ls.kind = EMITTER_MESH;
-        mesh_sample_triangle<LIGHTS>(sc, sc.meshes[sc.ats_light_mesh[li]], (unsigned int)sc.ats_light_prim[li], -1.0f, p, uv, &ls);
-        ls.weight = div_unguarded(ls.weight, pdf_sel);
-        ls.pdf = ls.pdf * pdf_sel;
+        const int lm = sc.ats_light_mesh[li];
+        mesh_sample_triangle<LIGHTS, RECS>(sc, sc.meshes[lm], (RECS && sc.light_tris) ? sc.light_tri_base[lm] : 0u, (unsigned int)sc.ats_light_prim[li], -1.0f, p, uv, &ls);
+        if (!RECS || pdf_sel != 1.0f) {
+            ls.weight = div_unguarded(ls.weight, pdf_sel);
+            ls.pdf = ls.pdf * pdf_sel;
+        }
         return ls;
     }
     unsigned int id = cdf_sample(sc.emitters_cdf, sc.n_emitters + 1, r_sel);
@@ -592,7 +614,7 @@
     if (LIGHTS == LIGHTS_AREA_ONLY || em.kind == EMITTER_MESH) {
         MeshRecord mr = sc.meshes[em.mesh];
         unsigned int prim = cdf_sample(sc.mesh_cdf + mr.cdf_base, mr.n_tris + 1, r);
-        mesh_sample_triangle<LIGHTS>(sc, mr, prim, mr.inv_area, p, uv, &ls);
+        mesh_sample_triangle<LIGHTS, RECS>(sc, mr, em.light_tri_base, prim, mr.inv_area, p, uv, &ls);
     } else if (em.kind == EMITTER_POINT) {
         V3 lp = mk3(em.v[0], em.v[1], em.v[2]);
         V3 d = lp - p;
@@ -620,8 +642,10 @@
             ls.weight = lum / pdf;
         }
     }
-    ls.weight = div_unguarded(ls.weight, pdf_sel);
-    ls.pdf = ls.pdf * pdf_sel;
+    if (!RECS || pdf_sel != 1.0f || (LIGHTS != LIGHTS_AREA_ONLY && em.kind == EMITTER_DIRECTIONAL)) {
+        ls.weight = div_unguarded(ls.weight, pdf_sel);
+        ls.pdf = ls.pdf * pdf_sel;
+    }
     return ls;
 }
 
diff --git a/rustlight_amd/csrc/kernels/stages.hip.h b/rustlight_amd/csrc/kernels/stages.hip.h
--- a/rustlight_amd/csrc/kernels/stages.hip.h
+++ b/rustlight_amd/csrc/kernels/stages.hip.h
@@ -71,7 +71,7 @@
     PU(U_FLAGS) = ST_RAY | (PREV_SENSOR << ST_PREV_SHIFT) | ST_PDF_SA;
 }
 
-template <bool DYNAMIC, class PS, class SMP = Rng, bool TAIL = false>
+template <bool DYNAMIC, class PS, class SMP = Rng, bool TAIL = false, bool PIXEL_TABLE = true>
 RL_DEV void raygen_slot(const RenderConst& rc, const DeviceScene& sc, PS& ps, unsigned& n_samples, unsigned& n_draws) {
     unsigned flags = PU(U_FLAGS);
     if (!(flags & ST_REGEN)) return;
@@ -153,7 +153,8 @@
         rng = load_rng(ps, Q_R0);
     }
     unsigned px, py;
-    if (per_pixel) { unsigned pix = rc.item_pixel[TAIL ? pitem : (split > 1u ? item / split : item)]; px = pix % rc.W; py = pix / rc.W; }
+    if (per_pixel && PIXEL_TABLE) { const uint2 xy = rc.item_xy[TAIL ? pitem : (split > 1u ? item / split : item)]; px = xy.x; py = xy.y; }
+    else if (per_pixel) { unsigned pix = rc.item_pixel[TAIL ? pitem : (split > 1u ? item / split : item)]; px = pix % rc.W; py = pix / rc.W; }
     else { px = bx + cursor % bw; py = by + cursor / bw; }
     SMP smp = SmpState<SMP>::begin(rc, rng, TAIL ? pitem : (split > 1u ? item / split : item), s);
     float u = (float)px + smp_next(smp);
@@ -237,7 +238,7 @@
     if (shadow_visible(sc, recs, stack, load3(ps, F_OX), load3(ps, F_SX))) storec(ps, F_LR, loadc(ps, F_LR) + loadc(ps, F_CR));
 }
 
-template <int MAT, bool MEDIUM, int LIGHTS = LIGHTS_ANY, bool DRAWS_ONLY = false, class SMP = Rng, class PS>
+template <int MAT, bool MEDIUM, int LIGHTS = LIGHTS_ANY, bool DRAWS_ONLY = false, class SMP = Rng, bool RECS = false, class PS>
 RL_DEV void shade_slot(const RenderConst& rc, const DeviceScene& sc, PS& ps, unsigned flags,
                        unsigned& n_vertices, unsigned& n_draws, unsigned& n_shadow, unsigned& n_ext) {
     n_ext += 1;
@@ -383,7 +384,7 @@
                 V2 c = smp_next2d(rng);
                 n_draws += 4;
                 n_shadow += 1;
-                LightSample ls = sample_light<LIGHTS>(sc, vp, !is_volume, is_volume ? mk3(0.0f, 0.0f, 0.0f) : sp.n_s, a, b, c);
+                LightSample ls = sample_light<LIGHTS, RECS>(sc, vp, !is_volume, is_volume ? mk3(0.0f, 0.0f, 0.0f) : sp.n_s, a, b, c);
                 if (ls.pdf != 0.0f) {
                     Col wl;
                     float p_dir;
diff --git a/rustlight_amd/csrc/kernels/wavefront.hip b/rustlight_amd/csrc/kernels/wavefront.hip
--- a/rustlight_amd/csrc/kernels/wavefront.hip
+++ b/rustlight_amd/csrc/kernels/wavefront.hip
@@ -37,6 +37,7 @@
             unsigned k = base + iy * bw + ix;
             rc.item_seed[k] = rng_next_u64(rng);
             rc.item_pixel[k] = (by + iy) * rc.W + (bx + ix);
+            if (rc.item_xy) rc.item_xy[k] = make_uint2(bx + ix, by + iy);
         }
 }
 
@@ -46,7 +47,29 @@
     unsigned bx, by, bw, bh;
     block_geometry(rc, rc.owned_blocks[j], &bx, &by, &bw, &bh);
     const unsigned c_end = min(rc.cursor_end, bw * bh), base = rc.block_item_base[j];
-    for (unsigned c = rc.cursor_begin; c < c_end; c++) rc.item_pixel[base + (c - rc.cursor_begin)] = (by + c / bw) * rc.W + (bx + c % bw);
+    for (unsigned c = rc.cursor_begin; c < c_end; c++) {
+        rc.item_pixel[base + (c - rc.cursor_begin)] = (by + c / bw) * rc.W + (bx + c % bw);
+        if (rc.item_xy) rc.item_xy[base + (c - rc.cursor_begin)] = make_uint2(bx + c % bw, by + c / bw);
+    }
+}
+
+__global__ void k_light_tri_records(DeviceScene sc, LightTriRecord* out, const uint32_t* rec_mesh, unsigned n_records) {
+    const unsigned r = blockIdx.x * blockDim.x + threadIdx.x;
+    if (r >= n_records) return;
+    const unsigned mesh = rec_mesh[r];
+    const MeshRecord mr = sc.meshes[mesh];
+    const unsigned gtri = mr.tri_base + (r - sc.light_tri_base[mesh]);
+    const unsigned i0 = sc.tri_indices[3 * gtri], i1 = sc.tri_indices[3 * gtri + 1], i2 = sc.tri_indices[3 * gtri + 2];
+    V3 v0, v1, v2;
+    light_tri_corners(sc, i0, i1, i2, &v0, &v1, &v2);
+    const V3 n_g = light_tri_normal(v0, v1, v2);
+    LightTriRecord rec;
+    rec.v0[0] = v0.x; rec.v0[1] = v0.y; rec.v0[2] = v0.z; rec.n0 = n_g.x;
+    rec.v1[0] = v1.x; rec.v1[1] = v1.y; rec.v1[2] = v1.z; rec.n1 = n_g.y;
+    rec.v2[0] = v2.x; rec.v2[1] = v2.y; rec.v2[2] = v2.z; rec.n2 = n_g.z;
+    rec.inv_area = light_tri_inv_area(v0, v1, v2);
+    rec.pad[0] = rec.pad[1] = rec.pad[2] = 0.0f;
+    out[r] = rec;
 }
 
 __global__ void k_init(RenderConst rc, Pool pool) {
@@ -251,6 +274,7 @@
     HipBuffer<unsigned> d_owned, d_item_base;
     HipBuffer<unsigned long long> d_block_seeds, d_item_seed;
     HipBuffer<unsigned> d_item_pixel;
+    HipBuffer<uint2> d_item_xy;
     HipBuffer<float> d_out;
     HipBuffer<Counters> d_counters;
     HipBuffer<Counters, Mem::Pinned> h_counters;
@@ -374,7 +398,6 @@
         if ((rc = upload(ctx, flat.materials, &ds.materials)) != RL_OK) break;
         if ((rc = upload(ctx, flat.bitmaps, &ds.bitmaps)) != RL_OK) break;
         if ((rc = upload(ctx, flat.bitmap_texels, &ds.bitmap_texels)) != RL_OK) break;
-        if ((rc = upload(ctx, scene->emitters, &ds.emitters)) != RL_OK) break;
         if ((rc = upload(ctx, scene->emitters_cdf, &ds.emitters_cdf)) != RL_OK) break;
         ds.n_emitters = (uint32_t)scene->emitters.size();
         ds.env_emitter = -1;
@@ -441,6 +464,29 @@
             treelet_blocks(bvh, &blocks, &root_t);
             if ((rc = upload(ctx, blocks, &ds.nodes_t)) != RL_OK) break;
             ds.root_t = root_t;
+        }
+        {
+            std::vector<uint32_t> base(flat.meshes.size(), 0u), rec_mesh;
+            for (size_t m = 0; m < flat.meshes.size(); m++) {
+                if (!(flat.meshes[m].flags & MESH_IS_LIGHT)) continue;
+                base[m] = (uint32_t)rec_mesh.size();
+                rec_mesh.insert(rec_mesh.end(), flat.meshes[m].n_tris, (uint32_t)m);
+            }
+            ds.light_tris = nullptr; ds.light_tri_base = nullptr;
+            std::vector<EmitterRecord> emitters = scene->emitters;
+            for (EmitterRecord& e : emitters) if (e.kind == EMITTER_MESH) e.light_tri_base = base[e.mesh];
+            if ((rc = upload(ctx, emitters, &ds.emitters)) != RL_OK) break;
+            if (!rec_mesh.empty()) {
+                const uint32_t* d_rec_mesh = nullptr;
+                const LightTriRecord* d_recs = nullptr;
+                if ((rc = upload(ctx, base, &ds.light_tri_base)) != RL_OK) break;
+                if ((rc = upload(ctx, rec_mesh, &d_rec_mesh)) != RL_OK) break;
+                if ((rc = upload(ctx, std::vector<LightTriRecord>(rec_mesh.size()), &d_recs)) != RL_OK) break;
+                const unsigned n = (unsigned)rec_mesh.size();
+                hipLaunchKernelGGL(k_light_tri_records, dim3((n + 63u) / 64u), dim3(64), 0, ctx->stream, ds, const_cast<LightTriRecord*>(d_recs), d_rec_mesh, n);
+                if (hipGetLastError() != hipSuccess || hipStreamSynchronize(ctx->stream) != hipSuccess) { rl_set_error("building the light-triangle records failed"); rc = RL_ERR_HIP; break; }
+                ds.light_tris = d_recs;
+            }
         }
         if (ctx->d_counters.ensure(1) != RL_OK) { rl_set_error("hipMalloc counters"); rc = RL_ERR_HIP; break; }
         if (ctx->h_counters.ensure(1) != RL_OK) { rl_set_error("hipHostMalloc counters"); rc = RL_ERR_HIP; break; }
```

After: 5542 (median of 6 runs). About the same (+0.8%).
